# baurst/liso

Measured on AMD Instinct MI355X. Metric: LISO train-step frames/sec (120k-pt clouds), higher is better.
Workload: dtype bf16 (detector, BASELINE configs[2]) + f32 via bf16x3 MFMA (SLIM); north_star's 1e-3 on logits / flow is met by `parity_leg` (f32 via bf16x3 MFMA everywhere) and `fp32_exact_leg`, not by the bf16 detector

## Files before the change

### include/liso_pillars.h

```cpp
#ifndef LISO_PILLARS_H
#define LISO_PILLARS_H

#include <stddef.h>
#include <stdint.h>

#ifdef __cplusplus
extern "C" {
#endif

#define LISO_PFN_OUT 64
#define LISO_PILLARS_MAX_BATCH 32
#define LISO_PFN_STATS_DOUBLES 80

typedef struct {
    float x_min, y_min, z_min;
    float vx, vy, vz;
    int gx, gy;
    int max_points;
    int max_voxels;
    int n_channels;
} liso_pillar_cfg;

size_t liso_pillars_voxelize_workspace_bytes(const liso_pillar_cfg* cfg, int batch, int n_total);

int liso_pillars_voxelize_f32(const float* points, const int* offsets_host, int batch, const liso_pillar_cfg* cfg,
                              int* coors, int* num_points, int* slots, int* num_voxels, int* cell_to_voxel,
                              void* workspace, size_t workspace_bytes, void* stream);

size_t liso_pfn_decorate_workspace_bytes(int batch, int max_voxels);
int liso_pfn_decorate_f32(const float* points, const liso_pillar_cfg* cfg, int batch, const int* coors, const int* num_points,
                          const int* slots, const int* num_voxels, int* pt_off, float* feat, int* voxel_cell, void* workspace,
                          size_t workspace_bytes, void* stream);

size_t liso_pfn_partials_bytes(void);
int liso_pfn_bn_prepare_f32(const float* feat, const int* pt_off, const liso_pillar_cfg* cfg, int batch, const int* num_voxels,
                            const float* weight, const float* gamma, const float* beta, float* running_mean,
                            float* running_var, float momentum, float eps, int training, float* bn_out, double* moments,
                            void* partials, void* stream);

int liso_pfn_forward_scatter(const float* feat, const int* pt_off, const int* voxel_cell, const liso_pillar_cfg* cfg, int batch,
                             const int* cell_to_voxel, const float* weight, const float* bn_out, void* canvas, int out_bf16,
                             float* occupancy, void* stream);

int liso_pfn_forward_rows(const float* feat, const int* pt_off, const int* voxel_cell, const liso_pillar_cfg* cfg, int batch,
                          const int* cell_to_voxel, const float* weight, const float* bn_out, void* rows, int out_bf16, int row_base,
                          int* cell_to_row, float* occupancy, void* stream);

int liso_pfn_backward(const float* feat, const int* pt_off, const int* voxel_cell, const liso_pillar_cfg* cfg, int batch,
                      const int* num_voxels, const float* weight, const float* gamma, const float* bn_out,
                      const double* moments, int training, const void* grad_canvas, int grad_bf16, float* grad_weight,
                      float* grad_gamma, float* grad_beta, void* partials, void* stream);

#ifdef __cplusplus
}
#endif
#endif
```

### liso_amd/_lib.py

```python
import ctypes
import os

import torch

_HERE = os.path.dirname(os.path.abspath(__file__))
LIB_PATH = os.path.join(_HERE, "libliso_hip.so")

_lib = None


class LisoHipError(RuntimeError):
    pass


_ERRORS = {-1: "LISO_EINVAL (bad pointer/size)", -2: "LISO_EWORKSPACE (workspace too small)",
           -3: "LISO_ELAUNCH (HIP launch failed)", -4: "LISO_GROUND_ELENGTH (int(67 / delta_R) > 255)"}


def _preload_torch_hip_runtime():
    tl = os.path.join(os.path.dirname(torch.__file__), "lib", "libamdhip64.so")
    if os.path.exists(tl):
        ctypes.CDLL(tl, mode=ctypes.RTLD_GLOBAL)


def lib():
    global _lib
    if _lib is None:
        if not os.path.exists(LIB_PATH):
            raise LisoHipError(
                f"{LIB_PATH} not found: build it with `python -c 'import __graft_entry__ as g; g.build()'` "
                "or `make -C liso_amd/csrc`.  liso_amd has no CPU fallback for device ops.")
        _preload_torch_hip_runtime()
        _lib = ctypes.CDLL(LIB_PATH)
        _declare(_lib)
    return _lib


def check(code, what):
    if code != 0:
        raise LisoHipError(f"{what} failed: {_ERRORS.get(code, code)}")


def stream_ptr(device=None):
    return ctypes.c_void_p(torch.cuda.current_stream(device).cuda_stream)


def ptr(t):
    return ctypes.c_void_p(t.data_ptr())


def multi_copy(pairs):
    import torch

    fast = []
    for d, s_ in pairs:
        if (d.is_cuda and s_.is_cuda and d.device == s_.device and d.dtype == s_.dtype and d.shape == s_.shape and d.is_contiguous()
                and s_.is_contiguous() and (not fast or fast[0][0].device == d.device)):
            if d.numel() and d.data_ptr() != s_.data_ptr():
                fast.append((d, s_))
        else:
            d.copy_(s_, non_blocking=True)
    if len(fast) == 1:
        fast[0][0].copy_(fast[0][1], non_blocking=True)
    elif fast:
        n = len(fast)
        dst = (ctypes.c_void_p * n)(*[d.data_ptr() for d, _ in fast])
        src = (ctypes.c_void_p * n)(*[s_.data_ptr() for _, s_ in fast])
        nb = (ctypes.c_size_t * n)(*[d.numel() * d.element_size() for d, _ in fast])
        with torch.cuda.device(fast[0][0].device):
            check(lib().liso_multi_copy(n, dst, src, nb, stream_ptr()), "multi_copy")


def copy_blocks(jobs):
    import torch

    n = len(jobs)
    if n == 0:
        return
    dst = (ctypes.c_void_p * n)()
    src = (ctypes.c_void_p * n)()
    rows = (ctypes.c_uint * n)()
    rb = (ctypes.c_uint * n)()
    ds = (ctypes.c_size_t * n)()
    ss = (ctypes.c_size_t * n)()

    def rows_view(t):
        assert t.dtype == torch.float32 and t.is_cuda
        if t.dim() == 1:
            assert t.stride(0) == 1 or t.numel() <= 1
            return 1, t.numel(), t.numel()
        inner = 1
        for k in range(t.dim() - 1, 0, -1):
            assert t.shape[k] == 1 or t.stride(k) == inner, (tuple(t.shape), t.stride())
            inner *= t.shape[k]
        return t.shape[0], inner, (t.stride(0) if t.shape[0] > 1 else inner)

    for i, (d, s_) in enumerate(jobs):
        assert tuple(d.shape) == tuple(s_.shape), (tuple(d.shape), tuple(s_.shape))
        r, c, dstr = rows_view(d)
        r2, c2, sstr = rows_view(s_)
        assert (r, c) == (r2, c2)
        dst[i], src[i], rows[i], rb[i], ds[i], ss[i] = d.data_ptr(), s_.data_ptr(), r, 4 * c, 4 * dstr, 4 * sstr
    with torch.cuda.device(jobs[0][0].device):
        check(lib().liso_multi_copy_rows(n, dst, src, rows, rb, ds, ss, stream_ptr()), "multi_copy_rows")


def require_cuda(*tensors):
    for t in tensors:
        if not t.is_cuda:
            raise LisoHipError("device op called with a CPU tensor; liso_amd has no CPU fallback")


_vp, _i, _f, _sz, _lg = ctypes.c_void_p, ctypes.c_int, ctypes.c_float, ctypes.c_size_t, ctypes.c_long
_d = ctypes.c_double

SIGNATURES = {
    "liso_iou3d_overlap_bev_f32": (_i, [_vp, _i, _vp, _i, _vp, _vp]),
    "liso_iou3d_iou_bev_f32": (_i, [_vp, _i, _vp, _i, _vp, _vp]),
    "liso_iou3d_nms_workspace_bytes": (_sz, [_i]),
    "liso_iou3d_nms_f32": (_i, [_vp, _i, _f, _vp, _vp, _vp, _sz, _vp]),
    "liso_iou3d_nms_normal_f32": (_i, [_vp, _i, _f, _vp, _vp, _vp, _sz, _vp]),
    "liso_iou3d_iou_bev_cpu_f32": (_i, [_vp, _i, _vp, _i, _vp]),
    "liso_pillars_voxelize_workspace_bytes": (_sz, [_vp, _i, _i]),
    "liso_pillars_voxelize_f32": (_i, [_vp, _vp, _i, _vp, _vp, _vp, _vp, _vp, _vp, _vp, _sz, _vp]),
    "liso_pfn_partials_bytes": (_sz, []),
    "liso_pfn_decorate_workspace_bytes": (_sz, [_i, _i]),
    "liso_pfn_decorate_f32": (_i, [_vp, _vp, _i, _vp, _vp, _vp, _vp, _vp, _vp, _vp, _vp, _sz, _vp]),
    "liso_pfn_bn_prepare_f32": (_i, [_vp, _vp, _vp, _i, _vp, _vp, _vp, _vp, _vp, _vp, _f, _f, _i, _vp, _vp, _vp, _vp]),
    "liso_pfn_forward_scatter": (_i, [_vp, _vp, _vp, _vp, _i, _vp, _vp, _vp, _vp, _i, _vp, _vp]),
    "liso_pfn_forward_rows": (_i, [_vp, _vp, _vp, _vp, _i, _vp, _vp, _vp, _vp, _i, _i, _vp, _vp, _vp]),
    "liso_pfn_backward": (_i, [_vp, _vp, _vp, _vp, _i, _vp, _vp, _vp, _vp, _vp, _i, _vp, _i, _vp, _vp, _vp, _vp, _vp]),
    "liso_kabsch_workspace_bytes": (_sz, [_vp]),
    "liso_kabsch_trafos_f32": (_i, [_vp, _vp, _vp, _vp, _vp, _vp, _vp, _vp, _vp, _vp, _vp, _sz, _vp]),
    "liso_kabsch_trafos_counted_f32": (_i, [_vp, _vp, _vp, _vp, _vp, _vp, _vp, _vp, _vp, _vp, _vp, _vp, _sz, _vp]),
    "liso_symm_ortho_fwd_f64": (_i, [_vp, _i, _vp, _vp, _vp, _vp, _vp]),
    "liso_symm_ortho_bwd_f64": (_i, [_vp, _vp, _vp, _vp, _i, _vp, _vp]),
    "liso_weighted_moments_workspace_bytes": (_sz, [_i]),
    "liso_weighted_moments_fwd_f32": (_i, [_vp, _vp, _vp, _i, ctypes.c_long, _vp, _vp, _sz, _vp]),
    "liso_weighted_moments_bwd_f32": (_i, [_vp, _vp, _vp, _i, ctypes.c_long, _vp, _vp, _vp, _vp, _vp]),
    "liso_bev_dynamic_flow_workspace_bytes": (_sz, [_i, _i, _i]),
    "liso_bev_dynamic_flow_f32": (_i, [_vp, _i, _vp, _vp, _vp, _i, _vp, _i, _i, _i, _i, _vp, _vp, _vp, _sz, _vp]),
    "liso_odom_inverse_minus_eye_f64": (_i, [_vp, _i, _vp, _vp]),
    "liso_fit_box_z_workspace_bytes": (_sz, [_i, _i]),
    "liso_fit_box_z_f32": (_i, [_vp, _i, _i, _vp, _i, _vp, _i, _vp, _i, _f, _vp, _vp, _vp, _vp, _sz, _vp]),
    "liso_dbscan_components": (_i, [_vp, _vp, _vp, _vp, _vp, _vp, _vp, _vp, _vp]),
    "liso_dbscan_labels": (_i, [_vp, _vp, _vp, _vp, _vp, _vp, _vp, _vp, _vp, _vp]),
    "liso_region_props": (_i, [_vp, _i, _i, _i, _i, _vp, _vp, _vp]),
    "liso_region_props_workspace_bytes": (_sz, [_i, _i, _i, _i]),
    "liso_region_props_ws": (_i, [_vp, _i, _i, _i, _i, _vp, _vp, _vp, _sz, _vp]),
    "liso_corr_lookup_fwd_f32": (_i, [_vp, _vp, _vp, _vp, _vp, _vp]),
    "liso_corr_lookup_fwd_tiled_f32": (_i, [_vp, _vp, _vp, _vp, _vp, _vp]),
    "liso_corr_lookup_bwd_dvol_f32": (_i, [_vp, _vp, _vp, _vp, _vp]),
    "liso_corr_pyramid_fwd_f32": (_i, [_vp, _vp, _vp, _vp]),
    "liso_corr_pyramid_bwd_f32": (_i, [_vp, _vp, _vp, _vp]),
    "liso_corr_bwd_features_workspace_bytes": (_sz, [_vp]),
    "liso_corr_bwd_features_f32": (_i, [_vp, _i, _vp, _vp, _vp, _vp, _vp, _vp, _sz, _vp]),
    "liso_rows_combine_f32": (_i, [_lg, _i, _vp, _lg, _vp, _lg, _vp, _lg, _vp, _lg, _vp, _lg, _i, _vp]),
    "liso_gru_out_rows_train_f32": (_i, [_lg, _i, _vp, _lg, _vp, _vp, _lg, _vp, _lg, _vp]),
    "liso_gru_out_rows_bwd_f32": (_i, [_lg, _i, _vp, _lg, _vp, _vp, _lg, _vp, _lg, _vp, _lg, _vp, _vp, _vp]),
    "liso_gru_in_rows_bwd_f32": (_i, [_lg, _i, _vp, _lg, _vp, _lg, _vp, _vp, _vp, _lg, _vp, _lg, _vp, _vp]),
    "liso_raft_state_step_train_f32": (_i, [_i, _i, _vp, _vp, _vp, _vp, _vp, _vp, _vp, _vp, _vp]),
    "liso_raft_pack_output_grads_f32": (_i, [_lg, _i, _vp, _vp, _vp, _vp]),
    "liso_nearest_point_loss_fwd_f32": (_i, [_vp] * 8),
    "liso_nearest_point_loss_bwd_f32": (_i, [_vp] * 9),
    "liso_slim_decode_weights_fwd": (_i, [_vp] * 6 + [_i] + [_vp] * 4),
    "liso_slim_decode_weights_bwd": (_i, [_vp] * 9),
    "liso_slim_decode_points_fwd": (_i, [_vp] * 9),
    "liso_slim_decode_points_bwd": (_i, [_vp] * 11),
    "liso_slim_loss_workspace_bytes": (_sz, []),
    "liso_slim_static_points_loss_fwd": (_i, [_i, ctypes.c_long, _vp, _i, _vp, _vp, _vp, _vp, _vp, _vp, _sz, _vp]),
    "liso_slim_static_points_loss_bwd": (_i, [_i, ctypes.c_long, _vp, _i, _vp, _vp, _vp, _vp, _vp, _vp, _vp, _vp, _vp]),
    "liso_slim_knn_queries": (_i, [_i, _i, ctypes.c_long, _i, _vp, _i, _vp, _vp, _vp, _vp, _vp]),
    "liso_slim_nearest_point_loss_fwd": (_i, [_vp, _vp, _i, _vp, _vp, _vp, _i, _vp, _vp, _vp, _vp, _vp, _sz, _vp]),
    "liso_slim_nearest_point_loss_bwd": (_i, [_vp, _vp, _i, _vp, _vp, _vp, _i, _vp, _vp, _vp, _vp, _vp, _vp, _vp]),
    "liso_bev_gather_fwd_f32": (_i, [_vp, _vp, ctypes.c_long, _i, ctypes.c_float, _vp, _vp]),
    "liso_bev_gather_bwd_f32": (_i, [_vp, _vp, _vp, _vp, ctypes.c_long, _i, _vp, _vp, _vp]),
    "liso_gru_in_fwd_f32": (_i, [_vp, _vp, _vp, ctypes.c_long, _vp, _vp, _vp, _vp, _vp]),
    "liso_gru_in_bwd_f32": (_i, [_vp, _vp, ctypes.c_long, _vp, _vp, _vp, _vp, _vp, _vp, ctypes.c_long, _vp, _vp]),
    "liso_gru_out_fwd_f32": (_i, [ctypes.c_long, _vp, _vp, _vp, _vp, _vp]),
    "liso_gru_out_bwd_f32": (_i, [ctypes.c_long, _vp, _vp, _vp, _vp, _vp, _vp, _vp, _vp]),
    "liso_gru_in_rows_f32": (_i, [ctypes.c_long, _i, _vp, ctypes.c_long, _vp, ctypes.c_long, _vp, _vp, ctypes.c_long, _vp]),
    "liso_gru_out_rows_f32": (_i, [ctypes.c_long, _i, _vp, ctypes.c_long, _vp, _vp, ctypes.c_long, _vp]),
    "liso_multi_copy": (_i, [_i, _vp, _vp, _vp, _vp]),
    "liso_bev_lin_index": (_i, [_vp, _i, _vp, _i, ctypes.c_long, _i, _i, _vp, _vp]),
    "liso_channel_extrema_workspace_bytes": (_sz, []),
    "liso_channel_extrema_f32": (_i, [_vp, ctypes.c_long, _i, _i, _vp, _vp, _sz, _vp]),
    "liso_bev_plan_tile_lin": (_i, [_vp, _i, ctypes.c_long, _i, _i, _i, _i, _vp, _vp]),
    "liso_bev_plan_rank": (_i, [_vp, _vp, ctypes.c_long, _vp, _vp, _vp]),
    "liso_bev_plan_expand": (_i, [_vp, _vp, _vp, _i, ctypes.c_long, _i, _i, _i, _i, _vp, _vp, _vp, _vp]),
    "liso_raft_state_step_f32": (_i, [_i, _i, _vp, ctypes.c_long, _vp, _vp, _vp, _vp]),
    "liso_raft_upsample_scratch_bytes": (_sz, [_vp]),
    "liso_raft_upsample_outputs_fwd_f32": (_i, [_vp] * 5),
    "liso_raft_upsample_outputs_bwd_f32": (_i, [_vp, _vp, _vp, _sz, _vp, _vp, _vp]),
    "liso_centerloss_workspace_bytes": (_sz, [_vp]),
    "liso_centerloss_fwd_f32": (_i, [_vp] * 17 + [_sz, _vp]),
    "liso_centerloss_bwd_f32": (_i, [_vp] * 21),
    "liso_render_center_targets_f32": (_i, [_vp] * 12),
    "liso_conv_pack_weights_batched": (_i, [_vp, _i, _vp]),
    "liso_conv_pack_weights_placed": (_i, [_vp, _i, _i, _vp]),
    "liso_conv_in_finalize": (_i, [_vp, _i, _i, _i, _i, ctypes.c_long, _vp, _vp, _f, _vp, _vp]),
    "liso_residual_affine_relu_f32": (_i, [_vp, _vp, _vp, _i, _i, _vp, _vp, _vp, _i, _i, _vp, _i, ctypes.c_long, _i, _vp]),
    "liso_scan_workspace_bytes": (_sz, [_i, ctypes.c_long]),
    "liso_scan_inclusive_i32": (_i, [_vp, _i, ctypes.c_long, _vp, _vp, _sz, _vp]),
    "liso_mine_boxes_from_regions": (_i, [_vp, _i, _i, _vp, _i, _vp, _i, _f, _f, _vp, _vp, _vp, _vp, _vp, _vp]),
    "liso_mine_filter_compact": (_i, [_vp] * 21),
    "liso_mine_box_motion": (_i, [_vp, _i, _i, _vp, _vp, _vp, _vp]),
    "liso_mine_nms_workspace_bytes": (_sz, [_i, _i]),
    "liso_mine_nms_prepare": (_i, [_i, _i, _i] + [_vp] * 11 + [_sz, _vp]),
    "liso_mine_nms_finish": (_i, [_i, _i, _i] + [_vp] * 16),
    "liso_adamw_step_f32": (_i, [_vp, _vp, _vp, _vp, _sz] + [ctypes.c_double] * 5 + [ctypes.c_long, _vp]),
    "liso_adamw_step_scaled_f32": (_i, [_vp, _vp, _vp, _vp, _sz] + [ctypes.c_double] * 6 + [ctypes.c_long, _vp]),
    "liso_adamw_pack_table_plan": (_i, [_vp, _i, _sz, _vp, _vp]),
    "liso_adamw_pack_table_fill": (_i, [_vp, _i, _sz, _vp, _sz]),
    "liso_adamw_step_packed_f32": (_i, [_vp, _vp, _vp, _vp, _sz] + [ctypes.c_double] * 6 + [ctypes.c_long, _vp, _i, _vp]),
    "liso_grad_nonfinite_f32": (_i, [_vp, _sz, _vp, _vp]),
    "liso_adamw_step_amp_f32": (_i, [_vp, _vp, _vp, _vp, _sz] + [ctypes.c_double] * 6 + [_vp, _vp]),
    "liso_loss_scale_update": (_i, [_vp, ctypes.c_double, ctypes.c_double, _i, _vp]),
    "liso_rmsprop_step_f32": (_i, [_vp, _vp, _vp, _sz] + [ctypes.c_double] * 4 + [_vp]),
    "liso_multi_copy_rows": (_i, [_i, _vp, _vp, _vp, _vp, _vp, _vp, _vp]),
    "liso_gather_f32": (_i, [_i, _vp, _vp, _vp, _vp]),
    "liso_bn_workspace_bytes": (_sz, [_i]),
    "liso_bn_relu_fwd": (_i, [_vp, _i, ctypes.c_long, _i, _vp, _vp, _vp, _vp, _f, _f, _i, _i, _vp, _vp, _vp, _sz, _vp]),
    "liso_in_workspace_bytes": (_sz, [_i, _i]),
    "liso_in_relu_fwd": (_i, [_vp, _i, _i, ctypes.c_long, _i, _vp, _vp, _f, _i, _vp, _vp, _vp, _sz, _vp]),
    "liso_in_relu_bwd": (_i, [_vp, _vp, _i, _i, ctypes.c_long, _i, _vp, _vp, _i, _vp, _vp, _vp, _vp, _sz, _vp]),
    "liso_in_relu_bwd_sum": (_i, [_vp, _vp, _i, _i, ctypes.c_long, _i, _vp, _vp, _i, _vp, _vp, _vp, _vp, _sz, _vp]),
    "liso_bn_relu_bwd": (_i, [_vp, _vp, _i, ctypes.c_long, _i, _vp, _vp, _i, _i, _vp, _vp, _vp, _vp, _sz, _vp]),
    "liso_bn_relu_bwd_strided": (_i, [_vp, ctypes.c_long, _vp, ctypes.c_long, _i, ctypes.c_long, _i, _vp, _vp, _i, _i, _vp, ctypes.c_long, _vp, _vp, _vp, _sz, _vp]),
    "liso_bn_relu_bwd_chained": (_i, [_vp, ctypes.c_long, _vp, ctypes.c_long, _i, ctypes.c_long, _i, _vp, _vp, _i, _i, _vp, ctypes.c_long, _vp, _vp, _vp, _sz, _vp, _vp]),
    "liso_bn_multi_workspace_bytes": (_sz, [_vp, _i, _i]),
    "liso_bn_relu_bwd_multi": (_i, [_vp, ctypes.c_long, _vp, ctypes.c_long, _vp, ctypes.c_long, _i, ctypes.c_long, _vp, _i, _i, _i, _vp, ctypes.c_long,
                                    _vp, _sz, _vp, _vp, _vp]),
    "liso_bn_relu_bwd_multi_check": (_i, [_vp, _i, _i, _i, ctypes.c_long, ctypes.c_long, ctypes.c_long, ctypes.c_long, ctypes.c_long, _vp]),
    "liso_knn_workspace_bytes": (_sz, [_vp, _i]),
    "liso_knn_build_f32": (_i, [_vp, _vp, _i, _i, _vp, _sz, _vp]),
    "liso_knn_sorted_ids": (_i, [_vp, _vp, _i, _vp, _vp]),
    "liso_knn_query_f32": (_i, [_vp, _vp, _vp, _vp, _i, _vp, _i, _i, _vp, _vp, _i, _vp]),
    "liso_conv_packed_bytes": (_sz, [_i, _i, _i, _i]),
    "liso_conv_pack_weights": (_i, [_vp, _i, _i, _i, _i, _i, _i, _i, _vp, _vp]),
    "liso_conv_stats_rows": (_i, [_vp]),
    "liso_conv_kernel_kind": (_i, [_vp]),
    "liso_conv_forward": (_i, [_vp] * 10),
    "liso_conv_set_option": (_i, [_i, _i]),
    "liso_conv_forward_sparse": (_i, [_vp] * 11),
    "liso_conv_plan_info": (_i, [_vp, _vp]),
    "liso_conv_wgrad_workspace_bytes": (_sz, [_vp]),
    "liso_conv_wgrad": (_i, [_vp, _vp, _vp, _vp, _vp, _i, _i, _vp, _vp, _vp, _sz, _vp]),
    "liso_conv_wgrad_deferred": (_i, [_vp, _vp, _vp, _vp, _vp, _i, _i, _vp, _vp, _vp, _sz, _vp, _vp]),
    "liso_conv_wgrad_reduce": (_i, [_vp, _vp]),
    "liso_conv_wgrad_sparse_workspace_bytes": (_sz, [_vp]),
    "liso_conv_wgrad_sparse_f32": (_i, [_vp, _vp, _vp, _vp, _i, _vp, _vp, _vp, _sz, _vp]),
    "liso_conv_wgrad_smallci_workspace_bytes": (_sz, [_i, _i, _i, _i, _i]),
    "liso_conv_wgrad_smallci_f32": (_i, [_vp, ctypes.c_long, _vp, ctypes.c_long, _i, _i, _i, _i, _i, _vp, _vp, _vp, _sz, _vp]),
    "liso_sparse_conv_stat_groups": (_i, [_i, _i, _i]),
    "liso_sparse_conv_workspace_bytes": (_sz, [_i, _i, _i, _i, _i, _i, _i]),
    "liso_sparse_conv_forward": (_i, [_vp, ctypes.c_long, _i, _vp, _vp, _vp, _i, _i, _i, _i, _i, _i, _i, _vp, _vp, _vp, _vp, _vp, _sz, _vp]),
    "liso_sparse_conv_forward_rows": (_i, [_vp, ctypes.c_long, _i, _vp, ctypes.c_long, _vp, _vp, _vp, _i, _i, _i, _i, _i, _i, _i, _vp, _vp, _vp, _vp, _vp,
                                           _sz, _vp]),
    "liso_sparse_conv_dgrad": (_i, [_vp, ctypes.c_long, _i, _vp, _vp, _i, _i, _i, _i, _i, _i, _vp, ctypes.c_long, _vp, _vp, _sz, _i, _vp]),
    "liso_sparse_stem_workspace_bytes": (_sz, [_i, _i, _i, _i]),
    "liso_sparse_stem_forward_f32": (_i, [_vp, ctypes.c_long, _vp, _vp, _vp, _i, _i, _i, _i, _i, _vp, _vp, _vp, _vp, _sz, _vp]),
    "liso_conv_bn_finalize": (_i, [_vp, _i, _i, _i, ctypes.c_long, _vp, _vp, _vp, _vp, _vp, _f, _f, _vp, _vp]),
    "liso_conv_bn_finalize_merged": (_i, [_vp, _i, _i, _i, ctypes.c_long, _vp, _vp, _vp, _vp, _vp, _f, _f, _vp, _vp, _vp, _i, _i, _vp]),
    "liso_points_in_boxes_workspace_bytes": (_sz, [_vp]),
    "liso_points_in_boxes_f32": (_i, [_vp] * 9 + [_sz, _vp]),
    "liso_match_greedy_f32": (_i, [_vp, ctypes.c_long, ctypes.c_long, _i, _i, _vp, _f, _vp, _vp, _vp, _vp, _vp, _vp, _vp]),
    "liso_fit_boxes_closeness_workspace_bytes": (_sz, [ctypes.c_long, _i]),
    "liso_fit_boxes_closeness_f32": (_i, [_vp, ctypes.c_long, _i, _vp, _vp, _i, _f, _vp, _vp, _vp, _sz, _vp]),
    "liso_bike_rollout_fwd_f32": (_i, [_i, _i, _vp, _vp, _vp, _vp, _f, _f, _f, _vp, _vp]),
    "liso_bike_rollout_bwd_f32": (_i, [_i, _i, _vp, _vp, _vp, _f, _f, _f, _vp, _vp, _vp, _vp, _vp, _vp]),
    "liso_smooth_tracks_jerk_f32": (_i, [_vp, _vp, _i, _i, _i, _f, _f, _vp, _vp]),
    "liso_flow_metrics_state_bytes": (_sz, []),
    "liso_flow_metrics_result_bytes": (_sz, []),
    "liso_flow_metrics_reset": (_i, [_vp, _vp]),
    "liso_flow_metrics_update": (_i, [_vp, _lg, _vp, _lg, _vp, _lg, _i, _vp, _lg, _vp, _lg, _vp, _lg, _vp, _vp, _vp, _vp, _i, _vp, _vp]),
    "liso_flow_metrics_read": (_i, [_vp, _vp, _vp]),
    "liso_det_nms_workspace_bytes": (_sz, [_i, _i]),
    "liso_det_nms_order": (_i, [_i, _i, _vp, _vp, _vp, _f, _vp, _vp, _vp, _sz, _vp]),
    "liso_det_nms_select": (_i, [_i, _i, _vp, _vp, _vp, _f, _i, _i, _vp, _vp, _vp]),
    "liso_det_nms_gather": (_i, [_i, _i, _i, _vp, _vp, _vp, _i, _vp]),
    "liso_det_val_pairs_f32": (_i, [_i, _i, _i] + [_vp] * 8),
    "liso_det_val_pairs_cpu_f32": (_i, [_i, _i, _i] + [_vp] * 7),
    "liso_det_val_transfer_classes": (_i, [_i, _i, _i] + [_vp] * 5 + [_f, _vp, _vp, _vp]),
    "liso_det_val_match_f32": (_i, [_i, _i, _i] + [_vp] * 10 + [_i, _vp, _i, _vp, _i] + [_vp] * 6),
    "liso_det_val_assign_f32": (_i, [_i, _i, _i] + [_vp] * 8 + [_i, _vp, _i, _vp, _i] + [_vp] * 5),
    "liso_match_assign_f32": (_i, [_vp, ctypes.c_long, _i, _i, _f, _vp, _vp, _vp]),
    "liso_ground_jcp_workspace_bytes": (_sz, [_vp]),
    "liso_ground_jcp_f32": (_i, [_vp, _vp, _vp, _vp, _vp, _sz, _vp]),
    "liso_ground_jcp_stages_f32": (_i, [_vp, _vp, _vp, _vp, _vp, _sz, _i, _i, _vp]),
    "liso_ground_cone_f32": (_i, [_i, _i, _i, _vp, _vp, ctypes.c_double, ctypes.c_double, _vp, _vp, _vp]),
    "liso_ground_compact_workspace_bytes": (_sz, [_i, _i]),
    "liso_ground_compact_f32": (_i, [_i, _i, _i, _vp, _vp, _vp, _vp, _vp, _vp, _sz, _vp]),
    "liso_bev_free_mask_workspace_bytes": (_sz, [_i, _i]),
    "liso_bev_free_mask": (_i, [_vp, ctypes.c_long, _i, _i, _i, _vp, _vp, _vp, _sz, _vp]),
    "liso_bev_select_free_cells": (_i, [_vp, _vp, _i, _i, _vp, _i, _vp, _vp]),
    "liso_snippet_paste": (_i, [_vp, ctypes.c_long, _vp, _vp, _vp, _vp, ctypes.c_double, ctypes.c_double, _i, _vp, _vp, _vp, _vp]),
    "liso_sample_transform_f32": (_i, [_i, _i, _i] + [_vp] * 7),
    "liso_sample_transform_poses_f64": (_i, [_i, _vp, _vp, _i, _vp, _i, _vp]),
    "liso_bev_crop_workspace_bytes": (_sz, [_i, _i]),
    "liso_bev_crop_f32": (_i, [_vp] * 14 + [_sz, _vp]),
    "liso_bev_point_maps_workspace_bytes": (_sz, [_i, _i, _i, _i]),
    "liso_bev_point_maps_f32": (_i, [_i] * 5 + [_vp] * 6 + [ctypes.c_double] + [_vp] * 5 + [_sz, _vp]),
    "liso_box_has_points_f32": (_i, [_i] * 4 + [_vp] * 7),
    "liso_filter_boxes": (_i, [_vp] * 6 + [_i] + [_vp] * 3),
    "liso_object_velocity_f64": (_i, [_i, _i] + [_vp] * 5),
    "liso_ignore_region_mask": (_i, [_i] * 4 + [ctypes.c_double] * 2 + [_vp] * 6),
    "liso_render_center_targets_ex_f32": (_i, [_vp] * 15),
    "liso_snippet_cut_workspace_bytes": (_sz, [_i, _i, _i]),
    "liso_snippet_cut_f32": (_i, [_i, _i, _i, _vp, _vp, _vp, _i, _vp, _vp, _lg] + [_vp] * 5 + [_sz, _vp]),
    "liso_track_sequences_workspace_bytes": (_sz, [_i, _i, _i, _i]),
    "liso_track_sequences": (_i, [_i] * 4 + [_vp] * 7 + [ctypes.c_double] + [_vp] * 10 + [_sz, _vp]),
    "liso_track_mining_workspace_bytes": (_sz, [_i] * 5),
    "liso_select_tracks": (_i, [_i] * 5 + [_vp] * 7 + [_i, _f, _d, _d, _i, _d, _d, _i, _d] + [_vp] * 13 + [_vp, _sz, _vp]),
    "liso_refine_tracks_apply": (_i, [_i] * 3 + [_vp] * 12 + [_i, _i, _d] + [_vp] * 7 + [_vp]),
    "liso_export_tracks": (_i, [_i] * 6 + [_vp] * 11 + [_i] + [_vp] * 13 + [_vp, _sz, _vp]),
    "liso_frame_prep_workspace_bytes": (_sz, [_vp]),
    "liso_prepare_tracker_frames": (_i, [_vp] * 27 + [_sz, _vp]),
    "liso_odometry_workspace_bytes": (_sz, [_vp]),
    "liso_odometry_workspace_layout": (_i, [_vp, _vp]),
    "liso_odometry_preprocess": (_i, [_vp, _i, _vp, _vp, _vp, _vp, _vp, _sz, _vp]),
    "liso_odometry_register": (_i, [_vp, _i] + [_vp] * 8 + [_sz, _vp]),
    "liso_odometry_map_update": (_i, [_vp, _i, _vp, _vp, _vp, _vp, _sz, _vp]),
    "liso_odometry_sequences": (_i, [_vp] * 11 + [_sz, _vp]),
    "liso_odometry_relative_f64": (_i, [_i, _vp, _vp, _vp, _vp]),
    "liso_correct_kitti_scan_f64": (_i, [_lg, _vp, _vp, _vp]),
    "liso_flow_labels_workspace_bytes": (_sz, [_i, _i]),
    "liso_flow_labels_f32": (_i, [_vp] * 18 + [_sz, _vp]),
    "liso_kitti_rows_cols_f32": (_i, [_i, _i, _i, _vp, _vp, _d, _i, _i, _vp, _vp, _vp]),
}


CONV_MAX_TAPS, CONV_MAX_CLASSES, CONV_BF16, CONV_F32X3, CONV_F32, CONV_F16 = 49, 4, 0, 1, 2, 3
ELEM_F32, ELEM_BF16, ELEM_F16 = 0, 1, 2
_ELEM_CODES = {torch.float32: ELEM_F32, torch.bfloat16: ELEM_BF16, torch.float16: ELEM_F16}
LOSS_SCALE_STATE_BYTES = 32


def elem_code(dtype):
    code = _ELEM_CODES.get(dtype)
    if code is None:
        raise TypeError(f"no device kernel takes {dtype} tensors (float32, bfloat16 or float16)")
    return code


def is_half(dtype):
    return elem_code(dtype) != ELEM_F32


def lane_channels(dtype):
    return 8 if is_half(dtype) else 4
CONV_OPT_SHARED_GPU = 1
CONV_OPT_ROLES_CUS = 2


class ConvDesc(ctypes.Structure):
    _fields_ = [("batch", _i), ("hi", _i), ("wi", _i), ("ci", _i), ("x_pix_stride", _i), ("ho", _i), ("wo", _i), ("co", _i),
                ("y_pix_stride", _i), ("y_ch_off", _i), ("hv", _i), ("wv", _i), ("isy", _i), ("isx", _i), ("osy", _i), ("osx", _i),
                ("n_classes", _i), ("class_tap_begin", _i * (CONV_MAX_CLASSES + 1)), ("class_ooy", _i * CONV_MAX_CLASSES),
                ("class_oox", _i * CONV_MAX_CLASSES), ("n_taps", _i), ("tap_dy", _i * CONV_MAX_TAPS), ("tap_dx", _i * CONV_MAX_TAPS),
                ("tap_w", _i * CONV_MAX_TAPS), ("w_taps", _i), ("mode", _i), ("out_f32", _i), ("in_relu", _i), ("out_relu", _i),
                ("in_affine_batch_stride", _i), ("wgrad_co", _i)]


class ConvPackPlacedJob(ctypes.Structure):
    _fields_ = [("src", _vp), ("dst", _vp), ("d0", _i), ("d1", _i), ("kh", _i), ("kw", _i), ("transposed", _i), ("for_dgrad", _i),
                ("mode", _i), ("K", _i), ("N", _i), ("k_offset", _i), ("n_offset", _i)]


class AdamwPackDest(ctypes.Structure):
    _fields_ = [("dst", _vp), ("for_dgrad", _i), ("mode", _i), ("K", _i), ("N", _i), ("k_offset", _i), ("n_offset", _i)]


class AdamwPackItem(ctypes.Structure):
    _fields_ = [("offset", _sz), ("d0", _i), ("d1", _i), ("kh", _i), ("kw", _i), ("transposed", _i), ("n_dest", _i),
                ("dest", AdamwPackDest * 2), ("mirror", _vp), ("mirror_row_stride", _sz)]


class ConvPackJob(ctypes.Structure):
    _fields_ = [("src", _vp), ("dst", _vp), ("d0", _i), ("d1", _i), ("kh", _i), ("kw", _i), ("transposed", _i), ("for_dgrad", _i),
                ("mode", _i)]


class WgradReduceJob(ctypes.Structure):
    _fields_ = [("slab", _vp), ("bias_slab", _vp), ("dw", _vp), ("dbias", _vp), ("cip", ctypes.c_long), ("cop", ctypes.c_long),
                ("splits", _i), ("bias_rows", _i), ("taps", _i), ("ci", _i), ("co", _i), ("transposed", _i)]


BN_MAX_GROUPS = 4


class BnGroup(ctypes.Structure):
    _fields_ = [("c_off", _i), ("c", _i), ("gamma", _vp), ("stats", _vp), ("grad_gamma", _vp), ("grad_beta", _vp)]


class KnnGrid(ctypes.Structure):
    _fields_ = [("x_min", _f), ("y_min", _f), ("cell", _f), ("nx", _i), ("ny", _i), ("z_min", _f), ("z_cell", _f), ("nz", _i)]


class CenterLossCfg(ctypes.Structure):
    _fields_ = [("batch", _i), ("h", _i), ("w", _i), ("res_x", _f), ("res_y", _f), ("z_min", _f), ("z_max", _f),
                ("sup_weight", _f), ("rot_reg_weight", _f)]


class NpLossCfg(ctypes.Structure):
    _fields_ = [("batch", _i), ("n", ctypes.c_long), ("n_b", ctypes.c_long), ("ext", _f * 4), ("fov_mode", _i), ("delta", _f)]


class SlimDecodeCfg(ctypes.Structure):
    _fields_ = [("samples", _i), ("n", ctypes.c_long), ("h", _i), ("w", _i), ("logit_mode", _i * 4), ("static_flow_zero", _i),
                ("dynamic_flow_zero", _i), ("overwrite_flow", _i), ("overwrite_logits", _i), ("non_rigid", _i), ("use_static_aggr", _i),
                ("dyn_grad_scale", _f), ("ext_lo", ctypes.c_double * 2), ("ext_span", ctypes.c_double * 2)]


class SlimDecodeOut(ctypes.Structure):
    FIELDS = ("dis_logit", "dis", "logits", "probs", "staticness", "dynamicness", "groundness", "dyn_flow", "stat_flow", "agg_flow", "saf_flow")
    _fields_ = [(k, _vp) for k in FIELDS] + [("flags", _vp)]


class SlimNpLossCfg(ctypes.Structure):
    _fields_ = [("samples", _i), ("clouds", _i), ("n", ctypes.c_long), ("n_b", ctypes.c_long), ("ext", _f * 4), ("fov_mode", _i), ("delta", _f)]


class BoxPtsCfg(ctypes.Structure):
    _fields_ = [("batch", _i), ("n", ctypes.c_long), ("k", _i), ("point_stride", _i), ("precision", _i), ("dims_bloat", _f)]


class FramePrepCfg(ctypes.Structure):
    _fields_ = [("n_seq", _i), ("max_frames", _i), ("max_box", _i), ("cap", _i), ("n_points", ctypes.c_long), ("point_stride", _i),
                ("n_fov_points", ctypes.c_long), ("fov_stride", _i), ("bev_range_x", _f), ("bev_range_y", _f), ("drop_on_bev_boundaries", _i),
                ("min_points_in_box", _i), ("fov_min_points", _i), ("align", _i), ("no_align_below_m", _d), ("full_align_above_m", _d)]


class OdometryCfg(ctypes.Structure):
    _fields_ = [("n_seq", _i), ("max_frames", _i), ("n_max", _i), ("point_stride", _i), ("map_voxels", _i), ("max_points_per_voxel", _i),
                ("max_num_iterations", _i), ("max_range", _d), ("min_range", _d), ("voxel_size", _d), ("initial_threshold", _d),
                ("min_motion_th", _d), ("convergence_criterion", _d)]


class GruCfg(ctypes.Structure):
    _fields_ = [("batch", _i), ("ch", _i), ("cx", _i), ("hw", ctypes.c_long)]


class UpsampleCfg(ctypes.Structure):
    _fields_ = [("n_it", _i), ("batch2", _i), ("dirs", _i), ("h", _i), ("w", _i), ("factor", _i), ("flow_scale", _f)]


class MineFilterCfg(ctypes.Structure):
    _fields_ = [("batch", _i), ("k", _i), ("min_points", _i), ("aspect_ratio_max", ctypes.c_double), ("max_box_len_m", ctypes.c_double),
                ("min_box_area_m2", ctypes.c_double), ("min_box_volume_m3", ctypes.c_double), ("park_invalid", _i)]


class DetGatherField(ctypes.Structure):
    _fields_ = [("src", _vp), ("dst", _vp), ("row_elems", _i), ("elem_bytes", _i), ("pad_bits", ctypes.c_uint64)]


class GroundCfg(ctypes.Structure):
    _fields_ = [("batch", _i), ("n_max", _i), ("point_stride", _i), ("width", _i), ("height", _i),
                ("sensor_height", ctypes.c_double), ("delta_r", ctypes.c_double)]


class TargetsCfg(ctypes.Structure):
    _fields_ = [("batch", _i), ("n_boxes", _i), ("h", _i), ("w", _i), ("range_x", _f), ("range_y", _f)]


class DbscanCfg(ctypes.Structure):
    _fields_ = [("batch", _i), ("gx", _i), ("gy", _i), ("window", _i), ("min_samples", _i), ("eps", _f), ("flow_weight", _f)]


class CorrCfg(ctypes.Structure):
    _fields_ = [("batch", _i), ("h", _i), ("w", _i), ("dim", _i), ("levels", _i), ("radius", _i)]


class KabschCfg(ctypes.Structure):
    _fields_ = [("batch", _i), ("n_points", _i), ("n_slots", _i), ("point_stride", _i), ("flow_stride", _i),
                ("slope", _f), ("scale_fg", _f), ("scale_bg", _f), ("softness", _i)]


class PillarCfg(ctypes.Structure):
    _fields_ = [("x_min", _f), ("y_min", _f), ("z_min", _f), ("vx", _f), ("vy", _f), ("vz", _f), ("gx", _i),
                ("gy", _i), ("max_points", _i), ("max_voxels", _i), ("n_channels", _i)]


class _Everything:
    def __contains__(self, name):
        return True


class KernelTimer:

    def __init__(self):
        self.enabled = set()
        self.events = {}
        self.units = {}
        self.bytes = {}
        self.weights = {}
        self.weight = 1.0

    def enable(self, name):
        self.enabled.add(name)
        self.events.setdefault(name, [])

    def enable_all(self):
        self.enabled = _Everything()

    def disable_all(self):
        self.enabled = set()

    def launch(self, name, fn, units=None, nbytes=None):
        if name not in self.enabled:
            return fn()
        a, b = torch.cuda.Event(enable_timing=True), torch.cuda.Event(enable_timing=True)
        a.record()
        r = fn()
        b.record()
        self.events.setdefault(name, []).append((a, b))
        self.weights.setdefault(name, []).append(float(self.weight))
        if units is not None:
            self.units.setdefault(name, []).append(units)
        if nbytes is not None:
            self.bytes.setdefault(name, []).append(nbytes)
        return r

    def mean_units(self, name):
        u = self.units.get(name, [])
        return sum(u) / len(u) if u else None

    def durations_ms(self, name):
        torch.cuda.synchronize()
        return [a.elapsed_time(b) for a, b in self.events.get(name, [])]

    def weighted_total_ms(self, name):
        return sum(d * w for d, w in zip(self.durations_ms(name), self.weights.get(name, [])))

    def reset(self):
        for k in self.events:
            self.events[k] = []
        self.units = {}
        self.bytes = {}
        self.weights = {}


TIMER = KernelTimer()


def _declare(l):
    for name, (res, args) in SIGNATURES.items():
        fn = getattr(l, name)
        fn.restype = res
        fn.argtypes = args
```

### liso_amd/csrc/pillars.hip

```cpp
#include <hip/hip_runtime.h>
#include <stdlib.h>
#include "zero_fill.h"
#include <cstring>
#include <hip/hip_bf16.h>
#include <limits.h>
#include <stdint.h>

#include "../../include/liso_iou3d.h"
#include "../../include/liso_conv.h"
#include "../../include/liso_pillars.h"
#include "dev_common.h"

namespace {

using liso_dev::check_launch;

constexpr int kTile = 1024;
constexpr int kOut = LISO_PFN_OUT;
constexpr int kFP = 12;
constexpr int kMaxPts = 32;
constexpr int kPfnThreads = 256;
constexpr int kPfnGrid = 1024;

struct BatchInfo {
    int off[LISO_PILLARS_MAX_BATCH + 1];
    int tile_off[LISO_PILLARS_MAX_BATCH + 1];
};

__device__ __forceinline__ int sample_of(const BatchInfo& bi, int batch, int i) {
    int b = 0;
    while (b + 1 < batch && i >= bi.off[b + 1]) b++;
    return b;
}

__global__ void assign_kernel(const float* __restrict__ pts, int n_total, int C, BatchInfo bi, int batch,
                              liso_pillar_cfg cfg, int* __restrict__ cell_of_point, int* __restrict__ count,
                              int* __restrict__ first_enc, int* __restrict__ pos_in_cell) {
    const int i = blockIdx.x * blockDim.x + threadIdx.x;
    int cell = -1;
    if (i < n_total) {
        const float* p = pts + (size_t)i * C;
        const float cx = floorf((p[0] - cfg.x_min) / cfg.vx);
        const float cy = floorf((p[1] - cfg.y_min) / cfg.vy);
        const float cz = floorf((p[2] - cfg.z_min) / cfg.vz);
        const bool ok = cx >= 0.f && cx < (float)cfg.gx && cy >= 0.f && cy < (float)cfg.gy && cz >= 0.f && cz < 1.f;
        if (ok) cell = (sample_of(bi, batch, i) * cfg.gx + (int)cx) * cfg.gy + (int)cy;
        cell_of_point[i] = cell;
    }
    const int lane = threadIdx.x & 63;
    const int prev = __shfl_up(cell, 1);
    const unsigned long long heads = __ballot(lane == 0 || cell != prev);
    const unsigned long long below = heads & ((2ull << lane) - 1ull);
    const int head_lane = 63 - __builtin_clzll(below);
    const unsigned long long above = lane == 63 ? 0ull : heads & ~((2ull << lane) - 1ull);
    const int next_head = above ? __ffsll((long long)above) - 1 : 64;
    int base = 0;
    if (cell >= 0 && head_lane == lane) {
        base = atomicAdd(&count[cell], next_head - lane);
        atomicMax(&first_enc[cell], INT_MAX - i);
    }
    base = __shfl(base, head_lane);
    if (i < n_total) pos_in_cell[i] = cell >= 0 ? base + (lane - head_lane) : 0;
}

__device__ __forceinline__ bool is_first(const int* cell_of_point, const int* first_enc, int i) {
    const int cell = cell_of_point[i];
    return cell >= 0 && first_enc[cell] == INT_MAX - i;
}

__global__ __launch_bounds__(kTile) void tile_count_kernel(const int* __restrict__ cell_of_point,
                                                           const int* __restrict__ first_enc, BatchInfo bi, int batch,
                                                           int* __restrict__ tile_count) {
    __shared__ int wsum[kTile / 64];
    const int tile = blockIdx.x;
    int b = 0;
    while (b + 1 < batch && tile >= bi.tile_off[b + 1]) b++;
    const int i = bi.off[b] + (tile - bi.tile_off[b]) * kTile + threadIdx.x;
    const bool f = i < bi.off[b + 1] && is_first(cell_of_point, first_enc, i);
    const unsigned long long m = __ballot(f);
    if ((threadIdx.x & 63) == 0) wsum[threadIdx.x >> 6] = __popcll(m);
    __syncthreads();
    if (threadIdx.x == 0) {
        int s = 0;
        for (int w = 0; w < kTile / 64; w++) s += wsum[w];
        tile_count[tile] = s;
    }
}

__global__ __launch_bounds__(kTile) void rank_kernel(const int* __restrict__ cell_of_point,
                                                     const int* __restrict__ first_enc,
                                                     const int* __restrict__ count, BatchInfo bi, int batch,
                                                     liso_pillar_cfg cfg, const int* __restrict__ tile_count,
                                                     int* __restrict__ coors, int* __restrict__ num_points,
                                                     int* __restrict__ cell_to_voxel, int* __restrict__ num_voxels) {
    __shared__ int wsum[kTile / 64];
    __shared__ int base_s;
    const int tile = blockIdx.x;
    int b = 0;
    while (b + 1 < batch && tile >= bi.tile_off[b + 1]) b++;
    if (threadIdx.x < 64) {
        int s = 0;
        for (int t = bi.tile_off[b] + threadIdx.x; t < tile; t += 64) s += tile_count[t];
        for (int o = 32; o > 0; o >>= 1) s += __shfl_xor(s, o);
        if (threadIdx.x == 0) base_s = s;
    }
    const int i = bi.off[b] + (tile - bi.tile_off[b]) * kTile + threadIdx.x;
    const bool f = i < bi.off[b + 1] && is_first(cell_of_point, first_enc, i);
    const unsigned long long m = __ballot(f);
    const int lane = threadIdx.x & 63, wave = threadIdx.x >> 6;
    if (lane == 0) wsum[wave] = __popcll(m);
    __syncthreads();
    int pre = base_s;
    for (int w = 0; w < wave; w++) pre += wsum[w];
    if (f) {
        const int ord = pre + __popcll(m & ((1ULL << lane) - 1ULL));
        if (ord < cfg.max_voxels) {
            const int cell = cell_of_point[i];
            const int v = b * cfg.max_voxels + ord;
            cell_to_voxel[cell] = v + 1;
            const int within = cell - b * cfg.gx * cfg.gy;
            coors[v * 4 + 0] = b;
            coors[v * 4 + 1] = 0;
            coors[v * 4 + 2] = within / cfg.gy;
            coors[v * 4 + 3] = within % cfg.gy;
            const int c = count[cell];
            num_points[v] = c < cfg.max_points ? c : cfg.max_points;
        }
    }
    if (tile == bi.tile_off[b + 1] - 1 && threadIdx.x == 0) {
        int tot = base_s;
        for (int w = 0; w < kTile / 64; w++) tot += wsum[w];
        num_voxels[b] = tot < cfg.max_voxels ? tot : cfg.max_voxels;
    }
}

constexpr int kScanTile = 1024;
__global__ __launch_bounds__(kScanTile) void cell_scan_block_kernel(const int* __restrict__ count, size_t cells, int* __restrict__ seg_off,
                                                                    int* __restrict__ block_tot) {
    __shared__ int wsum[kScanTile / 64];
    const size_t i = (size_t)blockIdx.x * kScanTile + threadIdx.x;
    const int lane = threadIdx.x & 63, wave = threadIdx.x >> 6;
    const int v = i < cells ? count[i] : 0;
    int incl = v;
#pragma unroll
    for (int o = 1; o < 64; o <<= 1) {
        const int t = __shfl_up(incl, o);
        if (lane >= o) incl += t;
    }
    if (lane == 63) wsum[wave] = incl;
    __syncthreads();
    int base = 0;
    for (int w = 0; w < wave; w++) base += wsum[w];
    if (i < cells) seg_off[i] = base + incl - v;
    if (threadIdx.x == kScanTile - 1) block_tot[blockIdx.x] = base + incl;
}

__global__ __launch_bounds__(1024) void cell_scan_tot_kernel(int* __restrict__ block_tot, int nblk) {
    __shared__ int wsum[16];
    const int t = threadIdx.x, lane = t & 63, wave = t >> 6;
    int v[4], tot = 0;
#pragma unroll
    for (int k = 0; k < 4; k++) {
        const int q = t * 4 + k;
        v[k] = q < nblk ? block_tot[q] : 0;
        tot += v[k];
    }
    int incl = tot;
#pragma unroll
    for (int o = 1; o < 64; o <<= 1) {
        const int up = __shfl_up(incl, o);
        if (lane >= o) incl += up;
    }
    if (lane == 63) wsum[wave] = incl;
    __syncthreads();
    int base = 0;
    for (int w = 0; w < wave; w++) base += wsum[w];
    int run = base + incl - tot;
#pragma unroll
    for (int k = 0; k < 4; k++) {
        const int q = t * 4 + k;
        if (q < nblk) block_tot[q] = run;
        run += v[k];
    }
}

__global__ __launch_bounds__(256) void seg_fill_kernel(const int* __restrict__ cell_of_point, int n_total, const int* __restrict__ seg_off,
                                                       const int* __restrict__ block_tot, const int* __restrict__ pos_in_cell,
                                                       int* __restrict__ seg) {
    const int i = blockIdx.x * blockDim.x + threadIdx.x;
    if (i >= n_total) return;
    const int c = cell_of_point[i];
    if (c < 0) return;
    seg[seg_off[c] + block_tot[c / kScanTile] + pos_in_cell[i]] = i;
}

constexpr int kSlotRegs = 16;
__device__ __forceinline__ void voxel_slots_one(const int* __restrict__ coors, const int* __restrict__ num_voxels, int max_voxels, int gx, int gy,
                                                const int* __restrict__ seg_off, const int* __restrict__ block_tot,
                                                const int* __restrict__ count, const int* __restrict__ seg, int max_points,
                                                int* __restrict__ slots, long v, int lane) {
    const int b = (int)(v / max_voxels), ord = (int)(v % max_voxels);
    if (ord >= num_voxels[b]) return;
    const int c = (b * gx + coors[v * 4 + 2]) * gy + coors[v * 4 + 3];
    const int off = seg_off[c] + block_tot[c / kScanTile], n = count[c];
    int* out = slots + (size_t)v * max_points;
    if (n <= 64) {
        const int e = lane < n ? seg[off + lane] : 0x7fffffff;
        int r = 0;
        for (int k = 0; k < n; k++) r += __shfl(e, k) < e ? 1 : 0;
        if (lane < n && r < max_points) out[r] = e;
        return;
    }
    int last = -1;
    const int rounds = min(max_points, n);
    if (n <= 64 * kSlotRegs) {
        int x[kSlotRegs];
#pragma unroll
        for (int u = 0; u < kSlotRegs; u++) x[u] = lane + 64 * u < n ? seg[off + lane + 64 * u] : 0x7fffffff;
        for (int r = 0; r < rounds; r++) {
            int m = 0x7fffffff;
#pragma unroll
            for (int u = 0; u < kSlotRegs; u++) m = (x[u] > last && x[u] < m) ? x[u] : m;
#pragma unroll
            for (int o = 32; o > 0; o >>= 1) m = min(m, __shfl_xor(m, o));
            if (lane == 0) out[r] = m;
            last = m;
        }
        return;
    }
    for (int r = 0; r < rounds; r++) {
        int m = 0x7fffffff;
        for (int j = lane; j < n; j += 64) {
            const int x = seg[off + j];
            m = (x > last && x < m) ? x : m;
        }
#pragma unroll
        for (int o = 32; o > 0; o >>= 1) m = min(m, __shfl_xor(m, o));
        if (lane == 0) out[r] = m;
        last = m;
    }
}

__global__ __launch_bounds__(256) void voxel_slots_kernel(const int* __restrict__ coors, const int* __restrict__ num_voxels, int max_voxels,
                                                          int batch, int gx, int gy, const int* __restrict__ seg_off,
                                                          const int* __restrict__ block_tot, const int* __restrict__ count,
                                                          const int* __restrict__ seg, int max_points, int* __restrict__ slots) {
    const int lane = threadIdx.x & 63;
    for (long v = (long)blockIdx.x * 4 + (threadIdx.x >> 6); v < (long)batch * max_voxels; v += (long)gridDim.x * 4)
        voxel_slots_one(coors, num_voxels, max_voxels, gx, gy, seg_off, block_tot, count, seg, max_points, slots, v, lane);
}

struct PfnGeom {
    float vx, vy, x_off, y_off, z_off;
};

__device__ __forceinline__ PfnGeom pfn_geom(const liso_pillar_cfg& c) {
    PfnGeom g;
    g.vx = c.vx; g.vy = c.vy;
    g.x_off = c.vx / 2 + c.x_min;
    g.y_off = c.vy / 2 + c.y_min;
    g.z_off = c.vz / 2 + c.z_min;
    return g;
}

constexpr int kGroup = 4;
constexpr int kStage = kGroup * kMaxPts;

__device__ __forceinline__ int kept_points(const int* __restrict__ num_points, const int* __restrict__ num_voxels, int max_voxels,
                                           int rows, int v) {
    if (v >= rows) return 0;
    const int b = v / max_voxels;
    return (v - b * max_voxels) < num_voxels[b] ? num_points[v] : 0;
}

__global__ __launch_bounds__(1024) void pfn_scan_block_kernel(const int* __restrict__ num_points, const int* __restrict__ num_voxels,
                                                              int max_voxels, int rows, int* __restrict__ pt_off,
                                                              int* __restrict__ block_tot) {
    __shared__ int wsum[16];
    const int i = blockIdx.x * 1024 + threadIdx.x;
    const int lane = threadIdx.x & 63, wave = threadIdx.x >> 6;
    const int v = kept_points(num_points, num_voxels, max_voxels, rows, i);
    int incl = v;
    for (int off = 1; off < 64; off <<= 1) {
        const int t = __shfl_up(incl, off);
        if (lane >= off) incl += t;
    }
    if (lane == 63) wsum[wave] = incl;
    __syncthreads();
    int base = 0;
    for (int w = 0; w < wave; w++) base += wsum[w];
    if (i < rows) pt_off[i] = base + incl - v;
    if (threadIdx.x == 1023) block_tot[blockIdx.x] = base + incl;
}

__global__ __launch_bounds__(1024) void pfn_scan_tot_kernel(int* __restrict__ block_tot, int nblocks) {
    __shared__ int wsum[16];
    const int lane = threadIdx.x & 63, wave = threadIdx.x >> 6;
    const int v = (int)threadIdx.x < nblocks ? block_tot[threadIdx.x] : 0;
    int incl = v;
    for (int off = 1; off < 64; off <<= 1) {
        const int t = __shfl_up(incl, off);
        if (lane >= off) incl += t;
    }
    if (lane == 63) wsum[wave] = incl;
    __syncthreads();
    int base = 0;
    for (int w = 0; w < wave; w++) base += wsum[w];
    if ((int)threadIdx.x < nblocks) block_tot[threadIdx.x] = base + incl - v;
    if ((int)threadIdx.x == nblocks - 1) block_tot[nblocks] = base + incl;
}

__global__ __launch_bounds__(1024) void pfn_scan_add_kernel(int* __restrict__ pt_off, int rows, const int* __restrict__ block_tot,
                                                            int nblocks) {
    const int i = blockIdx.x * 1024 + threadIdx.x;
    if (i < rows) pt_off[i] += block_tot[blockIdx.x];
    if (i == 0) pt_off[rows] = block_tot[nblocks];
}

template <int C>
__global__ __launch_bounds__(256) void pfn_decorate_kernel(const float* __restrict__ pts, liso_pillar_cfg cfg, int rows,
                                                           const int* __restrict__ coors, const int* __restrict__ num_points,
                                                           const int* __restrict__ slots, const int* __restrict__ num_voxels,
                                                           const int* __restrict__ pt_off, float* __restrict__ feat,
                                                           int* __restrict__ voxel_cell) {
#pragma clang fp contract(off)
    constexpr int F = C + 6;
    const long t = (long)blockIdx.x * blockDim.x + threadIdx.x;
    const int v = (int)(t >> 5), s = (int)(t & 31);
    if (v >= rows) return;
    const int num = kept_points(num_points, num_voxels, cfg.max_voxels, rows, v);
    const int xi = coors[v * 4 + 2], yi = coors[v * 4 + 3];
    if (s == 0) voxel_cell[v] = num > 0 ? ((v / cfg.max_voxels) * cfg.gx + xi) * cfg.gy + yi : -1;
    float p[C];
#pragma unroll
    for (int k = 0; k < C; k++) p[k] = 0.f;
    if (s < num) {
        const int idx = slots[(size_t)v * cfg.max_points + s];
        const float* q = pts + (size_t)idx * C;
        if constexpr (C == 4) {
            const float4 tt = *reinterpret_cast<const float4*>(q);
            p[0] = tt.x; p[1] = tt.y; p[2] = tt.z; p[3] = tt.w;
        } else {
#pragma unroll
            for (int k = 0; k < C; k++) p[k] = q[k];
        }
    }
    float sx = p[0], sy = p[1], sz = p[2];
#pragma unroll
    for (int o = 16; o > 0; o >>= 1) {
        sx += __shfl_xor(sx, o);
        sy += __shfl_xor(sy, o);
        sz += __shfl_xor(sz, o);
    }
    if (s >= num) return;
    const PfnGeom g = pfn_geom(cfg);
    const float fn = (float)num;
    const float mx = sx / fn, my = sy / fn, mz = sz / fn;
    const float fcx = p[0] - ((float)yi * g.vx + g.x_off);
    const float fcy = p[1] - ((float)xi * g.vy + g.y_off);
    const float fcz = p[2] - (0.f + g.z_off);
    float f[kFP];
#pragma unroll
    for (int k = 0; k < kFP; k++) f[k] = 0.f;
    f[0] = fcx; f[1] = fcy; f[2] = fcz;
#pragma unroll
    for (int k = 3; k < C; k++) f[k] = p[k];
    f[C + 0] = p[0] - mx; f[C + 1] = p[1] - my; f[C + 2] = p[2] - mz;
    f[C + 3] = fcx; f[C + 4] = fcy; f[C + 5] = fcz;
    f[F] = 1.f;
    float4* row = reinterpret_cast<float4*>(feat + ((size_t)pt_off[v] + s) * kFP);
    row[0] = make_float4(f[0], f[1], f[2], f[3]);
    row[1] = make_float4(f[4], f[5], f[6], f[7]);
    row[2] = make_float4(f[8], f[9], f[10], f[11]);
}

template <int C>
__global__ __launch_bounds__(kPfnThreads) void pfn_stats_kernel(const float* __restrict__ feat, const int* __restrict__ pt_off,
                                                                int rows, double* __restrict__ partials) {
    constexpr int F = C + 6, D = F + 1, NP = D * (D + 1) / 2;
    __shared__ __attribute__((aligned(16))) float tile[kPfnThreads / 64][64][kFP];
    __shared__ double red[kPfnThreads / 64][LISO_PFN_STATS_DOUBLES];
    const int lane = threadIdx.x & 63, wave = threadIdx.x >> 6;
    int pj[2] = {0, 0}, pk[2] = {0, 0};
    {
        int idx = 0;
        for (int j = 0; j < D; j++)
            for (int k = j; k < D; k++, idx++) {
                if (idx == lane) { pj[0] = j; pk[0] = k; }
                if (idx == lane + 64) { pj[1] = j; pk[1] = k; }
            }
    }
    const long n = pt_off[rows];
    const long waves = (long)gridDim.x * (kPfnThreads / 64);
    const long per = ((n + waves - 1) / waves + 63) / 64 * 64;
    const long w_id = (long)blockIdx.x * (kPfnThreads / 64) + wave;
    const long r0 = w_id * per, r1 = r0 + per < n ? r0 + per : n;
    double acc0 = 0.0, acc1 = 0.0;
    for (long base = r0; base < r1; base += 64) {
        const int cnt = (int)(r1 - base < 64 ? r1 - base : 64);
        const float4* src = reinterpret_cast<const float4*>(feat + (size_t)base * kFP);
        float4* dst = reinterpret_cast<float4*>(&tile[wave][0][0]);
        for (int i = lane; i < cnt * 3; i += 64) dst[i] = src[i];
        __builtin_amdgcn_wave_barrier();
        for (int s = 0; s < cnt; s++) {
            const float* f = tile[wave][s];
            acc0 += (double)f[pj[0]] * (double)f[pk[0]];
            if (lane + 64 < NP) acc1 += (double)f[pj[1]] * (double)f[pk[1]];
        }
        __builtin_amdgcn_wave_barrier();
    }
    red[wave][lane] = acc0;
    if (lane + 64 < LISO_PFN_STATS_DOUBLES) red[wave][lane + 64] = lane + 64 < NP ? acc1 : 0.0;
    __syncthreads();
    if (threadIdx.x < LISO_PFN_STATS_DOUBLES) {
        double s = 0.0;
        for (int w = 0; w < kPfnThreads / 64; w++) s += red[w][threadIdx.x];
        partials[(size_t)blockIdx.x * LISO_PFN_STATS_DOUBLES + threadIdx.x] = threadIdx.x < NP ? s : 0.0;
    }
}

__device__ __forceinline__ int pair_index(int j, int k, int D) {
    return j * D - j * (j - 1) / 2 + (k - j);
}

template <int C>
__global__ __launch_bounds__(1024) void pfn_bn_finalize_kernel(const double* __restrict__ partials, int nblocks,
                                                               const int* __restrict__ num_voxels, int batch,
                                                               int max_points, const float* __restrict__ weight,
                                                               const float* __restrict__ gamma,
                                                               const float* __restrict__ beta,
                                                               float* __restrict__ running_mean,
                                                               float* __restrict__ running_var, float momentum,
                                                               float eps, float* __restrict__ bn_out,
                                                               double* __restrict__ moments) {
    constexpr int F = C + 6, D = F + 1;
    constexpr int NS = LISO_PFN_STATS_DOUBLES, CH = 1024 / NS;
    __shared__ double part[CH][NS];
    __shared__ double mom[NS];
    const int e = threadIdx.x % NS, chunk = threadIdx.x / NS;
    if (chunk < CH) {
        double s = 0.0;
        const int per = (nblocks + CH - 1) / CH;
        const int lo = chunk * per, hi = lo + per < nblocks ? lo + per : nblocks;
        int blk = lo;
        for (; blk + 16 <= hi; blk += 16) {
            double v[16];
#pragma unroll
            for (int j = 0; j < 16; j++) v[j] = partials[(size_t)(blk + j) * NS + e];
#pragma unroll
            for (int j = 0; j < 16; j++) s += v[j];
        }
        for (; blk < hi; blk++) s += partials[(size_t)blk * NS + e];
        part[chunk][e] = s;
    }
    __syncthreads();
    if (threadIdx.x < NS) {
        double t = 0.0;
        for (int c = 0; c < CH; c++) t += part[c][threadIdx.x];
        mom[threadIdx.x] = t;
        moments[threadIdx.x] = t;
    }
    __syncthreads();
    __shared__ double rows_sq[kOut][F + 1], rows_sum[kOut][F + 1];
    if (threadIdx.x < kOut * F) {
        const int c = threadIdx.x / F, j = threadIdx.x % F;
        const double wj = (double)weight[c * F + j];
        double q = 0.0;
        for (int k = 0; k < F; k++) {
            const int a = j <= k ? j : k, bb = j <= k ? k : j;
            q += wj * (double)weight[c * F + k] * mom[pair_index(a, bb, D)];
        }
        rows_sq[c][j] = q;
        rows_sum[c][j] = wj * mom[pair_index(j, D - 1, D)];
    }
    __syncthreads();
    if (threadIdx.x < kOut) {
        const int c = threadIdx.x;
        long long P = 0;
        for (int b = 0; b < batch; b++) P += num_voxels[b];
        const double M = (double)P * (double)max_points;
        double sum = 0.0, sq = 0.0;
        for (int j = 0; j < F; j++) {
            sum += rows_sum[c][j];
            sq += rows_sq[c][j];
        }
        double mean = 0.0, var = 0.0;
        if (M > 0.0) {
            mean = sum / M;
            var = sq / M - mean * mean;
            if (var < 0.0) var = 0.0;
        }
        const double invstd = 1.0 / sqrt(var + (double)eps);
        const float scale = (float)((double)gamma[c] * invstd);
        bn_out[c] = scale;
        bn_out[kOut + c] = (float)((double)beta[c] - mean * (double)gamma[c] * invstd);
        bn_out[2 * kOut + c] = (float)mean;
        bn_out[3 * kOut + c] = (float)invstd;
        if (M > 1.0) {
            const double mo = (double)momentum;
            running_mean[c] = (float)((1.0 - mo) * (double)running_mean[c] + mo * mean);
            running_var[c] = (float)((1.0 - mo) * (double)running_var[c] + mo * (var * M / (M - 1.0)));
        }
    }
}

__global__ void pfn_bn_eval_kernel(const float* __restrict__ gamma, const float* __restrict__ beta,
                                   const float* __restrict__ running_mean, const float* __restrict__ running_var,
                                   float eps, float* __restrict__ bn_out) {
    const int c = threadIdx.x;
    if (c >= kOut) return;
    const float invstd = 1.f / sqrtf(running_var[c] + eps);
    bn_out[c] = gamma[c] * invstd;
    bn_out[kOut + c] = beta[c] - running_mean[c] * gamma[c] * invstd;
    bn_out[2 * kOut + c] = running_mean[c];
    bn_out[3 * kOut + c] = invstd;
}

template <typename T> __device__ __forceinline__ void store_out(T* p, float v);
template <> __device__ __forceinline__ void store_out<float>(float* p, float v) { *p = v; }
template <> __device__ __forceinline__ void store_out<__hip_bfloat16>(__hip_bfloat16* p, float v) { *p = __float2bfloat16(v); }
template <typename T> __device__ __forceinline__ float load_in(const T* p);
template <> __device__ __forceinline__ float load_in<float>(const float* p) { return *p; }
template <> __device__ __forceinline__ float load_in<__hip_bfloat16>(const __hip_bfloat16* p) { return __bfloat162float(*p); }
template <> __device__ __forceinline__ void store_out<_Float16>(_Float16* p, float v) { *p = (_Float16)v; }
template <> __device__ __forceinline__ float load_in<_Float16>(const _Float16* p) { return (float)*p; }

__device__ __forceinline__ void stage_rows(const float* __restrict__ feat, const int* __restrict__ pt_off, int rows, int v0, int lane,
                                           float (*frow)[kFP], int (&off)[kGroup + 1]) {
    int o = 0;
    if (lane <= kGroup) { const int v = v0 + lane; o = pt_off[v < rows ? v : rows]; }
#pragma unroll
    for (int g = 0; g <= kGroup; g++) off[g] = __shfl(o, g);
    const int total = off[kGroup] - off[0];
    const float4* src = reinterpret_cast<const float4*>(feat + (size_t)off[0] * kFP);
    float4* dst = reinterpret_cast<float4*>(&frow[0][0]);
    for (int i = lane; i < total * 3; i += 64) dst[i] = src[i];
}

constexpr int kCellsPerBlock = 256;

template <int C, typename OutT, bool ROWS>
__global__ __launch_bounds__(kPfnThreads) void pfn_forward_kernel(const float* __restrict__ feat, const int* __restrict__ pt_off,
                                                                  const int* __restrict__ voxel_cell, int rows, int max_points,
                                                                  long total_cells, int zero_blocks,
                                                                  const int* __restrict__ cell_to_voxel,
                                                                  const float* __restrict__ weight, const float* __restrict__ bn,
                                                                  OutT* __restrict__ canvas, float* __restrict__ occupancy,
                                                                  int* __restrict__ map_out, int row_base) {
    constexpr int F = C + 6;
    constexpr int kChunks = kOut * (int)sizeof(OutT) / 16;
    __shared__ __attribute__((aligned(16))) float frow[kPfnThreads / 64][kStage][kFP];
    __shared__ int vox[kCellsPerBlock];
    const int tid = threadIdx.x, lane = tid & 63, wave = tid >> 6;
    const int pillar_blocks = (int)gridDim.x - zero_blocks;
    if ((int)blockIdx.x >= pillar_blocks) {
        const long cell0 = (long)((int)blockIdx.x - pillar_blocks) * kCellsPerBlock;
        const long cell = cell0 + tid;
        int v1 = 0;
        if (cell < total_cells) {
            v1 = cell_to_voxel[cell];
            occupancy[cell] = v1 > 0 ? 1.f : 0.f;
            if constexpr (ROWS) map_out[cell] = v1 > 0 ? v1 + row_base : 0;
        }
        if constexpr (ROWS) return;
        vox[tid] = v1;
        __syncthreads();
        const uint4 z = make_uint4(0u, 0u, 0u, 0u);
        uint4* base = reinterpret_cast<uint4*>(canvas + (size_t)cell0 * kOut);
        for (int id = tid; id < kCellsPerBlock * kChunks; id += kPfnThreads) {
            const int cl = id / kChunks;
            if (cell0 + cl < total_cells && vox[cl] == 0) base[id] = z;
        }
        return;
    }
    float w[F];
#pragma unroll
    for (int k = 0; k < F; k++) w[k] = weight[lane * F + k];
    const float scale = bn[lane], shift = bn[kOut + lane];
    const float pad_val = fmaxf(shift, 0.f);
    const int wave_id = (int)blockIdx.x * (kPfnThreads / 64) + wave;
    const int n_waves = pillar_blocks * (kPfnThreads / 64);
    for (int v0 = wave_id * kGroup; v0 < rows; v0 += n_waves * kGroup) {
        int off[kGroup + 1];
        stage_rows(feat, pt_off, rows, v0, lane, frow[wave], off);
        int cell_l = -1;
        if (lane < kGroup && v0 + lane < rows) cell_l = voxel_cell[v0 + lane];
        __builtin_amdgcn_wave_barrier();
#pragma unroll
        for (int g = 0; g < kGroup; g++) {
            const int num = off[g + 1] - off[g];
            const int cell = __shfl(cell_l, g);
            if (num <= 0 || cell < 0) continue;
            float best = num < max_points ? pad_val : 0.f;
            const int r0 = off[g] - off[0];
            for (int s = 0; s < num; s++) {
                const float4* f4 = reinterpret_cast<const float4*>(frow[wave][r0 + s]);
                const float4 a = f4[0], b = f4[1], c4 = f4[2];
                const float f[kFP] = {a.x, a.y, a.z, a.w, b.x, b.y, b.z, b.w, c4.x, c4.y, c4.z, c4.w};
                float x = 0.f;
#pragma unroll
                for (int k = 0; k < F; k++) x = fmaf(w[k], f[k], x);
                best = fmaxf(best, fmaxf(fmaf(x, scale, shift), 0.f));
            }
            store_out<OutT>(canvas + (size_t)(ROWS ? v0 + g : cell) * kOut + lane, best);
        }
        __builtin_amdgcn_wave_barrier();
    }
}

template <int C, typename GT>
__global__ __launch_bounds__(kPfnThreads) void pfn_backward_kernel(const float* __restrict__ feat, const int* __restrict__ pt_off,
                                                                   const int* __restrict__ voxel_cell, int rows, int max_points,
                                                                   const float* __restrict__ weight, const float* __restrict__ bn,
                                                                   const GT* __restrict__ grad_canvas,
                                                                   float* __restrict__ partials) {
    constexpr int F = C + 6, NA = F + 2;
    __shared__ __attribute__((aligned(16))) float frow[kPfnThreads / 64][kStage][kFP];
    __shared__ float red[kPfnThreads / 64][NA][kOut];
    const int lane = threadIdx.x & 63, wave = threadIdx.x >> 6;
    float w[F], acc[NA];
#pragma unroll
    for (int k = 0; k < F; k++) w[k] = weight[lane * F + k];
#pragma unroll
    for (int k = 0; k < NA; k++) acc[k] = 0.f;
    const float scale = bn[lane], shift = bn[kOut + lane], mean = bn[2 * kOut + lane], invstd = bn[3 * kOut + lane];
    const float pad_val = fmaxf(shift, 0.f);
    const int wave_id = (int)blockIdx.x * (kPfnThreads / 64) + wave;
    const int n_waves = (int)gridDim.x * (kPfnThreads / 64);
    for (int v0 = wave_id * kGroup; v0 < rows; v0 += n_waves * kGroup) {
        int off[kGroup + 1];
        stage_rows(feat, pt_off, rows, v0, lane, frow[wave], off);
        int cell_l = -1;
        if (lane < kGroup && v0 + lane < rows) cell_l = voxel_cell[v0 + lane];
        __builtin_amdgcn_wave_barrier();
#pragma unroll
        for (int g = 0; g < kGroup; g++) {
            const int num = off[g + 1] - off[g];
            const int cell = __shfl(cell_l, g);
            if (num <= 0 || cell < 0) continue;
            const int r0 = off[g] - off[0];
            float best = -1.f, best_x = 0.f;
            int best_s = -1;
            for (int s = 0; s < num; s++) {
                const float* f = frow[wave][r0 + s];
                float x = 0.f;
#pragma unroll
                for (int k = 0; k < F; k++) x = fmaf(w[k], f[k], x);
                const float y = fmaxf(fmaf(x, scale, shift), 0.f);
                if (y > best) { best = y; best_s = s; best_x = x; }
            }
            if (num < max_points && pad_val > best) { best = pad_val; best_s = -1; best_x = 0.f; }
            const float gy = load_in<GT>(grad_canvas + (size_t)cell * kOut + lane);
            const float dz = best > 0.f ? gy : 0.f;
            if (best_s >= 0) {
                const float* f = frow[wave][r0 + best_s];
#pragma unroll
                for (int k = 0; k < F; k++) acc[k] = fmaf(dz, f[k], acc[k]);
            }
            acc[F] += dz;
            acc[F + 1] = fmaf(dz, (best_x - mean) * invstd, acc[F + 1]);
        }
        __builtin_amdgcn_wave_barrier();
    }
#pragma unroll
    for (int k = 0; k < NA; k++) red[wave][k][lane] = acc[k];
    __syncthreads();
    for (int idx = threadIdx.x; idx < NA * kOut; idx += kPfnThreads) {
        const int k = idx / kOut, c = idx % kOut;
        float s = 0.f;
        for (int wv = 0; wv < kPfnThreads / 64; wv++) s += red[wv][k][c];
        partials[((size_t)blockIdx.x * NA + k) * kOut + c] = s;
    }
}

template <int NA>
__global__ __launch_bounds__(1024) void pfn_backward_reduce_kernel(const float* __restrict__ partials, int nblocks,
                                                                   double* __restrict__ tot) {
    __shared__ double part[16][kOut];
    const int k = blockIdx.x, c = threadIdx.x & 63, chunk = threadIdx.x >> 6;
    const int per = (nblocks + 15) / 16;
    const int lo = chunk * per, hi = lo + per < nblocks ? lo + per : nblocks;
    double s = 0.0;
    {
        int blk = lo;
        for (; blk + 8 <= hi; blk += 8) {
            float v[8];
#pragma unroll
            for (int j = 0; j < 8; j++) v[j] = partials[((size_t)(blk + j) * NA + k) * kOut + c];
#pragma unroll
            for (int j = 0; j < 8; j++) s += (double)v[j];
        }
        for (; blk < hi; blk++) s += (double)partials[((size_t)blk * NA + k) * kOut + c];
    }
    part[chunk][c] = s;
    __syncthreads();
    if (chunk == 0) {
        double t = 0.0;
        for (int q = 0; q < 16; q++) t += part[q][c];
        tot[k * kOut + c] = t;
    }
}

template <int C>
__global__ __launch_bounds__(64) void pfn_backward_finalize_kernel(const double* __restrict__ tot,
                                                                   const int* __restrict__ num_voxels, int batch,
                                                                   int max_points, const float* __restrict__ weight,
                                                                   const float* __restrict__ gamma,
                                                                   const float* __restrict__ bn,
                                                                   const double* __restrict__ moments, int training,
                                                                   float* __restrict__ grad_weight,
                                                                   float* __restrict__ grad_gamma,
                                                                   float* __restrict__ grad_beta) {
    constexpr int F = C + 6, D = F + 1;
    const int c = threadIdx.x;
    if (c >= kOut) return;
    const double dbeta = tot[F * kOut + c], dgamma = tot[(F + 1) * kOut + c];
    grad_beta[c] = (float)dbeta;
    grad_gamma[c] = (float)dgamma;
    const double invstd = (double)bn[3 * kOut + c], mean = (double)bn[2 * kOut + c];
    const double gi = (double)gamma[c] * invstd;
    if (!training) {
        for (int k = 0; k < F; k++) grad_weight[c * F + k] = (float)(gi * tot[k * kOut + c]);
        return;
    }
    long long P = 0;
    for (int b = 0; b < batch; b++) P += num_voxels[b];
    const double M = (double)P * (double)max_points;
    double w[F];
    for (int k = 0; k < F; k++) w[k] = (double)weight[c * F + k];
    for (int k = 0; k < F; k++) {
        const double Fk = moments[pair_index(k, D - 1, D)];
        double xf = 0.0;
        for (int j = 0; j < F; j++) {
            const int a = j <= k ? j : k, bb = j <= k ? k : j;
            xf += w[j] * moments[pair_index(a, bb, D)];
        }
        const double xhat_f = invstd * (xf - mean * Fk);
        const double dw = M > 0.0 ? gi * (tot[k * kOut + c] - dbeta / M * Fk - dgamma / M * xhat_f) : 0.0;
        grad_weight[c * F + k] = (float)dw;
    }
}

inline bool cfg_ok(const liso_pillar_cfg* c, int batch) {
    return c && batch >= 1 && batch <= LISO_PILLARS_MAX_BATCH && c->gx > 0 && c->gy > 0 && c->max_points >= 1 &&
           c->max_points <= kMaxPts && c->max_voxels >= 1 && c->n_channels >= 3 && c->n_channels <= 5;
}

inline BatchInfo make_batch(const int* off, int batch) {
    BatchInfo bi;
    bi.tile_off[0] = 0;
    for (int b = 0; b <= LISO_PILLARS_MAX_BATCH; b++) bi.off[b] = off[b <= batch ? b : batch];
    for (int b = 0; b < LISO_PILLARS_MAX_BATCH; b++) {
        const int n = b < batch ? off[b + 1] - off[b] : 0;
        bi.tile_off[b + 1] = bi.tile_off[b] + (n + kTile - 1) / kTile;
    }
    return bi;
}

inline int pfn_grid(int rows) {
    const int need = (rows + kPfnThreads / 64 - 1) / (kPfnThreads / 64);
    return need < kPfnGrid ? (need > 0 ? need : 1) : kPfnGrid;
}

}

extern "C" {

size_t liso_pillars_voxelize_workspace_bytes(const liso_pillar_cfg* cfg, int batch, int n_total) {
    if (!cfg_ok(cfg, batch) || n_total < 0) return 0;
    const size_t cells = (size_t)batch * cfg->gx * cfg->gy;
    const size_t tiles = (size_t)(n_total + kTile - 1) / kTile + batch;
    if (cells > (size_t)4096 * kScanTile) return 0;
    return (3 * cells + 3 * (size_t)n_total + tiles + 64 + 4096) * sizeof(int) + 256;
}

int liso_pillars_voxelize_f32(const float* points, const int* offsets_host, int batch, const liso_pillar_cfg* cfg,
                              int* coors, int* num_points, int* slots, int* num_voxels, int* cell_to_voxel,
                              void* workspace, size_t workspace_bytes, void* stream) {
    if (!cfg_ok(cfg, batch) || !offsets_host) return LISO_EINVAL;
    const int n_total = offsets_host[batch];
    if (n_total < 0 || offsets_host[0] != 0) return LISO_EINVAL;
    for (int b = 0; b < batch; b++)
        if (offsets_host[b + 1] < offsets_host[b]) return LISO_EINVAL;
    if (!coors || !num_points || !slots || !num_voxels || !cell_to_voxel || !workspace || (n_total > 0 && !points))
        return LISO_EINVAL;
    if ((size_t)batch * cfg->gx * cfg->gy > (size_t)4096 * kScanTile) return LISO_EINVAL;
    if (workspace_bytes < liso_pillars_voxelize_workspace_bytes(cfg, batch, n_total)) return LISO_EWORKSPACE;
    hipStream_t st = (hipStream_t)stream;
    const size_t cells = (size_t)batch * cfg->gx * cfg->gy;
    int* count = (int*)workspace;
    int* first_enc = count + cells;
    int* cell_of_point = first_enc + cells;
    int* tile_count = cell_of_point + n_total;
    const size_t tiles_cap = (size_t)(n_total + kTile - 1) / kTile + batch;
    int* seg_off = tile_count + tiles_cap + 32;
    int* pos_in_cell = seg_off + cells;
    int* seg = pos_in_cell + n_total;
    int* block_tot = seg + n_total;
    const BatchInfo bi = make_batch(offsets_host, batch);
    const int tiles = bi.tile_off[batch];
    if (liso_zero::zero_async(count, 2 * cells * sizeof(int), st) != hipSuccess) return LISO_ELAUNCH;
    if (liso_zero::zero_async(cell_to_voxel, cells * sizeof(int), st) != hipSuccess) return LISO_ELAUNCH;
    if (liso_zero::zero_async(num_voxels, batch * sizeof(int), st) != hipSuccess) return LISO_ELAUNCH;
    if (n_total == 0) return LISO_OK;
    const int nb = (n_total + 255) / 256;
    hipLaunchKernelGGL(assign_kernel, dim3(nb), dim3(256), 0, st, points, n_total, cfg->n_channels, bi, batch, *cfg,
                       cell_of_point, count, first_enc, pos_in_cell);
    hipLaunchKernelGGL(tile_count_kernel, dim3(tiles), dim3(kTile), 0, st, cell_of_point, first_enc, bi, batch,
                       tile_count);
    hipLaunchKernelGGL(rank_kernel, dim3(tiles), dim3(kTile), 0, st, cell_of_point, first_enc, count, bi, batch, *cfg,
                       tile_count, coors, num_points, cell_to_voxel, num_voxels);
    const int scan_blocks = (int)((cells + kScanTile - 1) / kScanTile);
    cell_scan_block_kernel<<<scan_blocks, kScanTile, 0, st>>>(count, cells, seg_off, block_tot);
    cell_scan_tot_kernel<<<1, 1024, 0, st>>>(block_tot, scan_blocks);
    seg_fill_kernel<<<nb, 256, 0, st>>>(cell_of_point, n_total, seg_off, block_tot, pos_in_cell, seg);
    const long n_wave = (long)batch * cfg->max_voxels;
    voxel_slots_kernel<<<(unsigned)((n_wave + 3) / 4), 256, 0, st>>>(coors, num_voxels, cfg->max_voxels, batch, cfg->gx, cfg->gy, seg_off,
                                                                   block_tot, count, seg, cfg->max_points, slots);
    return check_launch();
}

size_t liso_pfn_partials_bytes(void) {
    const size_t stats = (size_t)kPfnGrid * LISO_PFN_STATS_DOUBLES * sizeof(double);
    const size_t bwd = (size_t)kPfnGrid * (11 + 2) * kOut * sizeof(float) + (11 + 2) * kOut * sizeof(double);
    return stats > bwd ? stats : bwd;
}

size_t liso_pfn_decorate_workspace_bytes(int batch, int max_voxels) {
    if (batch < 1 || max_voxels < 1) return 0;
    return ((size_t)(batch * (long)max_voxels + 1023) / 1024 + 2) * sizeof(int);
}

int liso_pfn_decorate_f32(const float* points, const liso_pillar_cfg* cfg, int batch, const int* coors, const int* num_points,
                          const int* slots, const int* num_voxels, int* pt_off, float* feat, int* voxel_cell, void* workspace,
                          size_t workspace_bytes, void* stream) {
    if (!cfg_ok(cfg, batch) || !coors || !num_points || !slots || !num_voxels || !pt_off || !feat || !voxel_cell || !workspace)
        return LISO_EINVAL;
    if (workspace_bytes < liso_pfn_decorate_workspace_bytes(batch, cfg->max_voxels)) return LISO_EWORKSPACE;
    const int rows = batch * cfg->max_voxels;
    const int nsb = (rows + 1023) / 1024;
    if (nsb > 1024) return LISO_EINVAL;
    hipStream_t st = (hipStream_t)stream;
    int* block_tot = (int*)workspace;
    pfn_scan_block_kernel<<<nsb, 1024, 0, st>>>(num_points, num_voxels, cfg->max_voxels, rows, pt_off, block_tot);
    pfn_scan_tot_kernel<<<1, 1024, 0, st>>>(block_tot, nsb);
    pfn_scan_add_kernel<<<nsb, 1024, 0, st>>>(pt_off, rows, block_tot, nsb);
    const unsigned grid = (unsigned)(((long)rows * 32 + 255) / 256);
    switch (cfg->n_channels) {
        case 3: pfn_decorate_kernel<3><<<grid, 256, 0, st>>>(points, *cfg, rows, coors, num_points, slots, num_voxels, pt_off, feat, voxel_cell); break;
        case 4: pfn_decorate_kernel<4><<<grid, 256, 0, st>>>(points, *cfg, rows, coors, num_points, slots, num_voxels, pt_off, feat, voxel_cell); break;
        default: pfn_decorate_kernel<5><<<grid, 256, 0, st>>>(points, *cfg, rows, coors, num_points, slots, num_voxels, pt_off, feat, voxel_cell); break;
    }
    return check_launch();
}

int liso_pfn_bn_prepare_f32(const float* feat, const int* pt_off, const liso_pillar_cfg* cfg, int batch, const int* num_voxels,
                            const float* weight, const float* gamma, const float* beta, float* running_mean,
                            float* running_var, float momentum, float eps, int training, float* bn_out, double* moments,
                            void* partials, void* stream) {
    if (!cfg_ok(cfg, batch) || !gamma || !beta || !running_mean || !running_var || !bn_out) return LISO_EINVAL;
    hipStream_t st = (hipStream_t)stream;
    if (!training) {
        pfn_bn_eval_kernel<<<1, 64, 0, st>>>(gamma, beta, running_mean, running_var, eps, bn_out);
        return check_launch();
    }
    if (!feat || !pt_off || !num_voxels || !weight || !moments || !partials) return LISO_EINVAL;
    const int rows = batch * cfg->max_voxels;
    const int grid = kPfnGrid;
#define LISO_PREP(CC)                                                                                                     \
    do {                                                                                                                  \
        pfn_stats_kernel<CC><<<grid, kPfnThreads, 0, st>>>(feat, pt_off, rows, (double*)partials);                           \
        pfn_bn_finalize_kernel<CC><<<1, 1024, 0, st>>>((const double*)partials, grid, num_voxels, batch, cfg->max_points,    \
                                                      weight, gamma, beta, running_mean, running_var, momentum, eps, bn_out, \
                                                      moments);                                                           \
    } while (0)
    switch (cfg->n_channels) {
        case 3: LISO_PREP(3); break;
        case 4: LISO_PREP(4); break;
        default: LISO_PREP(5); break;
    }
#undef LISO_PREP
    return check_launch();
}

static int pfn_forward_launch(const float* feat, const int* pt_off, const int* voxel_cell, const liso_pillar_cfg* cfg, int batch,
                              const int* cell_to_voxel, const float* weight, const float* bn_out, void* canvas, int out_bf16,
                              float* occupancy, int* map_out, int row_base, bool compact, void* stream) {
    if (!cfg_ok(cfg, batch) || !feat || !pt_off || !voxel_cell || !cell_to_voxel || !weight || !bn_out || !canvas || !occupancy)
        return LISO_EINVAL;
    if (out_bf16 != LISO_ELEM_F32 && out_bf16 != LISO_ELEM_BF16 && out_bf16 != LISO_ELEM_F16) return LISO_EINVAL;
    hipStream_t st = (hipStream_t)stream;
    const long cells = (long)batch * cfg->gx * cfg->gy;
    const int rows = batch * cfg->max_voxels;
    const int zero_blocks = (int)((cells + kCellsPerBlock - 1) / kCellsPerBlock);
    const int groups = (rows + kGroup - 1) / kGroup;
    int pfn_blocks = (groups + kPfnThreads / 64 - 1) / (kPfnThreads / 64);
    if (pfn_blocks > 4096) pfn_blocks = 4096;
    const unsigned grid = (unsigned)(zero_blocks + pfn_blocks);
#define LISO_FWD_(CC, T, R) pfn_forward_kernel<CC, T, R><<<grid, kPfnThreads, 0, st>>>(feat, pt_off, voxel_cell, rows, cfg->max_points, cells, zero_blocks, cell_to_voxel, weight, bn_out, (T*)canvas, occupancy, map_out, row_base)
#define LISO_FWD(CC, T) do { if (compact) LISO_FWD_(CC, T, true); else LISO_FWD_(CC, T, false); } while (0)
    switch (cfg->n_channels * 3 + out_bf16) {
        case 9: LISO_FWD(3, float); break;
        case 10: LISO_FWD(3, __hip_bfloat16); break;
        case 11: LISO_FWD(3, _Float16); break;
        case 12: LISO_FWD(4, float); break;
        case 13: LISO_FWD(4, __hip_bfloat16); break;
        case 14: LISO_FWD(4, _Float16); break;
        case 15: LISO_FWD(5, float); break;
        case 16: LISO_FWD(5, __hip_bfloat16); break;
        default: LISO_FWD(5, _Float16); break;
    }
#undef LISO_FWD
#undef LISO_FWD_
    return check_launch();
}

int liso_pfn_forward_scatter(const float* feat, const int* pt_off, const int* voxel_cell, const liso_pillar_cfg* cfg, int batch,
                             const int* cell_to_voxel, const float* weight, const float* bn_out, void* canvas, int out_bf16,
                             float* occupancy, void* stream) {
    return pfn_forward_launch(feat, pt_off, voxel_cell, cfg, batch, cell_to_voxel, weight, bn_out, canvas, out_bf16, occupancy, nullptr,
                              0, false, stream);
}

int liso_pfn_forward_rows(const float* feat, const int* pt_off, const int* voxel_cell, const liso_pillar_cfg* cfg, int batch,
                          const int* cell_to_voxel, const float* weight, const float* bn_out, void* rows, int out_bf16, int row_base,
                          int* cell_to_row, float* occupancy, void* stream) {
    if (!cell_to_row || row_base < 0 || (long)row_base + (long)batch * (cfg ? cfg->max_voxels : 0) >= (1L << 31)) return LISO_EINVAL;
    return pfn_forward_launch(feat, pt_off, voxel_cell, cfg, batch, cell_to_voxel, weight, bn_out, rows, out_bf16, occupancy, cell_to_row,
                              row_base, true, stream);
}

int liso_pfn_backward(const float* feat, const int* pt_off, const int* voxel_cell, const liso_pillar_cfg* cfg, int batch,
                      const int* num_voxels, const float* weight, const float* gamma, const float* bn_out,
                      const double* moments, int training, const void* grad_canvas, int grad_bf16, float* grad_weight,
                      float* grad_gamma, float* grad_beta, void* partials, void* stream) {
    if (!cfg_ok(cfg, batch) || !feat || !pt_off || !voxel_cell || !num_voxels || !weight || !gamma || !bn_out || !grad_canvas ||
        !grad_weight || !grad_gamma || !grad_beta || !partials || (training && !moments))
        return LISO_EINVAL;
    if (grad_bf16 != LISO_ELEM_F32 && grad_bf16 != LISO_ELEM_BF16 && grad_bf16 != LISO_ELEM_F16) return LISO_EINVAL;
    hipStream_t st = (hipStream_t)stream;
    const int rows = batch * cfg->max_voxels;
    const int grid = pfn_grid((rows + kGroup - 1) / kGroup);
#define LISO_BWD(CC, T)                                                                                              \
    do {                                                                                                             \
        constexpr int NA_ = CC + 8;                                                                                  \
        double* tot_ = (double*)((float*)partials + (size_t)kPfnGrid * (11 + 2) * kOut);                             \
        pfn_backward_kernel<CC, T><<<grid, kPfnThreads, 0, st>>>(feat, pt_off, voxel_cell, rows, cfg->max_points,     \
                                                                 weight, bn_out, (const T*)grad_canvas,             \
                                                                 (float*)partials);                                  \
        pfn_backward_reduce_kernel<NA_><<<NA_, 1024, 0, st>>>((const float*)partials, grid, tot_);                    \
        pfn_backward_finalize_kernel<CC><<<1, 64, 0, st>>>(tot_, num_voxels, batch, cfg->max_points, weight, gamma,   \
                                                           bn_out, moments, training, grad_weight, grad_gamma,       \
                                                           grad_beta);                                               \
    } while (0)
    switch (cfg->n_channels * 3 + grad_bf16) {
        case 9: LISO_BWD(3, float); break;
        case 10: LISO_BWD(3, __hip_bfloat16); break;
        case 11: LISO_BWD(3, _Float16); break;
        case 12: LISO_BWD(4, float); break;
        case 13: LISO_BWD(4, __hip_bfloat16); break;
        case 14: LISO_BWD(4, _Float16); break;
        case 15: LISO_BWD(5, float); break;
        case 16: LISO_BWD(5, __hip_bfloat16); break;
        default: LISO_BWD(5, _Float16); break;
    }
#undef LISO_BWD
    return check_launch();
}

}
```

### liso_amd/networks/pcl_to_feature_grid/pcl_to_feature_grid.py

```python
import ctypes

import numpy as np
import torch
from torch import nn

from liso_amd import _lib as L


class PFNLayer(nn.Module):

    def __init__(self, in_channels, out_channels, norm_cfg):
        super().__init__()
        self.units = out_channels
        self.norm = nn.BatchNorm1d(out_channels, eps=norm_cfg["eps"], momentum=norm_cfg["momentum"])
        self.linear = nn.Linear(in_channels, out_channels, bias=False)


class PillarFeatureNet(nn.Module):

    def __init__(self, in_channels, feat_channels, voxel_size, point_cloud_range, norm_cfg):
        super().__init__()
        assert len(feat_channels) == 1, "the LISO call site uses a single PFN layer (pcl_to_feature_grid.py:41-48)"
        self.in_channels = in_channels + 6
        self.pfn_layers = nn.ModuleList([PFNLayer(self.in_channels, feat_channels[0], norm_cfg)])
        self.voxel_size = voxel_size
        self.point_cloud_range = point_cloud_range


def voxelize_raw(points, offsets, pcfg):
    L.require_cuda(points)
    lib = L.lib()
    dev = points.device
    B = len(offsets) - 1
    n_total = int(offsets[-1])
    rows = B * pcfg.max_voxels
    i32 = dict(dtype=torch.int32, device=dev)
    coors = torch.empty((rows, 4), **i32)
    num_points = torch.empty((rows,), **i32)
    slots = torch.empty((rows, pcfg.max_points), **i32)
    num_voxels = torch.empty((B,), **i32)
    cell_to_voxel = torch.empty((B * pcfg.gx * pcfg.gy,), **i32)
    ws_bytes = lib.liso_pillars_voxelize_workspace_bytes(ctypes.byref(pcfg), B, n_total)
    ws = torch.empty(ws_bytes, dtype=torch.uint8, device=dev)
    off = (ctypes.c_int * (B + 1))(*[int(o) for o in offsets])
    with torch.cuda.device(dev):
        L.check(lib.liso_pillars_voxelize_f32(L.ptr(points), off, B, ctypes.byref(pcfg), L.ptr(coors),
                                              L.ptr(num_points), L.ptr(slots), L.ptr(num_voxels),
                                              L.ptr(cell_to_voxel), L.ptr(ws), ws_bytes, L.stream_ptr()),
                "pillars_voxelize")
    return coors, num_points, slots, num_voxels, cell_to_voxel


def decorate_rows(points, pcfg, B, coors, num_points, slots, num_voxels):
    lib = L.lib()
    dev = points.device
    rows = B * pcfg.max_voxels
    pt_off = torch.empty(rows + 1, dtype=torch.int32, device=dev)
    feat = torch.empty((max(points.shape[0], 1), 12), dtype=torch.float32, device=dev)
    voxel_cell = torch.empty(rows, dtype=torch.int32, device=dev)
    nbytes = lib.liso_pfn_decorate_workspace_bytes(B, pcfg.max_voxels)
    ws = torch.empty(nbytes, dtype=torch.uint8, device=dev)
    with torch.cuda.device(dev):
        L.check(L.TIMER.launch("pfn_decorate", lambda: lib.liso_pfn_decorate_f32(
            L.ptr(points), ctypes.byref(pcfg), B, L.ptr(coors), L.ptr(num_points), L.ptr(slots), L.ptr(num_voxels), L.ptr(pt_off),
            L.ptr(feat), L.ptr(voxel_cell), L.ptr(ws), nbytes, L.stream_ptr()), units=points.shape[0] * (points.shape[1] * 4 + 48)), "pfn_decorate")
    return pt_off, feat, voxel_cell


def pillar_prep(points, offsets, pcfg):
    B = len(offsets) - 1
    coors, num_points, slots, num_voxels, cell_to_voxel = voxelize_raw(points, offsets, pcfg)
    pt_off, feat, voxel_cell = decorate_rows(points, pcfg, B, coors, num_points, slots, num_voxels)
    return pt_off, feat, voxel_cell, num_voxels, cell_to_voxel


def _pfn_statistics(weight, gamma, beta, running_mean, running_var, points, offsets, pcfg, training, momentum, eps, prep):
    L.require_cuda(points, weight)
    lib = L.lib()
    dev = points.device
    B = len(offsets) - 1
    if prep is None:
        prep = pillar_prep(points, offsets, pcfg)
    pt_off, feat, _, num_voxels, _ = prep
    weight = weight.contiguous().float()
    with torch.cuda.device(dev):
        bn_out = torch.empty(4 * 64, dtype=torch.float32, device=dev)
        moments = torch.empty(80, dtype=torch.float64, device=dev)
        partials = torch.empty(lib.liso_pfn_partials_bytes(), dtype=torch.uint8, device=dev)
        L.check(lib.liso_pfn_bn_prepare_f32(L.ptr(feat), L.ptr(pt_off), ctypes.byref(pcfg), B, L.ptr(num_voxels),
                                            L.ptr(weight), L.ptr(gamma), L.ptr(beta), L.ptr(running_mean),
                                            L.ptr(running_var), float(momentum), float(eps), int(training),
                                            L.ptr(bn_out), L.ptr(moments), L.ptr(partials), L.stream_ptr()), "pfn_bn_prepare")
    return prep, weight, bn_out, moments


class _PillarFeatureScatter(torch.autograd.Function):

    @staticmethod
    def forward(ctx, weight, gamma, beta, running_mean, running_var, points, offsets, pcfg, training, momentum, eps,
                out_dtype, out=None, prep=None):
        code = L.elem_code(out_dtype)
        lib = L.lib()
        dev = points.device
        B = len(offsets) - 1
        prep, weight, bn_out, moments = _pfn_statistics(weight, gamma, beta, running_mean, running_var, points, offsets, pcfg, training,
                                                        momentum, eps, prep)
        pt_off, feat, voxel_cell, num_voxels, cell_to_voxel = prep
        with torch.cuda.device(dev):
            st = L.stream_ptr()
            if out is not None:
                canvas, occupancy = out
                assert canvas.shape == (B, pcfg.gx, pcfg.gy, 64) and canvas.dtype == out_dtype and canvas.is_contiguous()
                assert occupancy.shape == (B, 1, pcfg.gx, pcfg.gy) and occupancy.is_contiguous()
            else:
                canvas = torch.empty((B, pcfg.gx, pcfg.gy, 64), dtype=out_dtype, device=dev)
                occupancy = torch.empty((B, 1, pcfg.gx, pcfg.gy), dtype=torch.float32, device=dev)
            L.check(L.TIMER.launch("pfn_forward_scatter", lambda: lib.liso_pfn_forward_scatter(
                L.ptr(feat), L.ptr(pt_off), L.ptr(voxel_cell), ctypes.byref(pcfg), B, L.ptr(cell_to_voxel), L.ptr(weight),
                L.ptr(bn_out), L.ptr(canvas), code, L.ptr(occupancy), st),
                units=points.numel() * 4 + canvas.numel() * canvas.element_size() + occupancy.numel() * 4),
                "pfn_forward_scatter")
        ctx.save_for_backward(feat, pt_off, voxel_cell, num_voxels, weight, gamma, bn_out, moments)
        ctx.pcfg, ctx.B, ctx.training = pcfg, B, bool(training)
        ctx.mark_non_differentiable(occupancy)
        return canvas.permute(0, 3, 1, 2), occupancy

    @staticmethod
    def backward(ctx, grad_canvas, _grad_occ):
        feat, pt_off, voxel_cell, num_voxels, weight, gamma, bn_out, moments = ctx.saved_tensors
        lib = L.lib()
        dev = feat.device
        g = grad_canvas.permute(0, 2, 3, 1)
        if g.dtype not in (torch.float32, torch.bfloat16, torch.float16):
            g = g.float()
        g = g.contiguous()
        F = weight.shape[1]
        gw = torch.empty((64, F), dtype=torch.float32, device=dev)
        gg = torch.empty(64, dtype=torch.float32, device=dev)
        gb = torch.empty(64, dtype=torch.float32, device=dev)
        partials = torch.empty(lib.liso_pfn_partials_bytes(), dtype=torch.uint8, device=dev)
        with torch.cuda.device(dev):
            L.check(lib.liso_pfn_backward(L.ptr(feat), L.ptr(pt_off), L.ptr(voxel_cell), ctypes.byref(ctx.pcfg), ctx.B,
                                          L.ptr(num_voxels), L.ptr(weight), L.ptr(gamma), L.ptr(bn_out), L.ptr(moments),
                                          int(ctx.training), L.ptr(g), L.elem_code(g.dtype), L.ptr(gw), L.ptr(gg),
                                          L.ptr(gb), L.ptr(partials), L.stream_ptr()), "pfn_backward")
        return gw, gg, gb, None, None, None, None, None, None, None, None, None, None, None


@torch.no_grad()
def pillar_rows(weight, gamma, beta, running_mean, running_var, points, offsets, pcfg, training, momentum, eps, out_dtype, out=None,
                prep=None):
    from liso_amd.utils.mfma_conv import PillarCanvas

    code = L.elem_code(out_dtype)
    lib = L.lib()
    dev = points.device
    B = len(offsets) - 1
    prep, weight, bn_out, _ = _pfn_statistics(weight, gamma, beta, running_mean, running_var, points, offsets, pcfg, training, momentum,
                                              eps, prep)
    pt_off, feat, voxel_cell, num_voxels, cell_to_voxel = prep
    if out is None:
        out = PillarCanvas.empty(B, (pcfg.gx, pcfg.gy), pcfg.max_voxels, out_dtype, dev)
    R = B * pcfg.max_voxels
    assert tuple(out.shape) == (B, 64, pcfg.gx, pcfg.gy) and out.dtype == out_dtype and out.max_voxels == pcfg.max_voxels
    assert out.row_base + R <= out.rows.shape[0]
    rows = out.rows[out.row_base:out.row_base + R]
    with torch.cuda.device(dev):
        st = L.stream_ptr()
        cells = B * pcfg.gx * pcfg.gy
        L.check(L.TIMER.launch("pfn_forward_scatter", lambda: lib.liso_pfn_forward_rows(
            L.ptr(feat), L.ptr(pt_off), L.ptr(voxel_cell), ctypes.byref(pcfg), B, L.ptr(cell_to_voxel), L.ptr(weight),
            L.ptr(bn_out), L.ptr(rows), code, out.row_base, L.ptr(out.cell_map), L.ptr(out.occupancy), st),
            units=points.numel() * 4 + cells * 12),
            "pfn_forward_rows")
    return out


class PointsPillarFeatureNetWrapper(nn.Module):
    def __init__(self, cfg) -> None:
        super().__init__()
        self.cfg = cfg
        z_cut = cfg.data.setdefault("z_pillar_cutoff_value", 5.0)
        assert z_cut > 0.0, z_cut
        half = np.append(np.array(cfg.data.bev_range_m) / 2.0, z_cut)
        pc_range = np.concatenate([-half, half], axis=0)
        voxel_size = np.append(np.array(cfg.data.bev_range_m) / np.array(cfg.data.img_grid_size), 2 * z_cut)
        self.max_num_points, self.max_voxels = 20, 40000
        if "use_lidar_intensity" in cfg.data:
            num_input_channels = [3, 4][cfg.data.use_lidar_intensity]
        else:
            num_input_channels = 3
        if cfg.data.setdefault("num_point_channels", None):
            num_input_channels = int(cfg.data.num_point_channels)
            assert num_input_channels in (3, 4, 5), num_input_channels
        self.num_input_channels = num_input_channels
        crf = cfg.network.centerpoint.setdefault("channel_reduction_factor", 1)
        assert 64 // crf == 64, "the fused gfx950 PFN kernel is built for 64 output channels"
        self.pts_voxel_encoder = PillarFeatureNet(
            in_channels=num_input_channels, feat_channels=[64 // crf], voxel_size=voxel_size,
            point_cloud_range=pc_range, norm_cfg={"type": "BN1d", "eps": 0.001, "momentum": 0.01})
        self.voxel_size, self.pc_range = voxel_size, pc_range
        self.grid = tuple(int(g) for g in cfg.data.img_grid_size)
        self.out_dtype = torch.float32

    def _pcfg(self, n_channels):
        c = L.PillarCfg()
        c.x_min, c.y_min, c.z_min = (float(np.float32(v)) for v in self.pc_range[:3])
        c.vx, c.vy, c.vz = (float(np.float32(v)) for v in self.voxel_size)
        c.gx, c.gy = self.grid
        c.max_points, c.max_voxels, c.n_channels = self.max_num_points, self.max_voxels, n_channels
        return c

    @staticmethod
    def _cat(points):
        assert isinstance(points, (list, tuple)), type(points)
        offsets = [0]
        for p in points:
            assert p.dim() == 2, p.shape
            offsets.append(offsets[-1] + p.shape[0])
        cat = torch.cat([p.float() for p in points], dim=0).contiguous()
        return cat, offsets

    @torch.no_grad()
    def voxelize(self, points):
        cat, offsets = self._cat(points)
        pcfg = self._pcfg(cat.shape[1])
        return self._compact(cat, pcfg, len(points), voxelize_raw(cat, offsets, pcfg))

    @staticmethod
    def _compact(cat, pcfg, B, vox):
        coors, num_points, slots, num_voxels, _ = vox
        nv = num_voxels.cpu().tolist()
        rows = torch.cat([torch.arange(b * pcfg.max_voxels, b * pcfg.max_voxels + nv[b], device=cat.device)
                          for b in range(B)])
        sl = slots[rows].long()
        valid = torch.arange(pcfg.max_points, device=cat.device)[None, :] < num_points[rows][:, None]
        vox = torch.where(valid[..., None], cat[sl.clamp(min=0, max=max(cat.shape[0] - 1, 0))],
                          torch.zeros((), device=cat.device))
        return vox, num_points[rows], coors[rows]

    @torch.no_grad()
    def prepare(self, pts):
        cat, offsets = self._cat(pts)
        return (cat, offsets, pillar_prep(cat, offsets, self._pcfg(cat.shape[1])))

    def extract_pts_feat(self, pts, out=None, prep=None, compact=False):
        L.elem_code(self.out_dtype)
        if prep is not None:
            cat, offsets, prep = prep
        else:
            cat, offsets = self._cat(pts)
        C = cat.shape[1]
        assert C == self.num_input_channels, (C, self.num_input_channels)
        lyr = self.pts_voxel_encoder.pfn_layers[0]
        training = self.training and lyr.norm.training
        if training and lyr.norm.track_running_stats:
            lyr.norm.num_batches_tracked += 1
        if compact:
            assert not torch.is_grad_enabled(), "the compact canvas has no backward: inference only"
            canvas = pillar_rows(lyr.linear.weight, lyr.norm.weight, lyr.norm.bias, lyr.norm.running_mean, lyr.norm.running_var, cat,
                                 offsets, self._pcfg(C), training, lyr.norm.momentum, lyr.norm.eps, self.out_dtype, out, prep)
            return canvas, canvas.occupancy
        x, occ = _PillarFeatureScatter.apply(lyr.linear.weight, lyr.norm.weight, lyr.norm.bias, lyr.norm.running_mean,
                                             lyr.norm.running_var, cat, offsets, self._pcfg(C), training,
                                             lyr.norm.momentum, lyr.norm.eps, self.out_dtype, out, prep)
        return x, occ

    def forward(self, pcl_t0, img_t0=None, out=None, prep=None, compact=False):
        return self.extract_pts_feat(pcl_t0, out=out, prep=prep, compact=compact)
```

### liso_amd/slim/model/raft_mod.py

```python
import numpy as np
import torch
from torch import nn

from liso_amd.networks.pcl_to_feature_grid.pcl_to_feature_grid import PointsPillarFeatureNetWrapper
from liso_amd.slim.model.extractor import SmallEncoder
from liso_amd.slim.model.raft_code.corr import CorrBlock
from liso_amd.slim.model.deferred_wgrad import deferred_weight_gradients
from liso_amd.slim.model.raft_outputs import raft_network_outputs
from liso_amd.slim.model.raft_code.utils import initialize_flow, upflow_n, uplogits_n
from liso_amd.slim.model.update import SmallUpdateBlock


def move_channel_to_last_dim(tensor):
    return tensor.permute(0, 2, 3, 1)


def change_flow_convention_from_raft2usfl(flow, resolution_adapter):
    return torch.flip(flow, dims=[1]) * resolution_adapter


class RAFT(nn.Module):
    def __init__(self, cfg, head_decoder_fw, head_decoder_bw, **kwargs):
        super().__init__(**kwargs)
        self.cfg = cfg
        self.slim_cfg = cfg.SLIM
        half = 0.5 * np.array(cfg.data.bev_range_m)
        bev_pc_range = np.concatenate([-half, half], axis=0)
        self.head_decoder_fw, self.head_decoder_bw = head_decoder_fw, head_decoder_bw
        self.iters = self.slim_cfg.model.num_iters
        fs = self.slim_cfg.model.u_net.final_scale
        self.bev_rows_res_meters_per_fs_pixel = (bev_pc_range[2] - bev_pc_range[0]) / cfg.data.img_grid_size[0] * fs
        self.bev_cols_res_meters_per_fs_pixel = (bev_pc_range[3] - bev_pc_range[1]) / cfg.data.img_grid_size[1] * fs
        assert self.bev_rows_res_meters_per_fs_pixel == self.bev_cols_res_meters_per_fs_pixel
        self.pp_layer = PointsPillarFeatureNetWrapper(cfg)
        self.hidden_dim, self.context_dim = 96, 64
        assert self.slim_cfg.model.corr_cfg.module == "all" and self.slim_cfg.model.feature_downsampling_factor == 8
        self.fnet = SmallEncoder(output_dim=128, norm_fn=self.slim_cfg.model.raft_fnet_norm,
                                 dropout=self.slim_cfg.model.dropout_rate)
        self.cnet = SmallEncoder(output_dim=self.hidden_dim + self.context_dim, norm_fn="none",
                                 dropout=self.slim_cfg.model.dropout_rate)
        self.update_block = SmallUpdateBlock(cfg=self.slim_cfg, filters=self.hidden_dim)

    def forward(self, pcl_t0, pcl_t1, canvases=None):
        if canvases is not None:
            img_t0, occ_t0, img_t1, occ_t1 = canvases
        else:
            img_t0, occ_t0 = self.pp_layer(pcl_t0)
            img_t1, occ_t1 = self.pp_layer(pcl_t1)
        aux = {"t0": {"bev_net_input_dbg": occ_t0}, "t1": {"bev_net_input_dbg": occ_t1}}
        if not getattr(self, "batch_directions", True):
            o0, o1 = (occ_t0, occ_t1) if img_t0.is_cuda else (None, None)
            fmap_t0, fmap_t1 = self.fnet(img_t0, occupancy=o0), self.fnet(img_t1, occupancy=o1)
            fw = self.predict_single_flow_map_and_classes(img_t0, fmap_t0, fmap_t1, self.head_decoder_fw, occupancy_t0=o0)
            bw = self.predict_single_flow_map_and_classes(img_t1, fmap_t1, fmap_t0, self.head_decoder_bw, occupancy_t0=o1)
            return fw, bw, aux
        B = img_t0.shape[0]
        imgs = torch.cat([img_t0, img_t1], dim=0)
        occ = torch.cat([occ_t0, occ_t1], dim=0) if imgs.is_cuda else None
        fmap = self.fnet(imgs, occupancy=occ)
        fmap_swapped = torch.cat([fmap[B:], fmap[:B]], dim=0)
        both = self.predict_single_flow_map_and_classes(imgs, fmap, fmap_swapped, self.head_decoder_fw,
                                                        fused_dirs=2 if getattr(self, "fused_outputs", True) else None,
                                                        occupancy_t0=occ)
        if torch.is_tensor(both):
            n_it = both.shape[0] // (2 * B)
            aux["net_all"] = both
            return ([both[i * B:(i + 1) * B] for i in range(n_it)],
                    [both[(n_it + i) * B:(n_it + i + 1) * B] for i in range(n_it)], aux)
        aux["fw_bw_batched"] = both
        return [p[:B] for p in both], [p[B:] for p in both], aux

    def compact_canvas_ok(self, device):
        from liso_amd.utils import mfma_conv as MC

        if not MC.compact_canvas() or torch.is_grad_enabled() or torch.device(device).type != "cuda":
            return False
        pp = self.pp_layer
        shape, dtype = (1, 64, *pp.grid), pp.out_dtype
        if dtype != torch.float32:
            return False
        return all(getattr(e, "fold_inference", True) and MC._norm_kind(e.norm1) is not None and MC.sparse_stem_covers(shape, dtype, e.conv1)
                   for e in (self.fnet, self.cnet))

    def encode_pillars(self, pcl_t0, pcl_t1, out=None, compact=False):
        if compact:
            from liso_amd.utils.mfma_conv import PillarCanvas

            B = len(pcl_t0)
            assert len(pcl_t1) == B
            pp = self.pp_layer
            both = out if out is not None else PillarCanvas.empty(2 * B, pp.grid, pp.max_voxels, pp.out_dtype, pcl_t0[0].device)
            assert isinstance(both, PillarCanvas) and both.shape[0] == 2 * B and both.row_base == 0
            a, _ = pp(pcl_t0, out=both[:B], compact=True)
            b, _ = pp(pcl_t1, out=both[B:], compact=True)
            return (a, a.occupancy, b, b.occupancy, both, both.occupancy)
        if out is None:
            return (*self.pp_layer(pcl_t0), *self.pp_layer(pcl_t1))
        rows, occ = out
        B = rows.shape[0] // 2
        a = self.pp_layer(pcl_t0, out=(rows[:B], occ[:B]))
        b = self.pp_layer(pcl_t1, out=(rows[B:], occ[B:]))
        return (*a, *b, rows.permute(0, 3, 1, 2))

    def infer_forward_direction(self, pcl_t0, pcl_t1, canvases=None):
        if canvases is None:
            canvases = self.encode_pillars(pcl_t0, pcl_t1, compact=self.compact_canvas_ok(pcl_t0[0].device))
        img_t0, occ_t0, img_t1, occ_t1 = canvases[:4]
        aux = {"t0": {"bev_net_input_dbg": occ_t0}, "t1": {"bev_net_input_dbg": occ_t1}}
        B = img_t0.shape[0]
        occ_all = canvases[5] if len(canvases) > 5 else (torch.cat([occ_t0, occ_t1], dim=0) if img_t0.is_cuda else None)
        fmap = self.fnet(canvases[4] if len(canvases) > 4 else torch.cat([img_t0, img_t1], dim=0), occupancy=occ_all)
        out = self.predict_single_flow_map_and_classes(img_t0, fmap[:B], fmap[B:], self.head_decoder_fw, only_last=True,
                                                       occupancy_t0=occ_t0)
        return out[-1], aux

    def infer_both_directions(self, pcl_t0, pcl_t1, canvases=None):
        canvases = canvases if canvases is not None else self.encode_pillars(pcl_t0, pcl_t1)
        img_t0, occ_t0, img_t1, occ_t1 = canvases[:4]
        aux = {"t0": {"bev_net_input_dbg": occ_t0}, "t1": {"bev_net_input_dbg": occ_t1}}
        B = img_t0.shape[0]
        imgs = canvases[4] if len(canvases) > 4 else torch.cat([img_t0, img_t1], dim=0)
        occ = (canvases[5] if len(canvases) > 5 else torch.cat([occ_t0, occ_t1], dim=0)) if imgs.is_cuda else None
        fmap = self.fnet(imgs, occupancy=occ)
        out = self.predict_single_flow_map_and_classes(imgs, fmap, torch.cat([fmap[B:], fmap[:B]], dim=0), self.head_decoder_fw,
                                                       only_last=True, occupancy_t0=occ)
        return out[-1][:B], out[-1][B:], aux

    def predict_single_flow_map_and_classes(self, img_t0, fmap_t0, fmap_t1, decoder, only_last=False, fused_dirs=None,
                                            occupancy_t0=None):
        m = self.slim_cfg.model
        assert img_t0.shape[1] == m.point_pillars.nbr_point_feats, img_t0.shape
        ds = m.feature_downsampling_factor
        coords0 = initialize_flow(img_t0, downscale_factor=ds)
        coords1 = initialize_flow(img_t0, downscale_factor=ds)
        b, _, h, w = coords0.shape
        vanilla = m.flow_maps_archi == "vanilla"
        logits = None if vanilla else torch.zeros((b, 4, h, w), dtype=torch.float32, device=img_t0.device)
        use_w = m.predict_weight_for_static_aggregation is not False
        wl = torch.zeros((b, 1, h, w), dtype=torch.float32, device=img_t0.device) if use_w else None
        correlation = CorrBlock(fmap_t0, fmap_t1, num_levels=m.corr_cfg.num_levels, radius=m.corr_cfg.search_radius)
        cnet = self.cnet(img_t0, occupancy=occupancy_t0)
        net, inp = torch.split(cnet, [self.hidden_dim, self.context_dim], dim=1)
        net, inp = torch.tanh(net), torch.relu(inp)
        adapter = float(self.bev_rows_res_meters_per_fs_pixel)
        preds = []
        fuse = (fused_dirs is not None and not vanilla and not use_w and not only_last and img_t0.is_cuda
                and b % fused_dirs == 0)
        lowres_flows, lowres_logits = [], []
        mode = getattr(self, "defer_update_block_wgrad", True)
        infer = self.update_block.inference_state(net, inp) if (only_last and not use_w) else None
        packed = infer is not None and infer["packed"] and not vanilla
        if packed:
            coords0, coords1 = coords0.contiguous(), coords1.contiguous()
        if fuse and infer is None and torch.is_grad_enabled():
            from liso_amd.slim.model import raft_loop as RL
            from liso_amd.slim.model.raft_outputs import _RaftOutputs

            if RL.applicable(self.update_block, net, inp, m.corr_cfg.search_radius):
                flows, logits_all = RL.raft_loop(self.update_block, correlation, coords0, net, inp, m.num_iters, direct=mode == "direct")
                return _RaftOutputs.apply(flows, logits_all, fused_dirs, ds, ds * float(adapter))
        with deferred_weight_gradients(self.update_block, enabled=self.training and bool(mode), direct_accumulate=mode == "direct"):
            for it in range(m.num_iters):
                coords1 = coords1.detach()
                if not vanilla:
                    logits = logits.detach()
                if use_w:
                    wl = wl.detach()
                corr = correlation(coords1)
                if packed:
                    net, both = self.update_block.forward_inference(infer, corr, None, None)
                    logits = self.update_block.state_step(infer, both, coords0, coords1)
                    if it + 1 < m.num_iters:
                        continue
                    logits = logits.contiguous()
                else:
                    flow = coords1 - coords0
                    if infer is not None:
                        net, d_flow, d_logits, d_w = self.update_block.forward_inference(infer, corr, flow, logits)
                    else:
                        net, d_flow, d_logits, d_w = self.update_block(net, inp, corr, flow, logits, wl)
                    coords1 = coords1 + d_flow
                    if not vanilla:
                        logits = logits + d_logits
                    if use_w:
                        wl = wl + d_w
                if only_last and it + 1 < m.num_iters:
                    continue
                if fuse:
                    lowres_flows.append(coords1 - coords0)
                    lowres_logits.append(logits)
                    continue
                if only_last and not vanilla and not use_w and img_t0.is_cuda and not torch.is_grad_enabled():
                    from liso_amd.slim.model.raft_outputs import _RaftOutputs

                    preds.append(_RaftOutputs.apply((coords1 - coords0)[None], logits.contiguous()[None], 1, ds, ds * adapter))
                    continue
                up_flow = change_flow_convention_from_raft2usfl(upflow_n(coords1 - coords0, n=ds), resolution_adapter=adapter)
                if vanilla:
                    up_logits = torch.zeros((b, 4, h * ds, w * ds), dtype=torch.float32, device=img_t0.device)
                else:
                    up_logits = uplogits_n(logits, n=ds)
                up_w = uplogits_n(wl, n=ds) if use_w else None
                preds.append(decoder.concat2network_output(logits=up_logits, static_flow=up_flow, dynamic_flow=up_flow,
                                                           weight_logits_for_static_aggregation=up_w))
        if fuse:
            return raft_network_outputs(lowres_flows, lowres_logits, dirs=fused_dirs, factor=ds, resolution_adapter=adapter)
        return preds
```

### liso_amd/trainer.py

```python
import collections
import contextlib
import ctypes
import os

import torch
import torch.distributed as dist

from liso_amd import _lib as L

from liso_amd.losses.centerpoint_loss import centerpoint_loss, rotation_vec_on_unit_circle
from liso_amd.networks.simple_net.simple_net import BoxLearner
from liso_amd.utils import graph_capture as GC
from liso_amd.utils import tensor_tree as TT


def get_optimizer_scheduler(cfg, box_predictor, total_steps=None, flat=False):
    if flat:
        from liso_amd.utils.flat_adamw import FlatAdamW

        opt = FlatAdamW(box_predictor.parameters(), lr=cfg.optimization.learning_rate, weight_decay=0.01)
    else:
        opt = torch.optim.AdamW(box_predictor.parameters(), lr=cfg.optimization.learning_rate, weight_decay=0.01)
    common = dict(optimizer=opt, max_lr=cfg.optimization.learning_rate, pct_start=0.4, base_momentum=0.85, max_momentum=0.95,
                  div_factor=10.0)
    source = cfg.data.setdefault("train_on_box_source", "gt")
    if source == "gt":
        sched = torch.optim.lr_scheduler.OneCycleLR(total_steps=(total_steps or cfg.optimization.num_training_steps) + 2, **common)
    elif source == "mined":
        assert cfg.optimization.rounds.active, "assuming this"
        rounds = cfg.optimization.rounds
        sched = torch.optim.lr_scheduler.OneCycleLR(
            total_steps=(total_steps or rounds.steps_per_round * rounds.drop_net_weights_every_nth_round) + 2, final_div_factor=10,
            **common)
    else:
        raise NotImplementedError(source)
    return opt, sched


def get_slim_optimizer_scheduler(slim_cfg, params, flat=False):
    from liso_amd.utils.learning_rate import get_polynomial_decay_schedule_with_warmup

    if slim_cfg.optimizer == "rmsprop" and flat:
        from liso_amd.utils.flat_adamw import FlatRMSprop

        opt = FlatRMSprop(list(params), lr=slim_cfg.learning_rate.initial)
    elif slim_cfg.optimizer == "rmsprop":
        opt = torch.optim.RMSprop(params, lr=slim_cfg.learning_rate.initial)
    elif slim_cfg.optimizer == "adam":
        opt = torch.optim.Adam(params, lr=slim_cfg.learning_rate.initial)
    else:
        raise AssertionError("only rmsprop/adam supported")
    sched = get_polynomial_decay_schedule_with_warmup(
        optimizer=opt, num_warmup_steps=slim_cfg.learning_rate.warm_up.step_length,
        num_training_steps=slim_cfg.iterations.train, lr_end=slim_cfg.learning_rate.initial * 0.05)
    return opt, sched


def gather_gradients(device, params, add=False):
    jobs = []
    for p_, flat in params:
        g = p_.grad
        p_.grad = flat
        if g is None or g is flat:
            continue
        if add or g.dtype != torch.float32 or g.stride() != flat.stride() or g.shape != flat.shape:
            flat.add_(g) if add else flat.copy_(g)
            continue
        jobs.append((g, flat))
    if not jobs:
        return []
    n = len(jobs)
    src = (ctypes.c_void_p * n)(*[g.data_ptr() for g, _ in jobs])
    dst = (ctypes.c_void_p * n)(*[f.data_ptr() for _, f in jobs])
    cnt = (ctypes.c_size_t * n)(*[g.numel() for g, _ in jobs])
    with torch.cuda.device(device):
        L.check(L.lib().liso_gather_f32(n, src, dst, cnt, L.stream_ptr()), "gather_f32")
    return [g for g, _ in jobs]


_SIDE_STREAMS = {}


def side_stream(device, role, priority=0):
    key = (device.index if device.index is not None else torch.cuda.current_device(), role)
    if key not in _SIDE_STREAMS:
        _SIDE_STREAMS[key] = (torch.cuda.Stream(device=device, priority=priority), priority)
    st, made_with = _SIDE_STREAMS[key]
    assert priority == made_with, f"side stream {role!r} exists with priority {made_with}, requested with {priority}"
    return st


def _prepare_device(device, exact):
    from liso_amd.utils import mfma_conv as MC

    if exact is not None:
        MC.set_fp32_mode("exact" if exact else "x3")
    if device.type == "cuda":
        MC._sparse_flag(device)


def _broadcast_replicas(net):
    for t in list(net.parameters()) + list(net.buffers()):
        dist.broadcast(t.data, src=0)


@contextlib.contextmanager
def _captured_training_pass(tr, canvases, second_half=False):
    from liso_amd.utils import conv_panels as CP

    if not second_half:
        tr._flat_grad.zero_()
        for c in canvases:
            c.grad = None
        tr._step_table = CP.step_table(tr._pack_jobs, getattr(tr, "_opt_packs", None))
    gathered = tr._gather_params or []
    with CP.step(tr._step_table):
        for p_, _ in gathered:
            p_.grad = None
        try:
            yield
        finally:
            tr._gather_keepalive = gather_gradients(tr.device, gathered, second_half)


class DetectorTrainer:
    def __init__(self, cfg, device, compute_dtype=torch.float32, total_steps=None, fused_loss=None, use_graph=False, exact=None,
                 grad_buckets=None, loss_scale="default"):
        from liso_amd.losses import fused_centerpoint

        self.cfg, self.device = cfg, device
        _prepare_device(device, exact)
        self.use_graph = bool(use_graph) and device.type == "cuda"
        self._graph, self._graph2, self._graph_sig = None, None, None
        self._opt_packs = None
        self.fused_loss = (fused_centerpoint.supports(cfg) and device.type == "cuda") if fused_loss is None else fused_loss
        self.net = BoxLearner(cfg).to(device)
        self.net.model.set_compute_dtype(compute_dtype)
        if self.use_graph and not self.fused_loss:
            from liso_amd.utils.graph_safety import require_node_replay

            require_node_replay("DetectorTrainer(use_graph=True) without the fused loss")
        self.model = self.net
        self.world = dist.get_world_size() if dist.is_available() and dist.is_initialized() else 1
        self.optimizer, self.lr_scheduler = get_optimizer_scheduler(cfg, self.net, total_steps, flat=device.type == "cuda")
        self.loss_scaler = None
        if loss_scale == "default":
            loss_scale = "dynamic" if compute_dtype == torch.float16 else None
        if loss_scale is not None:
            if compute_dtype != torch.float16:
                raise ValueError(f"loss scaling is for fp16 training (compute_dtype {compute_dtype})")
            if device.type != "cuda":
                raise ValueError("fp16 training runs on the device kernels only")
            from liso_amd.utils.loss_scale import DeviceLossScale

            if loss_scale == "dynamic":
                self.loss_scaler = DeviceLossScale(device)
            elif isinstance(loss_scale, (int, float)) and not isinstance(loss_scale, bool):
                self.loss_scaler = DeviceLossScale(device, init_scale=float(loss_scale), dynamic=False)
            else:
                raise ValueError(f"loss_scale: 'dynamic', a number or None, got {loss_scale!r}")
            self.optimizer.loss_scale = self.loss_scaler
        if self.world > 1 and not self.use_graph:
            self.model = torch.nn.parallel.DistributedDataParallel(
                self.net, device_ids=[device.index] if device.type == "cuda" else None, bucket_cap_mb=64,
                broadcast_buffers=False, gradient_as_bucket_view=device.type != "cuda")
        self.n_grad_buckets = 1
        if self.use_graph:
            self._flat_grad = self.optimizer.flat_grad
            if self.world > 1:
                _broadcast_replicas(self.net)
                self.optimizer.grad_scale = 1.0 / self.world
                self._setup_gradient_buckets(grad_buckets)
            elif grad_buckets == 2:
                self._setup_gradient_buckets(2)
        from liso_amd.networks.centerpoint.fused_bn import defer_batch_counters
        self._bn_counters = defer_batch_counters(self.net.model.rpn) + defer_batch_counters(self.net.model.center_head)

    def _setup_gradient_buckets(self, grad_buckets):
        from liso_amd.utils import mfma_conv as MC

        rpn = self.net.model.rpn
        if grad_buckets is None:
            grad_buckets = int(os.environ.get("LISO_GRAD_BUCKETS", "2"))
        if grad_buckets < 2 or len(rpn.blocks) < 2 or not hasattr(self.optimizer, "offsets"):
            return
        first = next(rpn.blocks[1].parameters())
        split = self.optimizer.offsets[id(first)]
        order = [id(p_) for p_ in self.net.parameters() if p_.requires_grad]
        assert all(self.optimizer.offsets[i] < split for i in order[:order.index(id(first))])
        assert all(self.optimizer.offsets[i] >= split for i in order[order.index(id(first)):])
        self._bucket_split = int(split)
        self._grad_cut = MC.GradCut()
        self.n_grad_buckets = 2

    def _reduce_gradients(self, rest_of_backward):
        if getattr(self, "skip_collective", False):
            rest_of_backward()
            return
        if self.n_grad_buckets < 2:
            rest_of_backward()
            dist.all_reduce(self._flat_grad)
            return
        w1 = dist.all_reduce(self._flat_grad[self._bucket_split:], async_op=True)
        rest_of_backward()
        w2 = dist.all_reduce(self._flat_grad[:self._bucket_split], async_op=True)
        w1.wait()
        w2.wait()

    def loss(self, pcls, targets, canvas=None):
        if self.model.training:
            from liso_amd.networks.centerpoint.fused_bn import step_batch_counters
            step_batch_counters(self._bn_counters)
        cfg = self.cfg
        sup = cfg.loss.supervised.supervised_on_clusters
        gt_maps = {a: targets[a] for a in sup.attrs}
        mask = targets["center_bool_mask"]
        if self.fused_loss:
            from liso_amd.losses.fused_centerpoint import fused_centerpoint_loss

            _, _, raw, _ = self.model(None, pcls, None, centermaps_gt=None, decode=False, canvas=canvas)
            total, losses = fused_centerpoint_loss(
                cfg=cfg, raw_box_maps=raw, gt_maps=gt_maps, gt_center_mask=mask,
                ignore_region_is_true_mask=targets.get("ignore_region_is_true_mask", None),
                pillar_center_coors_m=self.net.pillar_center_coors_m)
            return total, losses, None
        pred_boxes, decoded, activated, aux = self.model(None, pcls, None, centermaps_gt=None)
        ignore = targets.get("ignore_region_is_true_mask", torch.zeros_like(mask))
        losses = centerpoint_loss(loss_cfg=cfg.loss, raw_activated_pred_box_maps=activated, decoded_pred_box_maps=decoded,
                                  gt_maps=gt_maps, gt_center_mask=mask,
                                  rotation_loss_weights_map=torch.ones_like(gt_maps["probs"]),
                                  box_prediction_cfg=cfg.box_prediction, ignore_region_is_true_mask=ignore)
        total = 0.0
        for v in losses.values():
            total = total + sup.weight * v
        rr = cfg.box_prediction.rotation_representation
        if rr.method == "vector":
            total = total + rotation_vec_on_unit_circle(activated) * rr.regul_weight
        return total, losses, pred_boxes

    def step(self, pcls, targets, prep=None):
        self.model.train()
        if self.use_graph:
            return self._graph_step(pcls, targets, prep)
        self.optimizer.zero_grad(set_to_none=True)
        total, losses, _ = self.loss(pcls, targets)
        self._backward(total)
        self.optimizer.step()
        self.lr_scheduler.step()
        return total.detach()

    def _backward(self, total):
        if self.loss_scaler is None:
            total.backward()
        else:
            total.backward(self.loss_scaler.seed)

    def loss_scale_stats(self):
        return None if self.loss_scaler is None else self.loss_scaler.stats()

    def eager_pass(self, pcls, targets):
        self.model.train()
        saved = [p.grad for p in self.net.parameters()]
        for p in self.net.parameters():
            p.grad = None
        ctx = self.model.no_sync() if hasattr(self.model, "no_sync") else contextlib.nullcontext()
        with GC.frozen_buffers(self.net, keep=lambda k, v: "running" in k or "num_batches" in k), ctx:
            total, _, _ = self.loss(pcls, targets)
            self._backward(total)
        for p, g in zip(self.net.parameters(), saved):
            p.grad = g
        return total.detach()

    def eval_model(self, val_batches, max_iterations=None, **run_val_args):
        from liso_amd.eval.eval_ours import run_val

        was_training = self.net.training
        self.net.eval()
        try:
            return run_val(self.cfg, val_batches, self.net, max_num_steps=max_iterations, **run_val_args)
        finally:
            self.net.train(was_training)

    def _pillars(self, pcls, out=None, prep=None):
        return self.net.model.pfn(pcl_t0=pcls, img_t0=None, out=out, prep=prep)

    def _capture(self, pcls, targets):
        from liso_amd.utils import mfma_conv as MC

        dev = self.device
        with GC.frozen_buffers(self.net) as restore:
            with torch.no_grad():
                bev, occ = self._pillars(pcls)
            self._static_bev = bev.detach().clone().requires_grad_(True)
            self._static_occ = occ.detach().clone()
            self._static_targets = {k: v.to(dev).clone() for k, v in targets.items()}
            side = side_stream(dev, "flow")
            self._graph2, self._pack_jobs, self._gather_params = None, [], None
            merged_jobs = []
            cut = self._grad_cut if self.n_grad_buckets == 2 else None
            rpn = self.net.model.rpn

            def body(part=None):
                with _captured_training_pass(self, [self._static_bev], second_half=part == 2):
                    MC.set_direct_grads(True, keep_touched=part == 2)
                    try:
                        if part in (None, 1):
                            rpn.grad_cut = cut
                            try:
                                total, _, _ = self.loss(None, self._static_targets, canvas=(self._static_bev, self._static_occ))
                            finally:
                                rpn.grad_cut = None
                            self._backward(total)
                            self._body_loss = total.detach()
                        if cut is not None and part in (None, 2):
                            cut.finish()
                    finally:
                        MC.set_direct_grads(False, keep_touched=True)
                return self._body_loss

            def after_first_pass():
                in_place = MC.direct_touched()
                outside = {id(p_) for p_ in self.net.model.pfn.parameters()}
                self._gather_params = [(p_, p_.grad) for p_ in self.net.parameters()
                                       if p_.requires_grad and p_.grad is not None and id(p_) not in in_place and id(p_) not in outside]

            if self._opt_packs is not None:
                self._opt_packs.ensure_current()
            GC.warm_up(body, side, pack_jobs=self._pack_jobs, merged_jobs=merged_jobs, after_first=after_first_pass, restore=restore)
            self._attach_optimizer_packs(merged_jobs)
            if cut is None:
                self._graph, self._static_loss = GC.capture(body, side)
            else:
                self._graph, self._static_loss = GC.capture(lambda: body(1), side)
                self._graph2, _ = GC.capture(lambda: body(2), side, pool=self._graph.pool())

    def _attach_optimizer_packs(self, merged_jobs):
        from liso_amd.utils import mfma_conv as MC
        from liso_amd.utils.flat_adamw import FlatAdamW

        if self._opt_packs is not None or not MC.optimizer_packs_enabled() or not self._pack_jobs:
            return
        if not isinstance(self.optimizer, FlatAdamW) or self.optimizer.loss_scale is not None:
            return
        from liso_amd.utils.optimizer_packs import OptimizerPacks

        self._opt_packs = OptimizerPacks(self.optimizer, self._pack_jobs, merged_jobs)
        self.optimizer.attach_packs(self._opt_packs)

    def _graph_step(self, pcls, targets, prep=None):
        tsig = targets.shapes() if isinstance(targets, _BatchedTargets) else tuple((k, tuple(v.shape), v.dtype) for k, v in sorted(targets.items()))
        from liso_amd.utils import mfma_conv as MC

        sig = (len(pcls), tsig, MC.optimizer_packs_enabled())
        if self._graph is None or sig != self._graph_sig:
            self._graph = None
            self._capture(pcls, targets)
            self._graph_sig = sig
        bev, occ = self._pillars(pcls, out=(self._static_bev.detach().permute(0, 2, 3, 1), self._static_occ), prep=prep)
        with torch.no_grad():
            stage = []
            if isinstance(targets, _BatchedTargets):
                off = {}
                for t in targets.per_sample:
                    for k, v in t.items():
                        o = off.get(k, 0)
                        stage.append((self._static_targets[k][o:o + v.shape[0]], v))
                        off[k] = o + v.shape[0]
            else:
                for k, v in targets.items():
                    stage.append((self._static_targets[k], v))
            L.multi_copy(stage)
        if self._opt_packs is not None and sig[2]:
            self._opt_packs.ensure_current()
        self._graph.replay()

        def rest_of_backward():
            if self._graph2 is not None:
                self._graph2.replay()
            if bev.requires_grad:
                bev.backward(self._static_bev.grad)

        if self.world > 1:
            self._reduce_gradients(rest_of_backward)
        else:
            rest_of_backward()
        self.optimizer.step()
        self.lr_scheduler.step()
        return self._static_loss.clone()


class SlimTrainer:

    def __init__(self, cfg, device, num_train_samples=1000, use_graph=False, exact=None):
        from liso_amd.slim.model.slim import SLIM

        _prepare_device(device, exact)
        self.cfg, self.slim_cfg, self.device = cfg, cfg.SLIM, device
        self.net = SLIM(cfg, num_train_samples=num_train_samples).to(device)
        self.model = self.net
        self.use_graph = bool(use_graph) and device.type == "cuda"
        self.world = dist.get_world_size() if dist.is_available() and dist.is_initialized() else 1
        if self.world > 1 and not self.use_graph:
            self.model = torch.nn.parallel.DistributedDataParallel(
                self.net, device_ids=[device.index] if device.type == "cuda" else None, bucket_cap_mb=64,
                broadcast_buffers=False, gradient_as_bucket_view=True)
        flat = device.type == "cuda" and self.model is self.net
        self.optimizer, self.lr_scheduler = get_slim_optimizer_scheduler(self.slim_cfg, self.net.parameters(), flat=flat)
        self._flat_opt = hasattr(self.optimizer, "flat_grad")
        import numpy as np
        half = 0.5 * np.array(cfg.data.bev_range_m, dtype=np.float32)
        self.bev_extent = np.concatenate([-half, half], axis=0)
        self._graph, self._graph_sig = None, None
        if self.use_graph:
            from liso_amd.utils.graph_safety import require_node_replay

            require_node_replay("SlimTrainer(use_graph=True)")
            self.net.raft_network.defer_update_block_wgrad = "direct"
            params = [p for p in self.net.parameters() if p.requires_grad]
            if self._flat_opt:
                self._flat_grad = self.optimizer.flat_grad
            else:
                self._flat_grad = torch.zeros(sum(p.numel() for p in params), dtype=torch.float32, device=device)
                off = 0
                for p in params:
                    p.grad = self._flat_grad[off:off + p.numel()].view_as(p)
                    off += p.numel()
            outside = {id(p) for p in self.net.raft_network.pp_layer.parameters()} if hasattr(self.net.raft_network, "pp_layer") else set()
            self._gather_params = [(p, p.grad) for p in params if id(p) not in outside]
            if self.world > 1:
                _broadcast_replicas(self.net)

    def _inputs(self, sample_t0, sample_t1):
        pc1, m1 = sample_t0["pcl_ta"]["pcl"].to(self.device), sample_t0["pcl_ta"]["pcl_is_valid"].to(self.device)
        pc2, m2 = sample_t1["pcl_ta"]["pcl"].to(self.device), sample_t1["pcl_ta"]["pcl_is_valid"].to(self.device)
        return pc1, m1, pc2, m2

    def loss(self, sample_t0, sample_t1, all_valid=None, canvases=None, gather_plan=None):
        from liso_amd.slim.slim_loss.knn_graph import KnnIndex
        from liso_amd.slim.slim_loss.slim_loss_adaptor import selfsupervisedSlimSingleScaleLoss

        pc1, m1, pc2, m2 = self._inputs(sample_t0, sample_t1)
        if all_valid is None:
            all_valid = (bool(m1.all()), bool(m2.all()))
        ext = [float(v) for v in self.bev_extent]
        idx1 = [KnnIndex(pc1[b][:, :3], extent=ext, all_rows_finite=True) for b in range(pc1.shape[0])] if all_valid[0] else None
        idx2 = [KnnIndex(pc2[b][:, :3], extent=ext, all_rows_finite=True) for b in range(pc2.shape[0])] if all_valid[1] else None
        if canvases is None:
            preds_fw, preds_bw = self.model(sample_t0, sample_t1, None)
        else:
            preds_fw, preds_bw = self.model(sample_t0, sample_t1, None, canvases=canvases, gather_plan=gather_plan)
        kw = dict(moving_thresh_module=self.net.moving_dynamicness_threshold, loss_cfg=self.slim_cfg.losses.unsupervised,
                  model_cfg=self.slim_cfg.model, bev_extent=self.bev_extent, metrics_collector={})
        stacked = getattr(self.net, "stacked_predictions", None)
        if stacked is not None and not self.slim_cfg.model.use_static_aggr_flow_for_aggr_flow:
            sfw, sbw, n_it = stacked
            rep = lambda t: t.repeat(n_it, *([1] * (t.dim() - 1)))
            total = n_it * selfsupervisedSlimSingleScaleLoss(
                pc1=rep(pc1), valid_mask_pc1=rep(m1), pc2=rep(pc2), valid_mask_pc2=rep(m2), pred_fw=sfw, pred_bw=sbw,
                knn_index_pc1=None if idx1 is None else idx1 * n_it, knn_index_pc2=None if idx2 is None else idx2 * n_it, **kw)
            return total, preds_fw, preds_bw
        total = torch.zeros(1, device=self.device)
        for pfw, pbw in zip(preds_fw, preds_bw):
            total = total + selfsupervisedSlimSingleScaleLoss(pc1=pc1, valid_mask_pc1=m1, pc2=pc2, valid_mask_pc2=m2, pred_fw=pfw,
                                                              pred_bw=pbw, knn_index_pc1=idx1, knn_index_pc2=idx2, **kw)
        return total, preds_fw, preds_bw

    def step(self, sample_t0, sample_t1, eager=False, update=True):
        self.model.train()
        if self.use_graph and not eager:
            return self._graph_step(sample_t0, sample_t1)
        total, _, _ = self.loss(sample_t0, sample_t1)
        if self.use_graph:
            self._flat_grad.zero_()
        else:
            self.optimizer.zero_grad(set_to_none=True)
        if not update:
            with self.model.no_sync() if hasattr(self.model, "no_sync") else contextlib.nullcontext():
                total.backward()
            return total.detach()
        total.backward()
        self._reduce_and_update()
        return total.detach()

    def eval_model(self, val_batches, max_iterations=None):
        from liso_amd.slim.validation import run_eval_on_this_dataset

        was_training = self.net.training
        self.net.eval()
        try:
            return run_eval_on_this_dataset(self.net, val_batches, max_iterations=max_iterations)
        finally:
            self.net.train(was_training)

    def _reduce_and_update(self):
        if self.use_graph and self.world > 1:
            dist.all_reduce(self._flat_grad)
            self._flat_grad.div_(self.world)
        self.optimizer.step()
        self.lr_scheduler.step()

    def _capture(self, sample_t0, sample_t1, all_valid):
        self._static = TT.tree_map((sample_t0, sample_t1), lambda t: t.to(self.device).clone())
        s0, s1 = self._static
        with GC.frozen_buffers(self.net) as restore:
            with torch.no_grad():
                canv = self._pillars(sample_t0, sample_t1)
            self._static_canv = tuple(c.detach().clone() for c in canv)
            leaves = [self._static_canv[i].requires_grad_(True) for i in (0, 2)]
            self._static_plan = None
            meta = getattr(self.net, "gather_plan_meta", None)
            if meta is None:
                with torch.no_grad():
                    self.net(s0, s1, None, canvases=self._static_canv)
                meta = getattr(self.net, "gather_plan_meta", None)
            if meta is not None:
                self._static_plan = self.net.build_gather_plan(s0, s1, *meta)
                self._static_plan.lin64
            thr = self.net.moving_dynamicness_threshold
            defer = self.world > 1 and bool(self.slim_cfg.model.use_static_aggr_flow_for_aggr_flow)
            self._thr_items = None

            def body():
                with _captured_training_pass(self, leaves):
                    thr._defer = [] if defer else None
                    try:
                        total, _, _ = self.loss(s0, s1, all_valid, canvases=self._static_canv, gather_plan=self._static_plan)
                        total.backward()
                    finally:
                        self._thr_items, thr._defer = thr._defer, None
                return total.detach()

            self._pack_jobs = []
            self._graph, self._static_loss = GC.capture(body, side_stream(self.device, "flow"), warm_ups=2, pack_jobs=self._pack_jobs,
                                                        restore=restore)

    def capture(self, sample_t0, sample_t1):
        _, m1, _, m2 = self._inputs(sample_t0, sample_t1)
        all_valid = (bool(m1.all()), bool(m2.all()))
        sig = (TT.tree_signature((sample_t0, sample_t1)), all_valid)
        if self._graph is None or sig != self._graph_sig:
            self._graph = None
            self._capture(sample_t0, sample_t1, all_valid)
            self._graph_sig = sig
            return True
        return False

    def _pillars(self, sample_t0, sample_t1):
        from liso_amd.slim.model.slim import get_network_input_pcls

        dev = self.device
        return self.net.raft_network.encode_pillars(get_network_input_pcls(self.cfg, sample_t0, "ta", to_device=dev),
                                                    get_network_input_pcls(self.cfg, sample_t1, "ta", to_device=dev))

    def _graph_step(self, sample_t0, sample_t1):
        if not self.capture(sample_t0, sample_t1):
            TT.tree_copy_(self._static, (sample_t0, sample_t1))
        canv = self._pillars(sample_t0, sample_t1)
        with torch.no_grad():
            for d, c in zip(self._static_canv, canv):
                d.copy_(c.detach(), non_blocking=True)
            if self._static_plan is not None:
                fresh = self.net.build_gather_plan(sample_t0, sample_t1, *self.net.gather_plan_meta)
                for name in ("lin", "sorted_lin", "order", "seg_rank"):
                    getattr(self._static_plan, name).copy_(getattr(fresh, name), non_blocking=True)
                self._static_plan.lin64.copy_(fresh.lin, non_blocking=True)
        self._graph.replay()
        if self._thr_items:
            with torch.no_grad():
                self.net.moving_dynamicness_threshold.apply_deferred(self._thr_items)
        live = [(canv[i], self._static_canv[i].grad) for i in (0, 2) if canv[i].requires_grad]
        if live:
            torch.autograd.backward([c for c, _ in live], [g for _, g in live])
        self._reduce_and_update()
        return self._static_loss.clone()


class _Prefetched:
    __slots__ = ("pair", "flow", "done", "targets", "boxes", "cluster_count")

    def __init__(self, pair, flow, done, targets=None, boxes=None, cluster_count=None):
        self.pair, self.flow, self.done = pair, flow, done
        self.targets, self.boxes, self.cluster_count = targets, boxes, cluster_count

    def is_for(self, pair):
        return self.pair[0] is pair[0] and self.pair[1] is pair[1]


class _BatchedTargets(dict):

    def __init__(self, per_sample):
        super().__init__()
        self.per_sample = list(per_sample)
        for k in self.per_sample[0]:
            dict.__setitem__(self, k, None)

    def __getitem__(self, k):
        v = dict.__getitem__(self, k)
        if v is None:
            v = torch.cat([t[k] for t in self.per_sample], dim=0)
            dict.__setitem__(self, k, v)
        return v

    def get(self, k, default=None):
        return self[k] if k in self else default

    def items(self):
        return [(k, self[k]) for k in self.keys()]

    def values(self):
        return [self[k] for k in self.keys()]

    def shapes(self):
        rows = {k: sum(t[k].shape[0] for t in self.per_sample) for k in self.per_sample[0]}
        return tuple((k, (rows[k],) + tuple(v.shape[1:]), v.dtype) for k, v in sorted(self.per_sample[0].items()))


class LisoLoopTrainer:

    def __init__(self, cfg, device, compute_dtype=torch.float32, total_steps=None, slim_state_dict=None, use_graph=False,
                 overlap=False, infer_batch=2, flow_ahead=0, exact=None):
        from liso_amd.networks.flow_cluster_detector.flow_cluster_detector import FlowClusterDetector
        from liso_amd.slim.model.slim import SLIM

        self.cfg, self.device = cfg, device
        _prepare_device(device, exact)
        self.use_graph = bool(use_graph) and device.type == "cuda"
        self._graph_infer = self.use_graph and use_graph in (True, "infer")
        self._graph_det = self.use_graph and use_graph in (True, "detector")
        self._graph_mine = self.use_graph and use_graph is True
        sync = lambda: torch.cuda.synchronize(device)
        self._infer_graphs, self._mine_graphs = GC.GraphLRU(sync), GC.GraphLRU(sync)
        tcfg = cfg.data.tracking_cfg
        self.infer_point_bucket = int(tcfg.setdefault("infer_point_bucket", 8192))
        self.max_infer_graphs = int(tcfg.setdefault("max_infer_graphs", 8))
        self.max_mine_graphs = int(tcfg.setdefault("max_mine_graphs", 6))
        self.mine_capture_budget = int(tcfg.setdefault("mine_capture_budget", 24))
        self.mine_capture_window = int(tcfg.setdefault("mine_capture_window", 400))
        self.mine_captures, self.mine_eager_fallbacks = 0, 0
        self._mine_calls, self._mine_capture_calls, self._mine_fallback_warned = 0, [], False
        self._views = collections.OrderedDict()
        self.overlap = bool(overlap) and device.type == "cuda"
        self.infer_batch, self.flow_ahead = int(infer_batch), int(flow_ahead)
        self.box_capacity, self.capacity_overflows = int(cfg.data.tracking_cfg.setdefault("flow_cluster_capacity", 64)), 0
        self._flow_stream, self._mine_stream, self._main_used_static = None, None, None
        self._inputs_ready = None
        self._flows, self._mined = [], []
        self.slim = SLIM(cfg, num_train_samples=1000).to(device)
        if slim_state_dict is not None:
            self.slim.load_state_dict(slim_state_dict)
        self.slim.eval()
        for p_ in self.slim.parameters():
            p_.requires_grad_(False)
        self.cluster_detector = FlowClusterDetector(cfg).to(device)
        self.detector = DetectorTrainer(cfg, device, compute_dtype=compute_dtype, total_steps=total_steps, use_graph=self._graph_det)
        if device.type == "cuda":
            self._flow_stream = side_stream(device, "flow")
            self._mine_stream = side_stream(device, "mine0", priority=-1)
            n_mine = max(1, int(os.environ.get("LISO_MINE_STREAMS", "1")))
            self._mine_streams = [self._mine_stream] + [side_stream(device, f"mine{k}", priority=-1) for k in range(1, n_mine)]
            self._mine_turn = 0
        self.infer_cus = 0
        if device.type == "cuda" and self.overlap:
            n_cu = torch.cuda.get_device_properties(device).multi_processor_count
            self.infer_cus = int(os.environ.get("LISO_INFER_CUS", str(n_cu // 2)))
            if self.infer_cus >= n_cu:
                self.infer_cus = 0
        self._pillar_prep = None
        self._prep_ahead = os.environ.get("LISO_PREP_AHEAD", "1") != "0"
        self.pre_nms, self.post_nms = tcfg.max_num_boxes_before_nms, tcfg.max_num_boxes_after_nms
        self.nms_iou = cfg.setdefault("nms_iou_threshold", 0.1)

    @torch.no_grad()
    def mine_boxes(self, sample_t0, sample_t1):
        flow = self._infer_flow(sample_t0, sample_t1)
        _, boxes = self._targets_from_flow(sample_t0, flow)
        return boxes, flow

    _stack_samples = staticmethod(TT.tree_stack)

    def _pad_loss_cloud(self, sample):
        pa, bk = sample["pcl_ta"], self.infer_point_bucket
        n = pa["pcl"].shape[1]
        pad = (-n) % bk if bk > 1 else 0
        full = sample.get("pcl_full_w_ground_ta")
        fpad = (-full.shape[1]) % bk if (bk > 1 and torch.is_tensor(full) and full.dim() == 3) else 0
        if pad == 0 and fpad == 0:
            return sample
        out = {**sample, "pcl_ta": TT.pad_pcl_ta(pa, n + pad)}
        if fpad:
            out["pcl_full_w_ground_ta"] = torch.nn.functional.pad(full, (0, 0, 0, fpad), value=float("nan"))
        return out

    def _view(self, sample):
        cuda = self.device.type == "cuda"
        cur = torch.cuda.current_stream(self.device) if cuda else None
        hit = self._views.get(id(sample))
        if hit is not None and hit[0] is sample:
            self._views.move_to_end(id(sample))
            _, v, ev, made_on, seen = hit
            if cuda and ev is not None and cur.cuda_stream != made_on and cur.cuda_stream not in seen:
                cur.wait_event(ev)
                for t in self._padded_tensors(sample, v):
                    t.record_stream(cur)
                seen.add(cur.cuda_stream)
            return v
        v = self._pad_loss_cloud(sample)
        ev = None
        if cuda and v is not sample:
            ev = torch.cuda.Event()
            ev.record(cur)
        self._views[id(sample)] = (sample, v, ev, cur.cuda_stream if cuda else None, set())
        while len(self._views) > 64:
            self._views.popitem(last=False)
        return v

    @staticmethod
    def _padded_tensors(sample, view):
        out = []
        if view["pcl_ta"] is not sample["pcl_ta"]:
            out += [view["pcl_ta"][k] for k in ("pcl", "pcl_is_valid", "pillar_coors")]
        if view.get("pcl_full_w_ground_ta") is not sample.get("pcl_full_w_ground_ta"):
            out.append(view["pcl_full_w_ground_ta"])
        return out

    def _infer_view(self, sample):
        v = self._view(sample)
        key = "pcl_full_w_ground_ta" if self.cfg.data.use_ground_for_network else "pcl_full_no_ground_ta"
        return {"pcl_ta": v["pcl_ta"], "gt": {"odom_ta_tb": v["gt"]["odom_ta_tb"]}, key: list(sample[key])}

    def _infer_flow(self, sample_t0, sample_t1):
        n_true = sample_t0["pcl_ta"]["pcl"].shape[1]
        flow = self._infer_flow_padded(self._infer_view(sample_t0), self._infer_view(sample_t1))
        return flow if flow.shape[1] == n_true else flow[:, :n_true].contiguous()

    @staticmethod
    def _graph_inputs(sample_t0, sample_t1):
        return tuple({"pcl_ta": s_["pcl_ta"], "gt": {"odom_ta_tb": s_["gt"]["odom_ta_tb"]}} for s_ in (sample_t0, sample_t1))

    def _infer_flow_padded(self, sample_t0, sample_t1):
        if not self._graph_infer:
            return self.slim.infer_point_flow_t0_t1(sample_t0, sample_t1)
        from liso_amd.slim.model.slim import get_network_input_pcls
        from liso_amd.utils import mfma_conv as MC

        dev = self.device
        ins = self._graph_inputs(sample_t0, sample_t1)
        sig = TT.tree_signature(ins)
        raft = self.slim.raft_network
        pcls = (get_network_input_pcls(self.cfg, sample_t0, "ta", to_device=dev), get_network_input_pcls(self.cfg, sample_t1, "ta", to_device=dev))
        st = self._infer_graphs.lookup(sig)
        with torch.no_grad():
            compact = raft.compact_canvas_ok(dev) if st is None else st["compact"]
            if st is None:
                canv = raft.encode_pillars(*pcls, compact=compact)
            else:
                raft.encode_pillars(*pcls, out=st["rows"], compact=compact)
            thr = self.slim.moving_dynamicness_threshold.value()
        if st is None:
            st = self._infer_graphs.insert(sig, {}, self.max_infer_graphs)
            st["in"] = TT.tree_map(ins, lambda t: t.to(dev).clone())
            B_ = canv[0].shape[0]
            st["compact"] = compact
            if compact:
                st["rows"], st["canv"] = canv[4], canv
            else:
                rows = torch.cat([canv[0], canv[2]], dim=0).permute(0, 2, 3, 1).contiguous()
                occ = torch.cat([canv[1], canv[3]], dim=0).contiguous()
                st["rows"] = (rows, occ)
                st["canv"] = (rows[:B_].permute(0, 3, 1, 2), occ[:B_], rows[B_:].permute(0, 3, 1, 2), occ[B_:], rows.permute(0, 3, 1, 2), occ)
            st["thr"] = thr.clone()
            s0, s1 = st["in"]
            with torch.no_grad(), MC.roles_cus(self.infer_cus):
                st["graph"], st["flow"] = GC.capture(
                    lambda: self.slim.infer_point_flow_t0_t1(s0, s1, canvases=st["canv"], dynamicness_threshold=st["thr"]),
                    self._flow_stream, warm_ups=2)
        else:
            TT.tree_copy_(st["in"], ins)
            st["thr"].copy_(thr, non_blocking=True)
        st["graph"].replay()
        return st["flow"]

    def eager_pass(self, sample_t0, sample_t1, also=()):
        return self.eager_pass_batch([(sample_t0, sample_t1)], also)

    def eager_pass_batch(self, pairs, also=()):
        with self._shared_gpu():
            return self._eager_pass_batch(pairs, also)

    def _shared_gpu(self):
        from liso_amd.utils import mfma_conv as MC

        return MC.shared_gpu() if self.device.type == "cuda" else contextlib.nullcontext()

    def _eager_pass_batch(self, pairs, also=()):
        from liso_amd.utils import mfma_conv as MC

        g, self._graph_infer = self._graph_infer, False
        try:
            allp = [*pairs, *also]
            with torch.no_grad():
                L.TIMER.weight = len(pairs) / len(allp)
                try:
                    with MC.roles_cus(self.infer_cus):
                        flow = self._infer_flow_padded(self._stack_infer_views([p_[0] for p_ in allp]), self._stack_infer_views([p_[1] for p_ in allp]))
                finally:
                    L.TIMER.weight = 1.0
                b = flow.shape[0] // len(allp)
                per = [self._targets_from_flow(p_[0], flow[k * b:(k + 1) * b].contiguous())[0] for k, p_ in enumerate(pairs)]
        finally:
            self._graph_infer = g
        targets = per[0] if len(per) == 1 else {k: torch.cat([t[k] for t in per], dim=0) for k in per[0]}
        return self.detector.eager_pass([c for p_ in pairs for c in p_[0]["pcl_full_no_ground_ta"]], targets)

    def _mine_from_graph(self, sample_t0, flow, side):
        from liso_amd.kabsch.shape_utils import Shape

        dev = self.device
        v = self._view(sample_t0)
        pa = v["pcl_ta"]
        gt = v[self.cfg.data.odom_source]
        flow = self._pad_flow(flow, pa["pcl"].shape[1])
        ins = {"pcl": pa["pcl"], "valid": pa["pcl_is_valid"], "coors": pa["pillar_coors"], "full": v["pcl_full_w_ground_ta"],
               "flow": flow, "dt": v["src_trgt_time_delta_s"], "odom": gt["odom_ta_tb"]}
        ins = {k: (t if t.device == dev else t.to(dev, non_blocking=True)) for k, t in ins.items()}
        sig = (side.cuda_stream,) + tuple((k, tuple(t.shape), t.dtype) for k, t in ins.items())
        st = self._mine_graphs.lookup(sig)
        self._mine_calls += 1
        while self._mine_capture_calls and self._mine_capture_calls[0] <= self._mine_calls - self.mine_capture_window:
            self._mine_capture_calls.pop(0)
        if st is None and len(self._mine_capture_calls) >= self.mine_capture_budget:
            self.mine_eager_fallbacks += 1
            if not self._mine_fallback_warned:
                self._mine_fallback_warned = True
                import warnings
                warnings.warn(f"LisoLoopTrainer: {self.mine_capture_budget} box-mining graph captures within {self.mine_capture_window} "
                              "calls -- new point-count signatures run stage B eagerly until the rate drops (raise "
                              "infer_point_bucket or max_mine_graphs)")
            targets, boxes = self._targets_from_flow(sample_t0, flow, capacity=self.box_capacity)
            return targets, boxes, self.cluster_detector.last_num_labels.max().reshape(1)
        if st is not None:
            if st["in_flat"] is not None:
                TT.pack_into(st["in_flat"], st["in_layout"], ins)
            else:
                for k, t in ins.items():
                    st["in"][k].copy_(t, non_blocking=True)
        else:
            st = self._mine_graphs.insert(sig, {}, self.max_mine_graphs)
            self.mine_captures += 1
            self._mine_capture_calls.append(self._mine_calls)
            si, st["in_flat"], st["in_layout"] = TT.packed_statics(ins)
            st["in"] = si
            sample = {"pcl_ta": {"pcl": si["pcl"], "pcl_is_valid": si["valid"], "pillar_coors": si["coors"]},
                      "pcl_full_w_ground_ta": si["full"], "src_trgt_time_delta_s": si["dt"],
                      self.cfg.data.odom_source: {"odom_ta_tb": si["odom"]}}

            def body():
                targets, boxes = self._targets_from_flow(sample, si["flow"], capacity=self.box_capacity, padded=True)
                return TT.pack([("t_" + k, t) for k, t in targets.items()] +
                               [("b_" + k, t) for k, t in boxes.__dict__.items() if torch.is_tensor(t)] +
                               [("n_clusters", self.cluster_detector.last_num_labels.max().reshape(1))])

            with torch.no_grad():
                st["graph"], (st["flat"], st["layout"]) = GC.capture(body, side, warm_ups=2)
        st["graph"].replay()
        out = TT.unpack(st["flat"].clone(), st["layout"])
        targets = {k[2:]: t for k, t in out.items() if k.startswith("t_")}
        boxes = Shape(**{k[2:]: t for k, t in out.items() if k.startswith("b_")})
        return targets, boxes, out["n_clusters"]

    @staticmethod
    def _pad_flow(flow, n):
        if flow.shape[1] == n:
            return flow
        if flow.shape[1] > n:
            return flow[:, :n].contiguous()
        return torch.nn.functional.pad(flow, (0, 0, 0, n - flow.shape[1]))

    def _targets_from_flow(self, sample_t0, flow, capacity=None, odom_minus_eye=None, padded=False):
        from liso_amd.datasets.targets import render_center_targets
        from liso_amd.utils.nms_iou import perform_nms_on_shapes_padded

        with torch.no_grad():
            if not padded:
                sample_t0 = self._view(sample_t0)
            flow = self._pad_flow(flow, sample_t0["pcl_ta"]["pcl"].shape[1])
            sample = dict(sample_t0)
            sample[self.cfg.data.flow_source] = {**sample_t0.get(self.cfg.data.flow_source, {}), "flow_ta_tb": flow}
            boxes = self.cluster_detector(sample, global_step=1, capacity=capacity, odom_minus_eye=odom_minus_eye)
            B = boxes.shape[0]
            if boxes.shape[1] > 0:
                boxes, (pos, dims, rot, valid) = perform_nms_on_shapes_padded(
                    boxes, max_num_boxes=self.post_nms, overlap_threshold=self.nms_iou, pre_nms_max_num_boxes=self.pre_nms,
                    return_target_arrays=True)
                rot = rot[..., None]
            else:
                z = torch.zeros((B, 1, 3), device=self.device)
                pos, dims, rot, valid = z, z + 1.0, z[..., :1], torch.zeros((B, 1), dtype=torch.bool, device=self.device)
            out = tuple(int(g) // 4 for g in self.cfg.data.img_grid_size)
            return render_center_targets(pos, dims, rot, valid, out, tuple(self.cfg.data.bev_range_m)), boxes

    def _stage_a(self, *pairs):
        side = self._flow_stream
        if self._inputs_ready is not None:
            side.wait_event(self._inputs_ready)
        if self._main_used_static is not None:
            side.wait_event(self._main_used_static)
            self._main_used_static = None
        with torch.cuda.stream(side), torch.no_grad():
            if len(pairs) == 1:
                flows = [self._infer_flow_padded(self._infer_view(pairs[0][0]), self._infer_view(pairs[0][1])).clone()]
            else:
                flow = self._infer_flow_padded(self._stack_infer_views([p_[0] for p_ in pairs]), self._stack_infer_views([p_[1] for p_ in pairs]))
                b = flow.shape[0] // len(pairs)
                flows = [flow[k * b:(k + 1) * b].clone() for k in range(len(pairs))]
            done = torch.cuda.Event()
            done.record(side)
        for p_, fl in zip(pairs, flows):
            self._flows.append(_Prefetched(pair=p_, flow=fl, done=done))

    def _same_shapes(self, pa, pb):
        sig = lambda pair: TT.tree_signature(self._graph_inputs(self._infer_view(pair[0]), self._infer_view(pair[1])), skip_dim=1)
        return sig(pa) == sig(pb)

    def _stack_infer_views(self, samples):
        views = [self._infer_view(s_) for s_ in samples]
        n = max(v["pcl_ta"]["pcl"].shape[1] for v in views)
        return self._stack_samples([self._grow_view(v, n) for v in views])

    @staticmethod
    def _grow_view(view, n):
        return {**view, "pcl_ta": TT.pad_pcl_ta(view["pcl_ta"], n)}

    @staticmethod
    def _take(store, pair):
        for k, e in enumerate(store):
            if e.is_for(pair):
                return store.pop(k)
        return None

    def _stage_b(self, pair):
        f = self._take(self._flows, pair)
        if f is None:
            self._stage_a(pair)
            f = self._take(self._flows, pair)
        side = self._mine_streams[self._mine_turn % len(self._mine_streams)]
        self._mine_turn += 1
        side.wait_event(f.done)
        if self._inputs_ready is not None:
            side.wait_event(self._inputs_ready)
        with torch.cuda.stream(side):
            f.flow.record_stream(side)
            count = torch.empty(1, dtype=torch.int64, pin_memory=True)
            if self._graph_mine:
                targets, boxes, n_clusters = self._mine_from_graph(pair[0], f.flow, side)
                count.copy_(n_clusters, non_blocking=True)
            else:
                targets, boxes = self._targets_from_flow(pair[0], f.flow, capacity=self.box_capacity)
                count.copy_(self.cluster_detector.last_num_labels.max().reshape(1), non_blocking=True)
            done = torch.cuda.Event()
            done.record(side)
        self._mined.append(_Prefetched(pair=pair, flow=f.flow, done=done, targets=targets, boxes=boxes, cluster_count=count))

    def _take_mined(self, pair, cur):
        m = self._take(self._mined, pair)
        if m is None:
            return None
        if os.environ.get("LISO_NO_COUNT_WAIT") == "1":
            cur.wait_event(m.done)
            for t in list(m.targets.values()) + [v for v in m.boxes.__dict__.values() if torch.is_tensor(v)]:
                t.record_stream(cur)
            return m.targets, m.boxes
        m.done.synchronize()
        cur.wait_event(m.done)
        if int(m.cluster_count[0]) > self.box_capacity:
            m.flow.record_stream(cur)
            self.capacity_overflows += 1
            return self._targets_from_flow(pair[0], m.flow)
        for t in list(m.targets.values()) + [v for v in m.boxes.__dict__.values() if torch.is_tensor(v)]:
            t.record_stream(cur)
        return m.targets, m.boxes

    def step(self, sample_t0, sample_t1, upcoming=()):
        return self.step_batch([(sample_t0, sample_t1)], upcoming)

    def step_batch(self, pairs, upcoming=(), inputs_ready=None):
        with self._shared_gpu():
            return self._step_batch(pairs, upcoming, inputs_ready)

    def _step_batch(self, pairs, upcoming=(), inputs_ready=None):
        cuda = self.device.type == "cuda"
        cur = torch.cuda.current_stream(self.device) if cuda else None
        if cuda:
            self._inputs_ready = inputs_ready
            if inputs_ready is not None:
                cur.wait_event(inputs_ready)
        mined = []
        for pair in pairs:
            sample_t0, sample_t1 = pair
            got = self._take_mined(pair, cur) if cuda else None
            if got is None:
                f = self._take(self._flows, pair)
                if f is not None:
                    cur.wait_event(f.done)
                    f.flow.record_stream(cur)
                    flow = f.flow
                else:
                    if self.overlap and cuda:
                        cur.wait_stream(self._flow_stream)
                    with torch.no_grad():
                        flow = self._infer_flow_padded(self._infer_view(sample_t0), self._infer_view(sample_t1))
                got = self._targets_from_flow(sample_t0, flow)
                if self.overlap and f is None:
                    self._main_used_static = torch.cuda.Event()
                    self._main_used_static.record(cur)
            mined.append(got)
        self.last_boxes = mined[-1][1]
        self.last_boxes_batch = [m[1] for m in mined]
        nb = len(pairs)
        if nb == 1:
            targets = mined[0][0]
        else:
            targets = _BatchedTargets([m[0] for m in mined])
        pcls = [c for p_ in pairs for c in p_[0]["pcl_full_no_ground_ta"]]
        prep = None
        if self.overlap and cuda and self._pillar_prep is not None:
            key, got_prep, done = self._pillar_prep
            self._pillar_prep = None
            if len(key) == len(pcls) and all(a is b_ for a, b_ in zip(key, pcls)):
                cur.wait_event(done)
                cat, _, parts = got_prep
                for t in (cat, *parts):
                    t.record_stream(cur)
                prep = got_prep
        loss = self.detector.step(pcls, targets, prep=prep) if prep is not None else self.detector.step(pcls, targets)
        if self.overlap and cuda and len(upcoming) >= len(pairs) and self._prep_ahead and self.detector.use_graph:
            nxt = [c for p_ in upcoming[:len(pairs)] for c in p_[0]["pcl_full_no_ground_ta"]]
            side = self._mine_stream
            if self._inputs_ready is not None:
                side.wait_event(self._inputs_ready)
            with torch.cuda.stream(side):
                got_prep = self.detector.net.model.pfn.prepare(nxt)
                done = torch.cuda.Event()
                done.record(side)
            self._pillar_prep = (nxt, got_prep, done)
        if self.overlap and len(upcoming) > 0:
            ahead = nb * (1 + len(self._mine_streams))
            fa = nb * self.flow_ahead
            up = list(upcoming[:ahead + fa + self.infer_batch - 1])
            has = lambda store, p: any(e.is_for(p) for e in store)
            self._mined = [e for e in self._mined if any(e.is_for(q) for q in up)]
            self._flows = [e for e in self._flows if any(e.is_for(q) for q in up)]
            missing = [p_ for k, p_ in enumerate(up) if not has(self._flows, p_) and not has(self._mined, p_)
                       and not any(p_[0] is q[0] and p_[1] is q[1] for q in up[:k])]
            if missing and any(p_ is q for p_ in missing for q in up[:ahead + fa]):
                while missing:
                    n = 1
                    while n < min(len(missing), self.infer_batch) and self._same_shapes(missing[0], missing[n]):
                        n += 1
                    self._stage_a(*missing[:n])
                    missing = missing[n:]
            for p_ in up[:ahead]:
                if not has(self._mined, p_):
                    self._stage_b(p_)
        return loss
```

Measured before the change: 1052.

## Share flow-inference pillar voxelisation with detector step via sub-batch PFN entry points

Result: faster. 1069 (median of 6 runs) (+1.6%).

```diff
diff --git a/include/liso_pillars.h b/include/liso_pillars.h
--- a/include/liso_pillars.h
+++ b/include/liso_pillars.h
@@ -51,6 +51,21 @@
                       const double* moments, int training, const void* grad_canvas, int grad_bf16, float* grad_weight,
                       float* grad_gamma, float* grad_beta, void* partials, void* stream);
 
+int liso_pfn_bn_prepare_sub_f32(const float* feat, const int* pt_off, const liso_pillar_cfg* cfg, int sample0, int batch,
+                                const int* num_voxels, const float* weight, const float* gamma, const float* beta,
+                                float* running_mean, float* running_var, float momentum, float eps, int training, float* bn_out,
+                                double* moments, void* partials, void* stream);
+int liso_pfn_forward_scatter_sub(const float* feat, const int* pt_off, const int* voxel_cell, const liso_pillar_cfg* cfg, int sample0,
+                                 int batch, const int* cell_to_voxel, const float* weight, const float* bn_out, void* canvas,
+                                 int out_bf16, float* occupancy, void* stream);
+int liso_pfn_forward_rows_sub(const float* feat, const int* pt_off, const int* voxel_cell, const liso_pillar_cfg* cfg, int sample0,
+                              int batch, const int* cell_to_voxel, const float* weight, const float* bn_out, void* rows, int out_bf16,
+                              int row_base, int* cell_to_row, float* occupancy, void* stream);
+int liso_pfn_backward_sub(const float* feat, const int* pt_off, const int* voxel_cell, const liso_pillar_cfg* cfg, int sample0,
+                          int batch, const int* num_voxels, const float* weight, const float* gamma, const float* bn_out,
+                          const double* moments, int training, const void* grad_canvas, int grad_bf16, float* grad_weight,
+                          float* grad_gamma, float* grad_beta, void* partials, void* stream);
+
 #ifdef __cplusplus
 }
 #endif
diff --git a/liso_amd/_lib.py b/liso_amd/_lib.py
--- a/liso_amd/_lib.py
+++ b/liso_amd/_lib.py
@@ -130,6 +130,10 @@
     "liso_pfn_forward_scatter": (_i, [_vp, _vp, _vp, _vp, _i, _vp, _vp, _vp, _vp, _i, _vp, _vp]),
     "liso_pfn_forward_rows": (_i, [_vp, _vp, _vp, _vp, _i, _vp, _vp, _vp, _vp, _i, _i, _vp, _vp, _vp]),
     "liso_pfn_backward": (_i, [_vp, _vp, _vp, _vp, _i, _vp, _vp, _vp, _vp, _vp, _i, _vp, _i, _vp, _vp, _vp, _vp, _vp]),
+    "liso_pfn_bn_prepare_sub_f32": (_i, [_vp, _vp, _vp, _i, _i, _vp, _vp, _vp, _vp, _vp, _vp, _f, _f, _i, _vp, _vp, _vp, _vp]),
+    "liso_pfn_forward_scatter_sub": (_i, [_vp, _vp, _vp, _vp, _i, _i, _vp, _vp, _vp, _vp, _i, _vp, _vp]),
+    "liso_pfn_forward_rows_sub": (_i, [_vp, _vp, _vp, _vp, _i, _i, _vp, _vp, _vp, _vp, _i, _i, _vp, _vp, _vp]),
+    "liso_pfn_backward_sub": (_i, [_vp, _vp, _vp, _vp, _i, _i, _vp, _vp, _vp, _vp, _vp, _i, _vp, _i, _vp, _vp, _vp, _vp, _vp]),
     "liso_kabsch_workspace_bytes": (_sz, [_vp]),
     "liso_kabsch_trafos_f32": (_i, [_vp, _vp, _vp, _vp, _vp, _vp, _vp, _vp, _vp, _vp, _vp, _sz, _vp]),
     "liso_kabsch_trafos_counted_f32": (_i, [_vp, _vp, _vp, _vp, _vp, _vp, _vp, _vp, _vp, _vp, _vp, _vp, _sz, _vp]),
@@ -481,6 +485,9 @@
                 ("gy", _i), ("max_points", _i), ("max_voxels", _i), ("n_channels", _i)]
 
 
+PILLARS_MAX_BATCH = 32
+
+
 class _Everything:
     def __contains__(self, name):
         return True
diff --git a/liso_amd/csrc/pillars.hip b/liso_amd/csrc/pillars.hip
--- a/liso_amd/csrc/pillars.hip
+++ b/liso_amd/csrc/pillars.hip
@@ -390,7 +390,9 @@
                 if (idx == lane + 64) { pj[1] = j; pk[1] = k; }
             }
     }
-    const long n = pt_off[rows];
+    const long p0 = pt_off[0];
+    const long n = pt_off[rows] - p0;
+    feat += (size_t)p0 * kFP;
     const long waves = (long)gridDim.x * (kPfnThreads / 64);
     const long per = ((n + waves - 1) / waves + 63) / 64 * 64;
     const long w_id = (long)blockIdx.x * (kPfnThreads / 64) + wave;
@@ -546,7 +548,7 @@
                                                                   const int* __restrict__ cell_to_voxel,
                                                                   const float* __restrict__ weight, const float* __restrict__ bn,
                                                                   OutT* __restrict__ canvas, float* __restrict__ occupancy,
-                                                                  int* __restrict__ map_out, int row_base) {
+                                                                  int* __restrict__ map_out, int row_base, long cell_base) {
     constexpr int F = C + 6;
     constexpr int kChunks = kOut * (int)sizeof(OutT) / 16;
     __shared__ __attribute__((aligned(16))) float frow[kPfnThreads / 64][kStage][kFP];
@@ -602,7 +604,7 @@
                 for (int k = 0; k < F; k++) x = fmaf(w[k], f[k], x);
                 best = fmaxf(best, fmaxf(fmaf(x, scale, shift), 0.f));
             }
-            store_out<OutT>(canvas + (size_t)(ROWS ? v0 + g : cell) * kOut + lane, best);
+            store_out<OutT>(canvas + (size_t)(ROWS ? v0 + g : cell - cell_base) * kOut + lane, best);
         }
         __builtin_amdgcn_wave_barrier();
     }
@@ -612,7 +614,7 @@
 __global__ __launch_bounds__(kPfnThreads) void pfn_backward_kernel(const float* __restrict__ feat, const int* __restrict__ pt_off,
                                                                    const int* __restrict__ voxel_cell, int rows, int max_points,
                                                                    const float* __restrict__ weight, const float* __restrict__ bn,
-                                                                   const GT* __restrict__ grad_canvas,
+                                                                   const GT* __restrict__ grad_canvas, long cell_base,
                                                                    float* __restrict__ partials) {
     constexpr int F = C + 6, NA = F + 2;
     __shared__ __attribute__((aligned(16))) float frow[kPfnThreads / 64][kStage][kFP];
@@ -650,7 +652,7 @@
                 if (y > best) { best = y; best_s = s; best_x = x; }
             }
             if (num < max_points && pad_val > best) { best = pad_val; best_s = -1; best_x = 0.f; }
-            const float gy = load_in<GT>(grad_canvas + (size_t)cell * kOut + lane);
+            const float gy = load_in<GT>(grad_canvas + (size_t)(cell - cell_base) * kOut + lane);
             const float dz = best > 0.f ? gy : 0.f;
             if (best_s >= 0) {
                 const float* f = frow[wave][r0 + best_s];
@@ -744,6 +746,11 @@
 inline bool cfg_ok(const liso_pillar_cfg* c, int batch) {
     return c && batch >= 1 && batch <= LISO_PILLARS_MAX_BATCH && c->gx > 0 && c->gy > 0 && c->max_points >= 1 &&
            c->max_points <= kMaxPts && c->max_voxels >= 1 && c->n_channels >= 3 && c->n_channels <= 5;
+}
+
+inline bool sub_ok(const liso_pillar_cfg* c, int sample0, int batch) {
+    return cfg_ok(c, batch) && sample0 >= 0 && sample0 <= LISO_PILLARS_MAX_BATCH - batch &&
+           (long)(sample0 + batch) * c->max_voxels < (1L << 31);
 }
 
 inline BatchInfo make_batch(const int* off, int batch) {
@@ -854,11 +861,11 @@
     return check_launch();
 }
 
-int liso_pfn_bn_prepare_f32(const float* feat, const int* pt_off, const liso_pillar_cfg* cfg, int batch, const int* num_voxels,
-                            const float* weight, const float* gamma, const float* beta, float* running_mean,
-                            float* running_var, float momentum, float eps, int training, float* bn_out, double* moments,
-                            void* partials, void* stream) {
-    if (!cfg_ok(cfg, batch) || !gamma || !beta || !running_mean || !running_var || !bn_out) return LISO_EINVAL;
+int liso_pfn_bn_prepare_sub_f32(const float* feat, const int* pt_off, const liso_pillar_cfg* cfg, int sample0, int batch,
+                                const int* num_voxels, const float* weight, const float* gamma, const float* beta,
+                                float* running_mean, float* running_var, float momentum, float eps, int training, float* bn_out,
+                                double* moments, void* partials, void* stream) {
+    if (!sub_ok(cfg, sample0, batch) || !gamma || !beta || !running_mean || !running_var || !bn_out) return LISO_EINVAL;
     hipStream_t st = (hipStream_t)stream;
     if (!training) {
         pfn_bn_eval_kernel<<<1, 64, 0, st>>>(gamma, beta, running_mean, running_var, eps, bn_out);
@@ -867,6 +874,8 @@
     if (!feat || !pt_off || !num_voxels || !weight || !moments || !partials) return LISO_EINVAL;
     const int rows = batch * cfg->max_voxels;
     const int grid = kPfnGrid;
+    pt_off += (size_t)sample0 * cfg->max_voxels;
+    num_voxels += sample0;
 #define LISO_PREP(CC)                                                                                                     \
     do {                                                                                                                  \
         pfn_stats_kernel<CC><<<grid, kPfnThreads, 0, st>>>(feat, pt_off, rows, (double*)partials);                           \
@@ -883,21 +892,34 @@
     return check_launch();
 }
 
-static int pfn_forward_launch(const float* feat, const int* pt_off, const int* voxel_cell, const liso_pillar_cfg* cfg, int batch,
-                              const int* cell_to_voxel, const float* weight, const float* bn_out, void* canvas, int out_bf16,
+int liso_pfn_bn_prepare_f32(const float* feat, const int* pt_off, const liso_pillar_cfg* cfg, int batch, const int* num_voxels,
+                            const float* weight, const float* gamma, const float* beta, float* running_mean,
+                            float* running_var, float momentum, float eps, int training, float* bn_out, double* moments,
+                            void* partials, void* stream) {
+    return liso_pfn_bn_prepare_sub_f32(feat, pt_off, cfg, 0, batch, num_voxels, weight, gamma, beta, running_mean, running_var, momentum,
+                                       eps, training, bn_out, moments, partials, stream);
+}
+
+static int pfn_forward_launch(const float* feat, const int* pt_off, const int* voxel_cell, const liso_pillar_cfg* cfg, int sample0,
+                              int batch, const int* cell_to_voxel, const float* weight, const float* bn_out, void* canvas, int out_bf16,
                               float* occupancy, int* map_out, int row_base, bool compact, void* stream) {
-    if (!cfg_ok(cfg, batch) || !feat || !pt_off || !voxel_cell || !cell_to_voxel || !weight || !bn_out || !canvas || !occupancy)
+    if (!sub_ok(cfg, sample0, batch) || !feat || !pt_off || !voxel_cell || !cell_to_voxel || !weight || !bn_out || !canvas || !occupancy)
         return LISO_EINVAL;
     if (out_bf16 != LISO_ELEM_F32 && out_bf16 != LISO_ELEM_BF16 && out_bf16 != LISO_ELEM_F16) return LISO_EINVAL;
     hipStream_t st = (hipStream_t)stream;
     const long cells = (long)batch * cfg->gx * cfg->gy;
     const int rows = batch * cfg->max_voxels;
+    const long cell_base = (long)sample0 * cfg->gx * cfg->gy;
+    pt_off += (size_t)sample0 * cfg->max_voxels;
+    voxel_cell += (size_t)sample0 * cfg->max_voxels;
+    cell_to_voxel += cell_base;
+    row_base -= sample0 * cfg->max_voxels;
     const int zero_blocks = (int)((cells + kCellsPerBlock - 1) / kCellsPerBlock);
     const int groups = (rows + kGroup - 1) / kGroup;
     int pfn_blocks = (groups + kPfnThreads / 64 - 1) / (kPfnThreads / 64);
     if (pfn_blocks > 4096) pfn_blocks = 4096;
     const unsigned grid = (unsigned)(zero_blocks + pfn_blocks);
-#define LISO_FWD_(CC, T, R) pfn_forward_kernel<CC, T, R><<<grid, kPfnThreads, 0, st>>>(feat, pt_off, voxel_cell, rows, cfg->max_points, cells, zero_blocks, cell_to_voxel, weight, bn_out, (T*)canvas, occupancy, map_out, row_base)
+#define LISO_FWD_(CC, T, R) pfn_forward_kernel<CC, T, R><<<grid, kPfnThreads, 0, st>>>(feat, pt_off, voxel_cell, rows, cfg->max_points, cells, zero_blocks, cell_to_voxel, weight, bn_out, (T*)canvas, occupancy, map_out, row_base, cell_base)
 #define LISO_FWD(CC, T) do { if (compact) LISO_FWD_(CC, T, true); else LISO_FWD_(CC, T, false); } while (0)
     switch (cfg->n_channels * 3 + out_bf16) {
         case 9: LISO_FWD(3, float); break;
@@ -915,38 +937,56 @@
     return check_launch();
 }
 
+int liso_pfn_forward_scatter_sub(const float* feat, const int* pt_off, const int* voxel_cell, const liso_pillar_cfg* cfg, int sample0,
+                                 int batch, const int* cell_to_voxel, const float* weight, const float* bn_out, void* canvas,
+                                 int out_bf16, float* occupancy, void* stream) {
+    return pfn_forward_launch(feat, pt_off, voxel_cell, cfg, sample0, batch, cell_to_voxel, weight, bn_out, canvas, out_bf16, occupancy,
+                              nullptr, 0, false, stream);
+}
+
 int liso_pfn_forward_scatter(const float* feat, const int* pt_off, const int* voxel_cell, const liso_pillar_cfg* cfg, int batch,
                              const int* cell_to_voxel, const float* weight, const float* bn_out, void* canvas, int out_bf16,
                              float* occupancy, void* stream) {
-    return pfn_forward_launch(feat, pt_off, voxel_cell, cfg, batch, cell_to_voxel, weight, bn_out, canvas, out_bf16, occupancy, nullptr,
-                              0, false, stream);
+    return liso_pfn_forward_scatter_sub(feat, pt_off, voxel_cell, cfg, 0, batch, cell_to_voxel, weight, bn_out, canvas, out_bf16,
+                                        occupancy, stream);
+}
+
+int liso_pfn_forward_rows_sub(const float* feat, const int* pt_off, const int* voxel_cell, const liso_pillar_cfg* cfg, int sample0,
+                              int batch, const int* cell_to_voxel, const float* weight, const float* bn_out, void* rows, int out_bf16,
+                              int row_base, int* cell_to_row, float* occupancy, void* stream) {
+    if (!cell_to_row || row_base < 0 || (long)row_base + (long)batch * (cfg ? cfg->max_voxels : 0) >= (1L << 31)) return LISO_EINVAL;
+    return pfn_forward_launch(feat, pt_off, voxel_cell, cfg, sample0, batch, cell_to_voxel, weight, bn_out, rows, out_bf16, occupancy,
+                              cell_to_row, row_base, true, stream);
 }
 
 int liso_pfn_forward_rows(const float* feat, const int* pt_off, const int* voxel_cell, const liso_pillar_cfg* cfg, int batch,
                           const int* cell_to_voxel, const float* weight, const float* bn_out, void* rows, int out_bf16, int row_base,
                           int* cell_to_row, float* occupancy, void* stream) {
-    if (!cell_to_row || row_base < 0 || (long)row_base + (long)batch * (cfg ? cfg->max_voxels : 0) >= (1L << 31)) return LISO_EINVAL;
-    return pfn_forward_launch(feat, pt_off, voxel_cell, cfg, batch, cell_to_voxel, weight, bn_out, rows, out_bf16, occupancy, cell_to_row,
-                              row_base, true, stream);
-}
-
-int liso_pfn_backward(const float* feat, const int* pt_off, const int* voxel_cell, const liso_pillar_cfg* cfg, int batch,
-                      const int* num_voxels, const float* weight, const float* gamma, const float* bn_out,
-                      const double* moments, int training, const void* grad_canvas, int grad_bf16, float* grad_weight,
-                      float* grad_gamma, float* grad_beta, void* partials, void* stream) {
-    if (!cfg_ok(cfg, batch) || !feat || !pt_off || !voxel_cell || !num_voxels || !weight || !gamma || !bn_out || !grad_canvas ||
+    return liso_pfn_forward_rows_sub(feat, pt_off, voxel_cell, cfg, 0, batch, cell_to_voxel, weight, bn_out, rows, out_bf16, row_base,
+                                     cell_to_row, occupancy, stream);
+}
+
+int liso_pfn_backward_sub(const float* feat, const int* pt_off, const int* voxel_cell, const liso_pillar_cfg* cfg, int sample0,
+                          int batch, const int* num_voxels, const float* weight, const float* gamma, const float* bn_out,
+                          const double* moments, int training, const void* grad_canvas, int grad_bf16, float* grad_weight,
+                          float* grad_gamma, float* grad_beta, void* partials, void* stream) {
+    if (!sub_ok(cfg, sample0, batch) || !feat || !pt_off || !voxel_cell || !num_voxels || !weight || !gamma || !bn_out || !grad_canvas ||
         !grad_weight || !grad_gamma || !grad_beta || !partials || (training && !moments))
         return LISO_EINVAL;
     if (grad_bf16 != LISO_ELEM_F32 && grad_bf16 != LISO_ELEM_BF16 && grad_bf16 != LISO_ELEM_F16) return LISO_EINVAL;
     hipStream_t st = (hipStream_t)stream;
     const int rows = batch * cfg->max_voxels;
     const int grid = pfn_grid((rows + kGroup - 1) / kGroup);
+    const long cell_base = (long)sample0 * cfg->gx * cfg->gy;
+    pt_off += (size_t)sample0 * cfg->max_voxels;
+    voxel_cell += (size_t)sample0 * cfg->max_voxels;
+    num_voxels += sample0;
 #define LISO_BWD(CC, T)                                                                                              \
     do {                                                                                                             \
         constexpr int NA_ = CC + 8;                                                                                  \
         double* tot_ = (double*)((float*)partials + (size_t)kPfnGrid * (11 + 2) * kOut);                             \
         pfn_backward_kernel<CC, T><<<grid, kPfnThreads, 0, st>>>(feat, pt_off, voxel_cell, rows, cfg->max_points,     \
-                                                                 weight, bn_out, (const T*)grad_canvas,             \
+                                                                 weight, bn_out, (const T*)grad_canvas, cell_base,  \
                                                                  (float*)partials);                                  \
         pfn_backward_reduce_kernel<NA_><<<NA_, 1024, 0, st>>>((const float*)partials, grid, tot_);                    \
         pfn_backward_finalize_kernel<CC><<<1, 64, 0, st>>>(tot_, num_voxels, batch, cfg->max_points, weight, gamma,   \
@@ -968,4 +1008,12 @@
     return check_launch();
 }
 
-}
+int liso_pfn_backward(const float* feat, const int* pt_off, const int* voxel_cell, const liso_pillar_cfg* cfg, int batch,
+                      const int* num_voxels, const float* weight, const float* gamma, const float* bn_out,
+                      const double* moments, int training, const void* grad_canvas, int grad_bf16, float* grad_weight,
+                      float* grad_gamma, float* grad_beta, void* partials, void* stream) {
+    return liso_pfn_backward_sub(feat, pt_off, voxel_cell, cfg, 0, batch, num_voxels, weight, gamma, bn_out, moments, training,
+                                 grad_canvas, grad_bf16, grad_weight, grad_gamma, grad_beta, partials, stream);
+}
+
+}
diff --git a/liso_amd/networks/pcl_to_feature_grid/pcl_to_feature_grid.py b/liso_amd/networks/pcl_to_feature_grid/pcl_to_feature_grid.py
--- a/liso_amd/networks/pcl_to_feature_grid/pcl_to_feature_grid.py
+++ b/liso_amd/networks/pcl_to_feature_grid/pcl_to_feature_grid.py
@@ -74,12 +74,19 @@
     return pt_off, feat, voxel_cell, num_voxels, cell_to_voxel
 
 
-def _pfn_statistics(weight, gamma, beta, running_mean, running_var, points, offsets, pcfg, training, momentum, eps, prep):
+def _is_sub_range(prep, sample0, B):
+    total = prep[3].shape[0]
+    assert 0 <= sample0 and sample0 + B <= total, (sample0, B, total)
+    return sample0 != 0 or total != B
+
+
+def _pfn_statistics(weight, gamma, beta, running_mean, running_var, points, offsets, pcfg, training, momentum, eps, prep, sample0=0):
     L.require_cuda(points, weight)
     lib = L.lib()
     dev = points.device
     B = len(offsets) - 1
     if prep is None:
+        assert sample0 == 0, sample0
         prep = pillar_prep(points, offsets, pcfg)
     pt_off, feat, _, num_voxels, _ = prep
     weight = weight.contiguous().float()
@@ -87,10 +94,12 @@
         bn_out = torch.empty(4 * 64, dtype=torch.float32, device=dev)
         moments = torch.empty(80, dtype=torch.float64, device=dev)
         partials = torch.empty(lib.liso_pfn_partials_bytes(), dtype=torch.uint8, device=dev)
-        L.check(lib.liso_pfn_bn_prepare_f32(L.ptr(feat), L.ptr(pt_off), ctypes.byref(pcfg), B, L.ptr(num_voxels),
-                                            L.ptr(weight), L.ptr(gamma), L.ptr(beta), L.ptr(running_mean),
-                                            L.ptr(running_var), float(momentum), float(eps), int(training),
-                                            L.ptr(bn_out), L.ptr(moments), L.ptr(partials), L.stream_ptr()), "pfn_bn_prepare")
+        tail = (L.ptr(num_voxels), L.ptr(weight), L.ptr(gamma), L.ptr(beta), L.ptr(running_mean), L.ptr(running_var), float(momentum),
+                float(eps), int(training), L.ptr(bn_out), L.ptr(moments), L.ptr(partials), L.stream_ptr())
+        if _is_sub_range(prep, sample0, B):
+            L.check(lib.liso_pfn_bn_prepare_sub_f32(L.ptr(feat), L.ptr(pt_off), ctypes.byref(pcfg), sample0, B, *tail), "pfn_bn_prepare_sub")
+        else:
+            L.check(lib.liso_pfn_bn_prepare_f32(L.ptr(feat), L.ptr(pt_off), ctypes.byref(pcfg), B, *tail), "pfn_bn_prepare")
     return prep, weight, bn_out, moments
 
 
@@ -98,14 +107,15 @@
 
     @staticmethod
     def forward(ctx, weight, gamma, beta, running_mean, running_var, points, offsets, pcfg, training, momentum, eps,
-                out_dtype, out=None, prep=None):
+                out_dtype, out=None, prep=None, sample0=0):
         code = L.elem_code(out_dtype)
         lib = L.lib()
         dev = points.device
         B = len(offsets) - 1
         prep, weight, bn_out, moments = _pfn_statistics(weight, gamma, beta, running_mean, running_var, points, offsets, pcfg, training,
-                                                        momentum, eps, prep)
+                                                        momentum, eps, prep, sample0)
         pt_off, feat, voxel_cell, num_voxels, cell_to_voxel = prep
+        sub = _is_sub_range(prep, sample0, B)
         with torch.cuda.device(dev):
             st = L.stream_ptr()
             if out is not None:
@@ -115,13 +125,14 @@
             else:
                 canvas = torch.empty((B, pcfg.gx, pcfg.gy, 64), dtype=out_dtype, device=dev)
                 occupancy = torch.empty((B, 1, pcfg.gx, pcfg.gy), dtype=torch.float32, device=dev)
-            L.check(L.TIMER.launch("pfn_forward_scatter", lambda: lib.liso_pfn_forward_scatter(
-                L.ptr(feat), L.ptr(pt_off), L.ptr(voxel_cell), ctypes.byref(pcfg), B, L.ptr(cell_to_voxel), L.ptr(weight),
-                L.ptr(bn_out), L.ptr(canvas), code, L.ptr(occupancy), st),
-                units=points.numel() * 4 + canvas.numel() * canvas.element_size() + occupancy.numel() * 4),
+            head = (L.ptr(feat), L.ptr(pt_off), L.ptr(voxel_cell), ctypes.byref(pcfg))
+            tail = (L.ptr(cell_to_voxel), L.ptr(weight), L.ptr(bn_out), L.ptr(canvas), code, L.ptr(occupancy), st)
+            L.check(L.TIMER.launch("pfn_forward_scatter", lambda: (lib.liso_pfn_forward_scatter_sub(*head, sample0, B, *tail) if sub
+                                                                   else lib.liso_pfn_forward_scatter(*head, B, *tail)),
+                units=(offsets[-1] - offsets[0]) * points.shape[1] * 4 + canvas.numel() * canvas.element_size() + occupancy.numel() * 4),
                 "pfn_forward_scatter")
         ctx.save_for_backward(feat, pt_off, voxel_cell, num_voxels, weight, gamma, bn_out, moments)
-        ctx.pcfg, ctx.B, ctx.training = pcfg, B, bool(training)
+        ctx.pcfg, ctx.B, ctx.training, ctx.sample0, ctx.sub = pcfg, B, bool(training), sample0, sub
         ctx.mark_non_differentiable(occupancy)
         return canvas.permute(0, 3, 1, 2), occupancy
 
@@ -140,16 +151,19 @@
         gb = torch.empty(64, dtype=torch.float32, device=dev)
         partials = torch.empty(lib.liso_pfn_partials_bytes(), dtype=torch.uint8, device=dev)
         with torch.cuda.device(dev):
-            L.check(lib.liso_pfn_backward(L.ptr(feat), L.ptr(pt_off), L.ptr(voxel_cell), ctypes.byref(ctx.pcfg), ctx.B,
-                                          L.ptr(num_voxels), L.ptr(weight), L.ptr(gamma), L.ptr(bn_out), L.ptr(moments),
-                                          int(ctx.training), L.ptr(g), L.elem_code(g.dtype), L.ptr(gw), L.ptr(gg),
-                                          L.ptr(gb), L.ptr(partials), L.stream_ptr()), "pfn_backward")
-        return gw, gg, gb, None, None, None, None, None, None, None, None, None, None, None
+            head = (L.ptr(feat), L.ptr(pt_off), L.ptr(voxel_cell), ctypes.byref(ctx.pcfg))
+            tail = (L.ptr(num_voxels), L.ptr(weight), L.ptr(gamma), L.ptr(bn_out), L.ptr(moments), int(ctx.training), L.ptr(g),
+                    L.elem_code(g.dtype), L.ptr(gw), L.ptr(gg), L.ptr(gb), L.ptr(partials), L.stream_ptr())
+            if ctx.sub:
+                L.check(lib.liso_pfn_backward_sub(*head, ctx.sample0, ctx.B, *tail), "pfn_backward_sub")
+            else:
+                L.check(lib.liso_pfn_backward(*head, ctx.B, *tail), "pfn_backward")
+        return gw, gg, gb, None, None, None, None, None, None, None, None, None, None, None, None
 
 
 @torch.no_grad()
 def pillar_rows(weight, gamma, beta, running_mean, running_var, points, offsets, pcfg, training, momentum, eps, out_dtype, out=None,
-                prep=None):
+                prep=None, sample0=0):
     from liso_amd.utils.mfma_conv import PillarCanvas
 
     code = L.elem_code(out_dtype)
@@ -157,8 +171,9 @@
     dev = points.device
     B = len(offsets) - 1
     prep, weight, bn_out, _ = _pfn_statistics(weight, gamma, beta, running_mean, running_var, points, offsets, pcfg, training, momentum,
-                                              eps, prep)
+                                              eps, prep, sample0)
     pt_off, feat, voxel_cell, num_voxels, cell_to_voxel = prep
+    sub = _is_sub_range(prep, sample0, B)
     if out is None:
         out = PillarCanvas.empty(B, (pcfg.gx, pcfg.gy), pcfg.max_voxels, out_dtype, dev)
     R = B * pcfg.max_voxels
@@ -168,10 +183,12 @@
     with torch.cuda.device(dev):
         st = L.stream_ptr()
         cells = B * pcfg.gx * pcfg.gy
-        L.check(L.TIMER.launch("pfn_forward_scatter", lambda: lib.liso_pfn_forward_rows(
-            L.ptr(feat), L.ptr(pt_off), L.ptr(voxel_cell), ctypes.byref(pcfg), B, L.ptr(cell_to_voxel), L.ptr(weight),
-            L.ptr(bn_out), L.ptr(rows), code, out.row_base, L.ptr(out.cell_map), L.ptr(out.occupancy), st),
-            units=points.numel() * 4 + cells * 12),
+        head = (L.ptr(feat), L.ptr(pt_off), L.ptr(voxel_cell), ctypes.byref(pcfg))
+        tail = (L.ptr(cell_to_voxel), L.ptr(weight), L.ptr(bn_out), L.ptr(rows), code, out.row_base, L.ptr(out.cell_map),
+                L.ptr(out.occupancy), st)
+        L.check(L.TIMER.launch("pfn_forward_scatter", lambda: (lib.liso_pfn_forward_rows_sub(*head, sample0, B, *tail) if sub
+                                                               else lib.liso_pfn_forward_rows(*head, B, *tail)),
+            units=(offsets[-1] - offsets[0]) * points.shape[1] * 4 + cells * 12),
             "pfn_forward_rows")
     return out
 
@@ -246,7 +263,12 @@
 
     def extract_pts_feat(self, pts, out=None, prep=None, compact=False):
         L.elem_code(self.out_dtype)
-        if prep is not None:
+        sample0 = 0
+        if prep is not None and len(prep) == 5:
+            cat, offsets, prep, sample0, batch = prep
+            assert 0 <= sample0 and sample0 + batch < len(offsets), (sample0, batch, len(offsets))
+            offsets = offsets[sample0:sample0 + batch + 1]
+        elif prep is not None:
             cat, offsets, prep = prep
         else:
             cat, offsets = self._cat(pts)
@@ -259,11 +281,11 @@
         if compact:
             assert not torch.is_grad_enabled(), "the compact canvas has no backward: inference only"
             canvas = pillar_rows(lyr.linear.weight, lyr.norm.weight, lyr.norm.bias, lyr.norm.running_mean, lyr.norm.running_var, cat,
-                                 offsets, self._pcfg(C), training, lyr.norm.momentum, lyr.norm.eps, self.out_dtype, out, prep)
+                                 offsets, self._pcfg(C), training, lyr.norm.momentum, lyr.norm.eps, self.out_dtype, out, prep, sample0)
             return canvas, canvas.occupancy
         x, occ = _PillarFeatureScatter.apply(lyr.linear.weight, lyr.norm.weight, lyr.norm.bias, lyr.norm.running_mean,
                                              lyr.norm.running_var, cat, offsets, self._pcfg(C), training,
-                                             lyr.norm.momentum, lyr.norm.eps, self.out_dtype, out, prep)
+                                             lyr.norm.momentum, lyr.norm.eps, self.out_dtype, out, prep, sample0)
         return x, occ
 
     def forward(self, pcl_t0, img_t0=None, out=None, prep=None, compact=False):
diff --git a/liso_amd/slim/model/raft_mod.py b/liso_amd/slim/model/raft_mod.py
--- a/liso_amd/slim/model/raft_mod.py
+++ b/liso_amd/slim/model/raft_mod.py
@@ -82,24 +82,47 @@
         return all(getattr(e, "fold_inference", True) and MC._norm_kind(e.norm1) is not None and MC.sparse_stem_covers(shape, dtype, e.conv1)
                    for e in (self.fnet, self.cnet))
 
-    def encode_pillars(self, pcl_t0, pcl_t1, out=None, compact=False):
+    encode_once = True
+
+    def encodes_once(self, n_pairs):
+        from liso_amd import _lib as L
+
+        pp = self.pp_layer
+        norm = pp.pts_voxel_encoder.pfn_layers[0].norm
+        if not self.encode_once or torch.is_grad_enabled() or (pp.training and norm.training):
+            return False
+        return 2 * n_pairs <= L.PILLARS_MAX_BATCH and 2 * n_pairs * pp.grid[0] * pp.grid[1] <= 4096 * 1024
+
+    def encode_pillars(self, pcl_t0, pcl_t1, out=None, compact=False, prep=None):
+        B = len(pcl_t0)
+        assert len(pcl_t1) == B
+        pp = self.pp_layer
+        once = self.encodes_once(B) and pcl_t0[0].is_cuda
+        assert prep is None or once, "a prepared voxelisation of both sweeps needs the one-call form"
         if compact:
             from liso_amd.utils.mfma_conv import PillarCanvas
 
-            B = len(pcl_t0)
-            assert len(pcl_t1) == B
-            pp = self.pp_layer
             both = out if out is not None else PillarCanvas.empty(2 * B, pp.grid, pp.max_voxels, pp.out_dtype, pcl_t0[0].device)
             assert isinstance(both, PillarCanvas) and both.shape[0] == 2 * B and both.row_base == 0
-            a, _ = pp(pcl_t0, out=both[:B], compact=True)
-            b, _ = pp(pcl_t1, out=both[B:], compact=True)
+            if once:
+                pp([*pcl_t0, *pcl_t1], out=both, prep=prep, compact=True)
+                a, b = both[:B], both[B:]
+            else:
+                a, _ = pp(pcl_t0, out=both[:B], compact=True)
+                b, _ = pp(pcl_t1, out=both[B:], compact=True)
             return (a, a.occupancy, b, b.occupancy, both, both.occupancy)
         if out is None:
-            return (*self.pp_layer(pcl_t0), *self.pp_layer(pcl_t1))
+            if once:
+                x, occ = pp([*pcl_t0, *pcl_t1]) if prep is None else pp([*pcl_t0, *pcl_t1], prep=prep)
+                return (x[:B], occ[:B], x[B:], occ[B:])
+            return (*pp(pcl_t0), *pp(pcl_t1))
         rows, occ = out
-        B = rows.shape[0] // 2
-        a = self.pp_layer(pcl_t0, out=(rows[:B], occ[:B]))
-        b = self.pp_layer(pcl_t1, out=(rows[B:], occ[B:]))
+        assert rows.shape[0] == 2 * B, (rows.shape, B)
+        if once:
+            x, _ = pp([*pcl_t0, *pcl_t1], out=(rows, occ), prep=prep)
+            return (x[:B], occ[:B], x[B:], occ[B:], x)
+        a = pp(pcl_t0, out=(rows[:B], occ[:B]))
+        b = pp(pcl_t1, out=(rows[B:], occ[B:]))
         return (*a, *b, rows.permute(0, 3, 1, 2))
 
     def infer_forward_direction(self, pcl_t0, pcl_t1, canvases=None):
diff --git a/liso_amd/trainer.py b/liso_amd/trainer.py
--- a/liso_amd/trainer.py
+++ b/liso_amd/trainer.py
@@ -576,14 +576,28 @@
 
 
 class _Prefetched:
-    __slots__ = ("pair", "flow", "done", "targets", "boxes", "cluster_count")
-
-    def __init__(self, pair, flow, done, targets=None, boxes=None, cluster_count=None):
+    __slots__ = ("pair", "flow", "done", "targets", "boxes", "cluster_count", "shared", "index")
+
+    def __init__(self, pair, flow, done, targets=None, boxes=None, cluster_count=None, shared=None, index=None):
         self.pair, self.flow, self.done = pair, flow, done
         self.targets, self.boxes, self.cluster_count = targets, boxes, cluster_count
+        self.shared, self.index = shared, index
 
     def is_for(self, pair):
         return self.pair[0] is pair[0] and self.pair[1] is pair[1]
+
+
+class _SharedVoxelisation:
+    __slots__ = ("prep", "clouds", "ready", "geometry", "seen")
+
+    def __init__(self, prep, clouds, ready, geometry):
+        self.prep, self.clouds, self.ready, self.geometry = prep, clouds, ready, geometry
+        self.seen = set()
+
+
+def _pillar_geometry(pfn):
+    return (tuple(float(v) for v in pfn.pc_range), tuple(float(v) for v in pfn.voxel_size), tuple(pfn.grid), pfn.max_num_points,
+            pfn.max_voxels, pfn.num_input_channels)
 
 
 class _BatchedTargets(dict):
@@ -618,7 +632,7 @@
 class LisoLoopTrainer:
 
     def __init__(self, cfg, device, compute_dtype=torch.float32, total_steps=None, slim_state_dict=None, use_graph=False,
-                 overlap=False, infer_batch=2, flow_ahead=0, exact=None):
+                 overlap=False, infer_batch=2, flow_ahead=0, exact=None, share_voxelisation=True):
         from liso_amd.networks.flow_cluster_detector.flow_cluster_detector import FlowClusterDetector
         from liso_amd.slim.model.slim import SLIM
 
@@ -667,6 +681,10 @@
                 self.infer_cus = 0
         self._pillar_prep = None
         self._prep_ahead = os.environ.get("LISO_PREP_AHEAD", "1") != "0"
+        self.share_voxelisation = bool(share_voxelisation) and os.environ.get("LISO_SHARE_VOXELISATION", "1") != "0"
+        self.slim.raft_network.encode_once = self.share_voxelisation
+        self.stage_a_replays, self.stage_a_voxelisations, self.shared_prep_steps = 0, 0, 0
+        self._infer_vox_calls, self._step_shared = 0, []
         self.pre_nms, self.post_nms = tcfg.max_num_boxes_before_nms, tcfg.max_num_boxes_after_nms
         self.nms_iou = cfg.setdefault("nms_iou_threshold", 0.1)
 
@@ -737,24 +755,36 @@
     def _graph_inputs(sample_t0, sample_t1):
         return tuple({"pcl_ta": s_["pcl_ta"], "gt": {"odom_ta_tb": s_["gt"]["odom_ta_tb"]}} for s_ in (sample_t0, sample_t1))
 
-    def _infer_flow_padded(self, sample_t0, sample_t1):
+    def _infer_flow_padded(self, sample_t0, sample_t1, share=None):
+        from liso_amd.slim.model.slim import get_network_input_pcls
+
+        raft = self.slim.raft_network
+        with torch.no_grad():
+            once = raft.encodes_once(len(get_network_input_pcls(self.cfg, sample_t0, "ta")))
+        self._infer_vox_calls = 1 if once else 2
         if not self._graph_infer:
             return self.slim.infer_point_flow_t0_t1(sample_t0, sample_t1)
-        from liso_amd.slim.model.slim import get_network_input_pcls
         from liso_amd.utils import mfma_conv as MC
 
         dev = self.device
         ins = self._graph_inputs(sample_t0, sample_t1)
         sig = TT.tree_signature(ins)
-        raft = self.slim.raft_network
         pcls = (get_network_input_pcls(self.cfg, sample_t0, "ta", to_device=dev), get_network_input_pcls(self.cfg, sample_t1, "ta", to_device=dev))
         st = self._infer_graphs.lookup(sig)
         with torch.no_grad():
             compact = raft.compact_canvas_ok(dev) if st is None else st["compact"]
+            prep = None
+            if once:
+                clouds = [*pcls[0], *pcls[1]]
+                prep = raft.pp_layer.prepare(clouds)
+                if share is not None:
+                    ready = torch.cuda.Event()
+                    ready.record(torch.cuda.current_stream(dev))
+                    share.append(_SharedVoxelisation(prep, clouds, ready, _pillar_geometry(raft.pp_layer)))
             if st is None:
-                canv = raft.encode_pillars(*pcls, compact=compact)
+                canv = raft.encode_pillars(*pcls, compact=compact, prep=prep)
             else:
-                raft.encode_pillars(*pcls, out=st["rows"], compact=compact)
+                raft.encode_pillars(*pcls, out=st["rows"], compact=compact, prep=prep)
             thr = self.slim.moving_dynamicness_threshold.value()
         if st is None:
             st = self._infer_graphs.insert(sig, {}, self.max_infer_graphs)
@@ -906,17 +936,22 @@
         if self._main_used_static is not None:
             side.wait_event(self._main_used_static)
             self._main_used_static = None
+        share = [] if self.share_voxelisation else None
         with torch.cuda.stream(side), torch.no_grad():
             if len(pairs) == 1:
-                flows = [self._infer_flow_padded(self._infer_view(pairs[0][0]), self._infer_view(pairs[0][1])).clone()]
+                flows = [self._infer_flow_padded(self._infer_view(pairs[0][0]), self._infer_view(pairs[0][1]), share).clone()]
             else:
-                flow = self._infer_flow_padded(self._stack_infer_views([p_[0] for p_ in pairs]), self._stack_infer_views([p_[1] for p_ in pairs]))
+                flow = self._infer_flow_padded(self._stack_infer_views([p_[0] for p_ in pairs]), self._stack_infer_views([p_[1] for p_ in pairs]),
+                                               share)
                 b = flow.shape[0] // len(pairs)
                 flows = [flow[k * b:(k + 1) * b].clone() for k in range(len(pairs))]
             done = torch.cuda.Event()
             done.record(side)
-        for p_, fl in zip(pairs, flows):
-            self._flows.append(_Prefetched(pair=p_, flow=fl, done=done))
+        self.stage_a_replays += 1
+        self.stage_a_voxelisations += self._infer_vox_calls
+        shared = share[0] if share else None
+        for k, (p_, fl) in enumerate(zip(pairs, flows)):
+            self._flows.append(_Prefetched(pair=p_, flow=fl, done=done, shared=shared, index=k))
 
     def _same_shapes(self, pa, pb):
         sig = lambda pair: TT.tree_signature(self._graph_inputs(self._infer_view(pair[0]), self._infer_view(pair[1])), skip_dim=1)
@@ -959,12 +994,14 @@
                 count.copy_(self.cluster_detector.last_num_labels.max().reshape(1), non_blocking=True)
             done = torch.cuda.Event()
             done.record(side)
-        self._mined.append(_Prefetched(pair=pair, flow=f.flow, done=done, targets=targets, boxes=boxes, cluster_count=count))
+        self._mined.append(_Prefetched(pair=pair, flow=f.flow, done=done, targets=targets, boxes=boxes, cluster_count=count,
+                                       shared=f.shared, index=f.index))
 
     def _take_mined(self, pair, cur):
         m = self._take(self._mined, pair)
         if m is None:
             return None
+        self._step_shared.append((m.shared, m.index))
         if os.environ.get("LISO_NO_COUNT_WAIT") == "1":
             cur.wait_event(m.done)
             for t in list(m.targets.values()) + [v for v in m.boxes.__dict__.values() if torch.is_tensor(v)]:
@@ -980,6 +1017,18 @@
             t.record_stream(cur)
         return m.targets, m.boxes
 
+    def _shared_prep(self, held, pcls):
+        if not self.share_voxelisation or not held or len(held) != len(pcls):
+            return None
+        sv, first = held[0]
+        if sv is None or any(h[0] is not sv or h[1] != first + j for j, h in enumerate(held)):
+            return None
+        if first + len(pcls) > len(sv.clouds) or any(sv.clouds[first + j] is not c for j, c in enumerate(pcls)):
+            return None
+        if sv.geometry != _pillar_geometry(self.detector.net.model.pfn):
+            return None
+        return sv, first
+
     def step(self, sample_t0, sample_t1, upcoming=()):
         return self.step_batch([(sample_t0, sample_t1)], upcoming)
 
@@ -995,12 +1044,14 @@
             if inputs_ready is not None:
                 cur.wait_event(inputs_ready)
         mined = []
+        self._step_shared = []
         for pair in pairs:
             sample_t0, sample_t1 = pair
             got = self._take_mined(pair, cur) if cuda else None
             if got is None:
                 f = self._take(self._flows, pair)
                 if f is not None:
+                    self._step_shared.append((f.shared, f.index))
                     cur.wait_event(f.done)
                     f.flow.record_stream(cur)
                     flow = f.flow
@@ -1032,8 +1083,26 @@
                 for t in (cat, *parts):
                     t.record_stream(cur)
                 prep = got_prep
+        if prep is None and self.overlap and cuda:
+            hit = self._shared_prep(self._step_shared if len(self._step_shared) == nb else [], pcls)
+            if hit is not None:
+                sv, first = hit
+                cur.wait_event(sv.ready)
+                if cur.cuda_stream not in sv.seen:
+                    cat, _, parts = sv.prep
+                    for t in (cat, *parts):
+                        t.record_stream(cur)
+                    sv.seen.add(cur.cuda_stream)
+                prep = (*sv.prep, first, len(pcls))
+                self.shared_prep_steps += 1
+        self._step_shared = []
         loss = self.detector.step(pcls, targets, prep=prep) if prep is not None else self.detector.step(pcls, targets)
-        if self.overlap and cuda and len(upcoming) >= len(pairs) and self._prep_ahead and self.detector.use_graph:
+        prep_ahead = self.overlap and cuda and len(upcoming) >= len(pairs) and self._prep_ahead and self.detector.use_graph
+        if prep_ahead and self.share_voxelisation:
+            held = [next((e for e in (*self._mined, *self._flows) if e.is_for(p_)), None) for p_ in upcoming[:len(pairs)]]
+            prep_ahead = self._shared_prep([(e.shared, e.index) if e is not None else (None, None) for e in held],
+                                           [c for p_ in upcoming[:len(pairs)] for c in p_[0]["pcl_full_no_ground_ta"]]) is None
+        if prep_ahead:
             nxt = [c for p_ in upcoming[:len(pairs)] for c in p_[0]["pcl_full_no_ground_ta"]]
             side = self._mine_stream
             if self._inputs_ready is not None:
@@ -1053,10 +1122,18 @@
             missing = [p_ for k, p_ in enumerate(up) if not has(self._flows, p_) and not has(self._mined, p_)
                        and not any(p_[0] is q[0] and p_[1] is q[1] for q in up[:k])]
             if missing and any(p_ is q for p_ in missing for q in up[:ahead + fa]):
+                align = nb if self.share_voxelisation and nb > 1 and self.infer_batch % nb == 0 else 1
+                where = {id(p_): k for k, p_ in reversed(list(enumerate(up)))}
                 while missing:
                     n = 1
                     while n < min(len(missing), self.infer_batch) and self._same_shapes(missing[0], missing[n]):
                         n += 1
+                    if align > 1:
+                        whole = [m for m in range(n, 0, -1) if (where[id(missing[m - 1])] + 1) % align == 0]
+                        if whole:
+                            n = whole[0]
+                        elif where[id(missing[0])] >= ahead + fa:
+                            break
                     self._stage_a(*missing[:n])
                     missing = missing[n:]
             for p_ in up[:ahead]:
```
